# su1phurd/UAV-WRF-LES-PPO-LSTM

Hardware: AMD Instinct MI355X
Metric: env-steps/sec (rollout + GAE + 5-epoch PPO update), 4096 envs x 128 T per GPU, LSTM h=128 x1 (higher is better)
Workload: dtype f32

## Files before the change

include/uavppo.h:

```cpp
#ifndef UAVPPO_H
#define UAVPPO_H

#include <stddef.h>
#include <stdint.h>

#ifdef __cplusplus
extern "C" {
#endif

typedef struct uav_ctx uav_ctx;
typedef void* uav_stream;

#define UAV_ABI_VERSION 9

#define UAV_GAE_REFERENCE_EXACT 0
#define UAV_GAE_STANDARD        1

#define UAV_ENV_V20 0
#define UAV_ENV_V21 1
#define UAV_ENV_V11 2

#define UAV_FIELD_PROCEDURAL   0
#define UAV_FIELD_MATERIALISED 1

int         uav_abi_version(void);
const char* uav_last_error(void);

int  uav_create(uav_ctx** out, int device, size_t ws_bytes);
void uav_destroy(uav_ctx* ctx);

#define UAV_ARITH_FP16X3   0
#define UAV_ARITH_BF16X6   1
#define UAV_ARITH_F32_MFMA 2
int uav_set_lstm_arith(uav_ctx* ctx, int mode);
int uav_get_lstm_arith(const uav_ctx* ctx);
#define UAV_DEBUG_STEP_F32 1u
#define UAV_DEBUG_X_F32    2u
#define UAV_DEBUG_DG_F32   4u
#define UAV_DEBUG_GEMM_TN_OFF 0x10u
int uav_set_debug_flags(uav_ctx* ctx, unsigned flags);
int uav_absmax(uav_ctx* ctx, const float* x, int64_t n, float* out, uav_stream stream);

int uav_gae(uav_ctx* ctx, const float* rew, const float* val, const float* done,
            const float* last_val, int n_env, int horizon, float gamma, float lam, int mode,
            float* adv, uav_stream stream);

int uav_adv_stats(uav_ctx* ctx, const float* adv, int64_t n, double* stats3, uav_stream stream);
int uav_adv_normalise(uav_ctx* ctx, const float* adv, const float* val, int64_t n,
                      const double* stats3, float* adv_out, float* ret_out, uav_stream stream);

int uav_pack_success_bits(uav_ctx* ctx, const uint8_t* flags, int64_t n, int cap, uint8_t* msg, uav_stream stream);

int uav_ppo_loss(uav_ctx* ctx, const float* logits, const float* value, const int32_t* act,
                 const float* logp_old, const float* adv, const float* ret, const float* val_old,
                 int64_t n, int n_act, float inv_n, float clip, float ent_beta,
                 double* loss_sums, float* dlogits, float* dvalue, float* dhead_bias,
                 uav_stream stream);

int uav_ppo_loss_from_y(uav_ctx* ctx, const float* y, const float* w_head, const float* b_head,
                        const int32_t* act, const float* logp_old, const float* adv, const float* ret,
                        const float* val_old, int64_t n, int hidden, int n_act, float inv_n, float clip,
                        float ent_beta, double* loss_sums, float* dheads, float* dhead_bias,
                        uav_stream stream);

int uav_policy_sample(uav_ctx* ctx, const float* logits, int64_t n, int n_act, const float* u,
                      uint64_t seed, uint64_t counter, int64_t index_offset, const int32_t* forced_act,
                      int32_t* act_out, float* logp_out, float* probs_out, int32_t* nan_count,
                      uav_stream stream);

int uav_policy_sample_at(uav_ctx* ctx, const float* heads, int64_t heads_stride, int64_t n, int n_act, uint64_t seed,
                         uint64_t counter, int64_t index_offset, const int32_t* forced_act, int32_t* act_out, int T, int t,
                         int32_t* act_buf, float* val_buf, float* logp_buf, int32_t* nan_count, uav_stream stream);
int uav_store_transition(uav_ctx* ctx, int n, int T, int t, float* keep, const float* rew, const float* done,
                         const uint8_t* flags, float* keep_buf, float* rew_buf, float* done_buf, uint8_t* flags_buf,
                         uav_stream stream);

int uav_clip_adam(uav_ctx* ctx, float* param, const float* grad, float* exp_avg,
                  float* exp_avg_sq, int64_t n, int64_t step, float lr, float beta1, float beta2,
                  float eps, float max_norm, float* gnorm_out, float* pmax_out, uav_stream stream);
int uav_clip_adamw(uav_ctx* ctx, float* param, const float* grad, float* exp_avg, float* exp_avg_sq, int64_t n,
                   int64_t step, float lr, float beta1, float beta2, float eps, float weight_decay, float max_norm,
                   float* gnorm_out, uav_stream stream);
int uav_smooth_l1(uav_ctx* ctx, const float* pred, const float* target, int64_t n, float beta, double* loss_mean,
                  float* dpred, uav_stream stream);
int uav_mse_bce(uav_ctx* ctx, const float* out, const float* target, int64_t n, double* loss_mean, float* dout,
                uav_stream stream);

size_t uav_disc_param_count(int obs_dim, int n_act, int hidden);

int uav_disc_grad(uav_ctx* ctx, const float* params, const float* obs_e, const int32_t* act_e, int64_t n_e, const float* obs_p,
                  const int32_t* act_p, int64_t n_p, int obs_dim, int n_act, int hidden, float inv_ne, float inv_np,
                  double* loss_sums, float* grad, uav_stream stream);

int uav_disc_reward(uav_ctx* ctx, const float* params, const float* obs, const int32_t* act, int64_t n, int obs_dim, int n_act,
                    int hidden, float env_coef, float gail_coef, const float* rew_env, float* rew_out, uav_stream stream);

size_t uav_lstm_stepper_bytes(int N, int I, int H);
int uav_lstm_stepper_begin(uav_ctx* ctx, void* state, const float* w_ih, const float* w_hh, const float* b_ih,
                           const float* b_hh, const float* h0, const float* c0, int N, int I, int H, uav_stream stream);
int uav_lstm_stepper_step(uav_ctx* ctx, void* state, const float* x, const void* below, const float* keep_t, int N, int T,
                          int t, int I, int H, float* y, float* stash, float* hn, float* cn, uav_stream stream);
typedef struct uav_stepper_call {
    void* state; const float* x; const void* below; const float* keep_t;
    int t, I;
    float *y, *stash, *hn, *cn;
} uav_stepper_call;
int uav_lstm_stepper_step_pair(uav_ctx* ctx, const uav_stepper_call* a, const uav_stepper_call* b, int N, int T, int H,
                               uav_stream stream);

int uav_gemm_f32(uav_ctx* ctx, int64_t M, int64_t N, int64_t K, const float* A, int64_t sa_m,
                 int64_t sa_k, const float* B, int64_t sb_k, int64_t sb_n, float* C, int64_t ldc,
                 const float* bias, int accumulate, uav_stream stream);

int uav_gemm_f16x3(uav_ctx* ctx, int64_t M, int64_t N, int64_t K, const float* A, int64_t sa_m,
                   int64_t sa_k, const float* B, int64_t sb_k, int64_t sb_n, float* C, int64_t ldc,
                   const float* bias, int accumulate, const float* a_absmax, uav_stream stream);

int uav_colsum(uav_ctx* ctx, const float* x, int64_t rows, int cols, float* out, uav_stream stream);
int uav_ln_relu(uav_ctx* ctx, float* z, float* a, float* rstd, const float* gamma, const float* beta, int64_t rows,
                int cols, uav_stream stream);
int uav_ln_relu_bwd(uav_ctx* ctx, float* d, const float* xhat, const float* rstd, const float* gamma, const float* beta,
                    int64_t rows, int cols, float* dgamma, float* dbeta, uav_stream stream);

int64_t uav_mlp_param_count(int in_dim, int h1, int h2, int n_act);
int64_t uav_mlp_stash_floats(int h1, int h2);
int uav_mlp_fwd(uav_ctx* ctx, const float* params, const float* x, int64_t B, int in_dim, int h1,
                int h2, int n_act, float* heads, float* stash, uav_stream stream);
int uav_mlp_bwd(uav_ctx* ctx, const float* params, const float* x, float* stash,
                const float* dheads, int64_t B, int in_dim, int h1, int h2, int n_act,
                float* grad, uav_stream stream);

int uav_mlp_ppo_grad(uav_ctx* ctx, const float* params, const float* obs, const int32_t* act, const float* logp_old,
                     const float* adv, const float* ret, const float* val_old, int64_t n, int in_dim, int h1, int h2,
                     int n_act, float inv_n, float clip, float ent_beta, double* loss_sums, float* grad,
                     uav_stream stream);

int uav_lstm_fwd(uav_ctx* ctx, const float* x, const float* keep, const float* h0, const float* c0,
                 const float* w_ih, const float* w_hh, const float* b_ih, const float* b_hh,
                 int N, int T, int I, int H, float* y, float* hn, float* cn, float* stash,
                 const float* w_head, const float* b_head, int n_heads, float* heads,
                 uav_stream stream);
int uav_lstm_bwd(uav_ctx* ctx, const float* keep, const float* stash, const float* w_hh,
                 const float* dy, const float* dheads, const float* w_head, int n_heads,
                 const float* dhn, const float* dcn, int N, int T, int H, float* dgates, float* dh0,
                 float* dc0, const float* w_ih, int I, float* dx, uav_stream stream);
size_t uav_lstm_dgates_bytes(uav_ctx* ctx, int N, int T, int H);
int uav_lstm_dgates_f32(uav_ctx* ctx, const float* dgates, int N, int T, int H, float* out, uav_stream stream);
#define UAV_BWD_FUSES_DX 1
#define UAV_BWD_TAKES_DHEADS 2
#define UAV_BWD_STACKS 4
int uav_lstm_bwd_caps(uav_ctx* ctx, int I, int H);
typedef struct uav_lstm_bwd_layer {
    const float* keep;
    const float* stash;
    const float* w_hh;
    const float* w_ih;
    float* dgates;
    float* dx;
    const float* dhn;
    const float* dcn;
    float* dh0;
    float* dc0;
} uav_lstm_bwd_layer;
int uav_lstm_bwd_stack(uav_ctx* ctx, int n_layers, const uav_lstm_bwd_layer* layers, const float* dy, const float* dheads,
                       const float* w_head, int n_heads, int N, int T, int H, uav_stream stream);
int uav_lstm_wgrad(uav_ctx* ctx, const float* x, const float* keep, const float* h0, const float* y,
                   const float* stash, const float* dgates, const float* w_ih, const float* dheads,
                   int n_heads, int N, int T, int I, int H, float* dw_ih, float* dw_hh, float* db, float* db_hh,
                   float* dw_head, float* dx, uav_stream stream);

typedef struct uav_env_cfg {
    int32_t variant;
    int32_t field_mode;
    int32_t n_fields;
    int32_t bonus_is_f64;
    int32_t env_offset;
    int32_t n_env_total;
    int32_t trend_k;
    int32_t pad_;
    double  radius;
    double  bonus;
    uint64_t seed;
    const double* bank;
    const double* bank_src;
    const void*   curriculum;
} uav_env_cfg;

int uav_episode_rows(uav_ctx* ctx, const float* rew, const float* info, const uint8_t* flags, int n_env, int T, int env_offset,
                     double* carry, double* rows, int cap, int32_t* count, uav_stream stream);
size_t uav_curriculum_state_bytes(void);
int uav_curriculum_init(uav_ctx* ctx, void* state, double radius, double bonus, int bonus_is_f64, uav_stream stream);
int uav_curriculum_update(uav_ctx* ctx, void* state, const uint8_t* msgs, int world, int cap, uav_stream stream);

size_t uav_env_state_bytes(int n_env);
int uav_env_reset(uav_ctx* ctx, void* state, int n_env, const uav_env_cfg* cfg ,
                  float* obs_out, uav_stream stream);
int uav_env_step(uav_ctx* ctx, void* state, int n_env, const uav_env_cfg* cfg ,
                 const int32_t* act, const double* noise, float* obs_out, float* rew, float* done,
                 uint8_t* flags, float* info, float* term_obs, double* rew64, uav_stream stream);
int uav_env_peek(uav_ctx* ctx, const void* state, int n_env, float* pos, double* source,
                 int32_t* steps, int32_t* episode, uav_stream stream);

int uav_env_materialise(uav_ctx* ctx, const void* state, int n_env, const uav_env_cfg* cfg ,
                        int env_index, double* field_out, uav_stream stream);

int uav_rollout(uav_ctx* ctx, void* env_state, int n_env, const uav_env_cfg* cfg ,
                int policy_kind, const float* params, int hidden, int horizon, uint64_t iter,
                float* cur_obs, float* h, float* c, float* obs, int32_t* act, float* rew,
                float* val, float* logp, float* done, uint8_t* flags, float* keep, float* last_val,
                const int32_t* forced_act, const double* noise, int32_t* nan_count,
                float* stash, float* y_out, float* info, float* heads, uav_stream stream);

int uav_greedy_episodes(uav_ctx* ctx, void* env_state, int n_env, const uav_env_cfg* cfg , int policy_kind,
                        const float* params, int hidden, int steps, float* cur_obs, float* h, float* c, uint8_t* active,
                        const double* noise, int32_t* act, float* obs, float* pos, uint8_t* flags, int32_t* nan_count,
                        uav_stream stream);

typedef struct uav_stop_rule {
    int32_t window;
    float   pos_std_max, conc_coef, conc_peak, conc_min;
} uav_stop_rule;

int uav_greedy_episodes_stop(uav_ctx* ctx, void* env_state, int n_env, const uav_env_cfg* cfg , int policy_kind,
                             const float* params, int hidden, int steps, float* cur_obs, float* h, float* c, uint8_t* active,
                             const double* noise, int32_t* act, float* obs, float* pos, uint8_t* flags, int32_t* nan_count,
                             const uav_stop_rule* rule , float* stop_win, int32_t* stop_cnt, float* rule_val,
                             uav_stream stream);

int uav_stop_stability(uav_ctx* ctx, int n, const uav_stop_rule* rule , const float* pos, const float* obs2,
                       int64_t obs2_stride, const uint8_t* active, float* stop_win, int32_t* stop_cnt, uint8_t* stop,
                       float* value, uav_stream stream);

size_t uav_peak_stop_param_count(int hidden);

int uav_peak_stop_scan(uav_ctx* ctx, const float* params, int hidden, int window, const float* series, int64_t row_stride,
                       int64_t elem_stride, int n, int steps, const uint8_t* active, float* hist, int32_t* hist_cnt,
                       float prob_min, float* peak, float* prob, int32_t* first_hit, uav_stream stream);

int uav_rollout_tail(uav_ctx* ctx, void* env_state, int n_env, const uav_env_cfg* cfg , const float* y, int64_t y_stride,
                     int hidden, const float* w_head, const float* b_head, int n_act, float* heads, int64_t heads_stride, int T,
                     int t, uint64_t seed, uint64_t counter, int64_t index_offset, const int32_t* forced_act, const double* noise,
                     int32_t* act_out, float* cur_obs, float* obs_seq, float* keep, int32_t* act_buf, float* val_buf,
                     float* logp_buf, float* keep_buf, float* rew_buf, float* done_buf, uint8_t* flags_buf, int32_t* nan_count,
                     uav_stream stream);

#define UAV_COMM_ID_BYTES 128
int uav_rccl_version(int* out );
int uav_comm_unique_id(void* id_out );
int uav_comm_init(uav_ctx* ctx, const void* id , int rank, int world);
int uav_comm_world(const uav_ctx* ctx);
int uav_comm_rank(const uav_ctx* ctx);
int uav_comm_destroy(uav_ctx* ctx);
int uav_allreduce(uav_ctx* ctx, float* flat_grad, int64_t count, uav_stream stream);
int uav_allreduce_f64(uav_ctx* ctx, double* buf, int64_t count, uav_stream stream);
int uav_allgather_bytes(uav_ctx* ctx, const void* send, void* recv, int64_t bytes_per_rank, uav_stream stream);

#ifdef __cplusplus
}
#endif
#endif
```

uav-wrf-les-ppo-lstm_amd/csrc/adam.hip:

```cpp
#include "common.h"

constexpr int NORM_BLOCKS = 256;

__global__ __launch_bounds__(256) void sumsq_partial(const float* __restrict__ g, int64_t n,
                                                     double* __restrict__ partial, unsigned* __restrict__ pmax_bits) {
    __shared__ double sm[4];
    if (pmax_bits && blockIdx.x == 0 && threadIdx.x == 0) *pmax_bits = 0u;
    double q = 0.0;
    for (int64_t i = (int64_t)blockIdx.x * 256 + threadIdx.x; i < n; i += (int64_t)gridDim.x * 256) {
        const double v = (double)g[i];
        q += v * v;
    }
    q = block256_sum(q, sm);
    if (threadIdx.x == 0) partial[blockIdx.x] = q;
}

__global__ __launch_bounds__(256) void adam_kernel(float* __restrict__ p, const float* __restrict__ g,
                                                   float* __restrict__ m, float* __restrict__ v, int64_t n,
                                                   const double* __restrict__ partial, int nb, float max_norm,
                                                   float* __restrict__ gnorm_out, float b1, float b2,
                                                   float step_size, float sqrt_bc2, float eps, float decay,
                                                   unsigned* __restrict__ pmax_bits) {
#pragma clang fp contract(off)
    __shared__ double sm[4];
    __shared__ float coef_s;
    double q = 0.0;
    for (int i = threadIdx.x; i < nb; i += 256) q += partial[i];
    q = block256_sum(q, sm);
    if (threadIdx.x == 0) {
        const float norm = (float)sqrt(q);
        float coef = max_norm / (norm + 1e-6f);
        coef = coef > 1.0f ? 1.0f : coef;
        if (!(max_norm > 0.f)) coef = 1.0f;
        coef_s = coef;
        if (gnorm_out && blockIdx.x == 0) *gnorm_out = norm;
    }
    __syncthreads();
    const float coef = coef_s;
    float amax = 0.f;
    for (int64_t i = (int64_t)blockIdx.x * 256 + threadIdx.x; i < n; i += (int64_t)gridDim.x * 256) {
        const float gi = g[i] * coef;
        const float mi = m[i] + (gi - m[i]) * (1.0f - b1);
        const float vi = v[i] * b2 + (1.0f - b2) * gi * gi;
        m[i] = mi;
        v[i] = vi;
        const float denom = sqrtf(vi) / sqrt_bc2 + eps;
        const float pn = p[i] * decay - step_size * (mi / denom);
        p[i] = pn;
        amax = fmaxf(amax, pn == pn ? fabsf(pn) : __builtin_inff());
    }
    if (pmax_bits) {
#pragma unroll
        for (int o = 32; o > 0; o >>= 1) amax = fmaxf(amax, __shfl_xor(amax, o, 64));
        __shared__ float wmax[4];
        if ((threadIdx.x & 63) == 0) wmax[threadIdx.x >> 6] = amax;
        __syncthreads();
        if (threadIdx.x == 0)
            atomicMax(pmax_bits, __float_as_uint(fmaxf(fmaxf(wmax[0], wmax[1]), fmaxf(wmax[2], wmax[3]))));
    }
}

__global__ __launch_bounds__(256) void absmax_kernel(const float* __restrict__ x, int64_t n, unsigned* __restrict__ out) {
    float amax = 0.f;
    for (int64_t i = (int64_t)blockIdx.x * 256 + threadIdx.x; i < n; i += (int64_t)gridDim.x * 256) {
        const float v = x[i];
        amax = fmaxf(amax, v == v ? fabsf(v) : __builtin_inff());
    }
#pragma unroll
    for (int o = 32; o > 0; o >>= 1) amax = fmaxf(amax, __shfl_xor(amax, o, 64));
    if ((threadIdx.x & 63) == 0) atomicMax(out, __float_as_uint(amax));
}

extern "C" int uav_absmax(uav_ctx* ctx, const float* x, int64_t n, float* out, uav_stream stream) {
    UAV_REQUIRE(ctx && x && out && n > 0, "uav_absmax: bad argument");
    UAV_CHECK_HIP(hipMemsetAsync(out, 0, sizeof(float), as_stream(stream)));
    int nb = (int)((n + 4095) / 4096);
    if (nb > 1024) nb = 1024;
    hipLaunchKernelGGL(absmax_kernel, dim3(nb), dim3(256), 0, as_stream(stream), x, n, reinterpret_cast<unsigned*>(out));
    UAV_LAUNCH_CHECK();
    return 0;
}

static int clip_adam_impl(uav_ctx* ctx, float* param, const float* grad, float* exp_avg, float* exp_avg_sq, int64_t n,
                          int64_t step, float lr, float beta1, float beta2, float eps, float weight_decay, float max_norm,
                          float* gnorm_out, float* pmax_out, uav_stream stream) {
    UAV_REQUIRE(ctx && param && grad && exp_avg && exp_avg_sq && n > 0 && step >= 1, "uav_clip_adam: bad argument");
    unsigned* pmax_bits = reinterpret_cast<unsigned*>(pmax_out);
    double* partial = (double*)ctx->ws;
    int nb = (int)((n + 1023) / 1024);
    if (nb > NORM_BLOCKS) nb = NORM_BLOCKS;
    hipLaunchKernelGGL(sumsq_partial, dim3(nb), dim3(256), 0, as_stream(stream), grad, n, partial, pmax_bits);
    const double bc1 = 1.0 - pow((double)beta1, (double)step);
    const double bc2 = 1.0 - pow((double)beta2, (double)step);
    const float step_size = (float)((double)lr / bc1);
    const float sqrt_bc2 = (float)sqrt(bc2);
    int ab = (int)((n + 255) / 256);
    if (ab > 2048) ab = 2048;
    hipLaunchKernelGGL(adam_kernel, dim3(ab), dim3(256), 0, as_stream(stream), param, grad, exp_avg, exp_avg_sq, n,
                       partial, nb, max_norm, gnorm_out, beta1, beta2, step_size, sqrt_bc2, eps, 1.0f - lr * weight_decay, pmax_bits);
    UAV_LAUNCH_CHECK();
    return 0;
}

extern "C" int uav_clip_adam(uav_ctx* ctx, float* param, const float* grad, float* exp_avg, float* exp_avg_sq, int64_t n,
                             int64_t step, float lr, float beta1, float beta2, float eps, float max_norm, float* gnorm_out,
                             float* pmax_out, uav_stream stream) {
    return clip_adam_impl(ctx, param, grad, exp_avg, exp_avg_sq, n, step, lr, beta1, beta2, eps, 0.f, max_norm, gnorm_out,
                          pmax_out, stream);
}

extern "C" int uav_clip_adamw(uav_ctx* ctx, float* param, const float* grad, float* exp_avg, float* exp_avg_sq, int64_t n,
                              int64_t step, float lr, float beta1, float beta2, float eps, float weight_decay, float max_norm,
                              float* gnorm_out, uav_stream stream) {
    return clip_adam_impl(ctx, param, grad, exp_avg, exp_avg_sq, n, step, lr, beta1, beta2, eps, weight_decay, max_norm,
                          gnorm_out, nullptr, stream);
}

__global__ __launch_bounds__(256) void smooth_l1_kernel(const float* __restrict__ pred, const float* __restrict__ target,
                                                        int64_t n, float beta, double* __restrict__ loss_mean,
                                                        float* __restrict__ dpred) {
    __shared__ double sm[4];
    double s = 0.0;
    const float inv_n = 1.0f / (float)n;
    for (int64_t i = threadIdx.x; i < n; i += 256) {
        const float d = pred[i] - target[i], a = fabsf(d);
        if (a < beta) { s += 0.5 * (double)d * d / beta; dpred[i] = d / beta * inv_n; }
        else { s += (double)a - 0.5 * beta; dpred[i] = (d > 0.f ? 1.f : d < 0.f ? -1.f : d) * inv_n; }
    }
    const double r = block256_sum(s, sm);
    if (threadIdx.x == 0) loss_mean[0] = r / (double)n;
}

extern "C" int uav_smooth_l1(uav_ctx* ctx, const float* pred, const float* target, int64_t n, float beta, double* loss_mean,
                             float* dpred, uav_stream stream) {
    UAV_REQUIRE(ctx && pred && target && loss_mean && dpred && n > 0 && beta > 0.f, "uav_smooth_l1: bad argument");
    hipLaunchKernelGGL(smooth_l1_kernel, dim3(1), dim3(256), 0, as_stream(stream), pred, target, n, beta, loss_mean, dpred);
    UAV_LAUNCH_CHECK();
    return 0;
}

__global__ __launch_bounds__(256) void mse_bce_kernel(const float* __restrict__ out, const float* __restrict__ target, int64_t n,
                                                      double* __restrict__ loss_mean, float* __restrict__ dout) {
    __shared__ double sm[4];
    double s = 0.0;
    const float inv_n = 1.0f / (float)n;
    for (int64_t i = threadIdx.x; i < n; i += 256) {
        const float d = out[2 * i] - target[2 * i];
        const float z = out[2 * i + 1], yb = target[2 * i + 1];
        const float p = 1.0f / (1.0f + expf(-z));
        const float lgp = logf(p), lgq = logf(1.0f - p);
        const float lp = lgp < -100.f ? -100.f : lgp, lq = lgq < -100.f ? -100.f : lgq;
        s += (double)d * d - ((double)yb * lp + (1.0 - (double)yb) * lq);
// ... 15 lines not shown
```

uav-wrf-les-ppo-lstm_amd/csrc/gae.hip:

```cpp
#include "common.h"

__global__ __launch_bounds__(256) void gae_scan_kernel(const float* __restrict__ rew,
                                                       const float* __restrict__ val,
                                                       const float* __restrict__ done,
                                                       const float* __restrict__ last_val, int n_env,
                                                       int T, float gamma, float gl, int mode,
                                                       float* __restrict__ adv) {
#pragma clang fp contract(off)
    const int lane = threadIdx.x & 63;
    const int env = blockIdx.x * 4 + (threadIdx.x >> 6);
    if (env >= n_env) return;
    const size_t row = (size_t)env * T;
    const int nchunk = (T + 63) >> 6;
    float carry = 0.f;
    float v_right = 0.f, d_right = 0.f;
    for (int c = nchunk - 1; c >= 0; --c) {
        const int t = c * 64 + lane;
        const bool in = t < T;
        const float r = in ? rew[row + t] : 0.f;
        const float v = in ? val[row + t] : 0.f;
        const float d = in ? done[row + t] : 0.f;
        float v1 = __shfl_down(v, 1, 64);
        float d1 = __shfl_down(d, 1, 64);
        if (lane == 63) { v1 = v_right; d1 = d_right; }
        float a = 1.f, b = 0.f;
        if (in) {
            float nnt, nv;
            const bool last = (t == T - 1);
            if (mode == UAV_GAE_REFERENCE_EXACT) {
                nnt = 1.0f - (last ? d : d1);
                nv = (last ? v : v1) * nnt;
            } else {
                nnt = 1.0f - d;
                nv = (last ? (last_val ? last_val[env] : 0.f) : v1) * nnt;
            }
            b = (r + gamma * nv) - v;
            a = gl * nnt;
        }
#pragma unroll
        for (int o = 1; o < 64; o <<= 1) {
            const float a2 = __shfl_down(a, o, 64);
            const float b2 = __shfl_down(b, o, 64);
            if (lane + o < 64) {
                b = b + a * b2;
                a = a * a2;
            }
        }
        const float A = b + a * carry;
        if (in) adv[row + t] = A;
        carry = __shfl(A, 0, 64);
        v_right = __shfl(v, 0, 64);
        d_right = __shfl(d, 0, 64);
    }
}

constexpr int STATS_BLOCKS = 512;

__global__ __launch_bounds__(256) void adv_stats_partial(const float* __restrict__ x, int64_t n,
                                                         double* __restrict__ partial) {
    __shared__ double sm[4];
    double s = 0.0, q = 0.0;
    for (int64_t i = (int64_t)blockIdx.x * 256 + threadIdx.x; i < n; i += (int64_t)gridDim.x * 256) {
        const double v = (double)x[i];
        s += v;
        q += v * v;
    }
    s = block256_sum(s, sm);
    q = block256_sum(q, sm);
    if (threadIdx.x == 0) {
        partial[2 * blockIdx.x] = s;
        partial[2 * blockIdx.x + 1] = q;
    }
}

__global__ __launch_bounds__(256) void adv_stats_final(const double* __restrict__ partial, int nb,
                                                       int64_t n, double* __restrict__ stats3) {
    __shared__ double sm[4];
    double s = 0.0, q = 0.0;
    for (int i = threadIdx.x; i < nb; i += 256) {
        s += partial[2 * i];
        q += partial[2 * i + 1];
    }
    s = block256_sum(s, sm);
    q = block256_sum(q, sm);
    if (threadIdx.x == 0) {
        stats3[0] = s;
        stats3[1] = q;
        stats3[2] = (double)n;
    }
}

__global__ __launch_bounds__(256) void adv_normalise_kernel(const float* __restrict__ adv,
                                                            const float* __restrict__ val, int64_t n,
                                                            const double* __restrict__ stats3,
                                                            float* __restrict__ adv_out,
                                                            float* __restrict__ ret_out) {
#pragma clang fp contract(off)
    const double cnt = stats3[2];
    const double mean_d = stats3[0] / cnt;
    const double var = (stats3[1] - cnt * mean_d * mean_d) / (cnt - 1.0);
    const float mean = (float)mean_d;
    float sd = (float)sqrt(var > 0.0 ? var : (var == var ? 0.0 : var));
    if (sd < 1e-6f || sd != sd) sd = 1.0f;
    const float den = sd + 1e-6f;
    for (int64_t i = (int64_t)blockIdx.x * 256 + threadIdx.x; i < n; i += (int64_t)gridDim.x * 256) {
        const float a = (adv[i] - mean) / den;
        adv_out[i] = a;
        ret_out[i] = a + val[i];
    }
}

__global__ __launch_bounds__(1024) void pack_success_kernel(const uint8_t* __restrict__ flags, int64_t n, int cap,
                                                            uint8_t* __restrict__ msg) {
    __shared__ int part[32];
    const int tid = threadIdx.x;
    int64_t per = (n + 1023) / 1024;
    per = (per + 15) / 16 * 16;
    const int64_t lo = (int64_t)tid * per, hi = (lo + per < n) ? lo + per : n;
    const bool vec = (reinterpret_cast<uintptr_t>(flags) & 15) == 0;
    auto visit = [&](auto&& f) {
        int64_t i = lo;
        if (vec)
            for (; i + 16 <= hi; i += 16) {
                const uint4 w = *reinterpret_cast<const uint4*>(flags + i);
                if ((w.x | w.y | w.z | w.w) == 0u) continue;
                const unsigned ww[4] = {w.x, w.y, w.z, w.w};
#pragma unroll
                for (int q = 0; q < 4; ++q)
#pragma unroll
                    for (int k = 0; k < 4; ++k) {
                        const uint8_t v = (ww[q] >> (8 * k)) & 255;
                        if (v) f(v);
                    }
            }
        for (; i < hi; ++i)
            if (flags[i]) f(flags[i]);
    };
    int cnt = 0;
    visit([&](uint8_t) { ++cnt; });
    for (int i = tid; i < 4 + cap + 1; i += 1024) msg[i] = 0;
    const int lane = tid & 63, wv = tid >> 6;
    int inc = cnt;
#pragma unroll
    for (int o = 1; o < 64; o <<= 1) {
        const int v = __shfl_up(inc, o, 64);
        if (lane >= o) inc += v;
    }
    if (lane == 63) part[wv] = inc;
    __syncthreads();
    if (wv == 0) {
        int t = lane < 16 ? part[lane] : 0;
#pragma unroll
        for (int o = 1; o < 16; o <<= 1) {
// ... 91 lines not shown
            __syncthreads();
            for (int i = lane; i < nb; i += 64) chunk[i] = m[4 + base + i];
            __syncthreads();
            CurriculumState s = sh;
            for (int k = 0; k < nb;) {
                const int need = CUR_WINDOW - s.hist_len;
                const int n = (nb - k < need) ? nb - k : need;
                int succ = 0;
                for (int j = 0; j < n; j += 64) {
                    const int i = j + lane;
                    succ += __popcll(__ballot(i < n && chunk[k + i] != 0));
                }
                k += n;
                const double env_radius = s.radius;
                s.episodes += n; s.successes += succ;
                s.hist_len += n; s.win_succ += succ;
                const bool full = s.hist_len >= CUR_WINDOW;
                double rate = 0.0;
                if (full) {
                    rate = (double)s.win_succ / (double)s.hist_len;
                    s.bonus = s.bonus * pow(CUR_DECAY_FACTOR, 1.0 + rate);
                    s.bonus_is_f64 = 1.0;
                }
                s.bonus = fmax(s.bonus, 0.1);
                if (full) {
                    if (rate > CUR_SUCCESS_THRESHOLD)
                        s.radius = fmax(CUR_MIN_RADIUS, s.radius * pow(CUR_RADIUS_DECAY, 2.0 + 3.0 * (rate - CUR_SUCCESS_THRESHOLD)));
                    else if (rate < 0.25)
                        s.radius = fmin(CUR_INITIAL_RADIUS, s.radius * 1.1);
                    const double d = s.radius - env_radius;
                    if (fabs(d) > 5.0) s.radius = env_radius + 5.0 * (d > 0.0 ? 1.0 : (d < 0.0 ? -1.0 : 0.0));
                    s.hist_len = 0; s.win_succ = 0;
                }
            }
            __syncthreads();
            if (lane == 0) sh = s;
        }
    }
    __syncthreads();
    if (lane == 0) *st = sh;
}

extern "C" {

int uav_gae(uav_ctx* ctx, const float* rew, const float* val, const float* done,
            const float* last_val, int n_env, int horizon, float gamma, float lam, int mode,
            float* adv, uav_stream stream) {
    UAV_REQUIRE(ctx && rew && val && done && adv, "uav_gae: NULL argument");
    UAV_REQUIRE(n_env > 0 && horizon > 0, "uav_gae: n_env=%d horizon=%d", n_env, horizon);
    UAV_REQUIRE(mode == UAV_GAE_REFERENCE_EXACT || mode == UAV_GAE_STANDARD, "uav_gae: mode %d", mode);
    const float gl = (float)((double)gamma * (double)lam);
    const int blocks = (n_env + 3) / 4;
    hipLaunchKernelGGL(gae_scan_kernel, dim3(blocks), dim3(256), 0, as_stream(stream), rew, val, done,
                       last_val, n_env, horizon, gamma, gl, mode, adv);
    UAV_LAUNCH_CHECK();
    return 0;
}

int uav_adv_stats(uav_ctx* ctx, const float* adv, int64_t n, double* stats3, uav_stream stream) {
    UAV_REQUIRE(ctx && adv && stats3 && n > 0, "uav_adv_stats: bad argument");
    int nb = (int)((n + 1023) / 1024);
    if (nb > STATS_BLOCKS) nb = STATS_BLOCKS;
    double* partial = (double*)ctx->ws;
    hipLaunchKernelGGL(adv_stats_partial, dim3(nb), dim3(256), 0, as_stream(stream), adv, n, partial);
    hipLaunchKernelGGL(adv_stats_final, dim3(1), dim3(256), 0, as_stream(stream), partial, nb, n, stats3);
    UAV_LAUNCH_CHECK();
    return 0;
}

int uav_adv_normalise(uav_ctx* ctx, const float* adv, const float* val, int64_t n,
                      const double* stats3, float* adv_out, float* ret_out, uav_stream stream) {
    UAV_REQUIRE(ctx && adv && val && stats3 && adv_out && ret_out && n > 0, "uav_adv_normalise: bad argument");
    int nb = (int)((n + 1023) / 1024);
    if (nb > 2048) nb = 2048;
    hipLaunchKernelGGL(adv_normalise_kernel, dim3(nb), dim3(256), 0, as_stream(stream), adv, val, n, stats3,
                       adv_out, ret_out);
    UAV_LAUNCH_CHECK();
    return 0;
}


int uav_episode_rows(uav_ctx* ctx, const float* rew, const float* info, const uint8_t* flags, int n_env, int T, int env_offset,
                     double* carry, double* rows, int cap, int32_t* count, uav_stream stream) {
    UAV_REQUIRE(ctx && rew && info && flags && carry && rows && count && n_env > 0 && T > 0 && cap > 0, "uav_episode_rows: bad argument");
    hipLaunchKernelGGL(episode_rows_kernel, dim3((n_env + 63) / 64), dim3(64), 0, as_stream(stream), rew, info, flags, n_env, T, env_offset,
                       carry, rows, cap, count);
    UAV_LAUNCH_CHECK();
    return 0;
}

size_t uav_curriculum_state_bytes(void) { return sizeof(CurriculumState); }

int uav_curriculum_init(uav_ctx* ctx, void* state, double radius, double bonus, int bonus_is_f64, uav_stream stream) {
    UAV_REQUIRE(ctx && state && radius > 0.0, "uav_curriculum_init: bad argument");
    hipLaunchKernelGGL(curriculum_init_kernel, dim3(1), dim3(64), 0, as_stream(stream), (CurriculumState*)state, radius, bonus, bonus_is_f64);
    UAV_LAUNCH_CHECK();
    return 0;
}

int uav_curriculum_update(uav_ctx* ctx, void* state, const uint8_t* msgs, int world, int cap, uav_stream stream) {
    UAV_REQUIRE(ctx && state && msgs && world > 0 && cap > 0, "uav_curriculum_update: bad argument");
    hipLaunchKernelGGL(curriculum_update_kernel, dim3(1), dim3(64), 0, as_stream(stream), (CurriculumState*)state, msgs, world, cap);
    UAV_LAUNCH_CHECK();
    return 0;
}

int uav_pack_success_bits(uav_ctx* ctx, const uint8_t* flags, int64_t n, int cap, uint8_t* msg, uav_stream stream) {
    UAV_REQUIRE(ctx && flags && msg && n > 0 && cap > 0, "uav_pack_success_bits: bad argument");
    hipLaunchKernelGGL(pack_success_kernel, dim3(1), dim3(1024), 0, as_stream(stream), flags, n, cap, msg);
    UAV_LAUNCH_CHECK();
    return 0;
}

}
```

uav-wrf-les-ppo-lstm_amd/csrc/lstm.hip:

```cpp
#include <stdlib.h>
#include <type_traits>
#include "common.h"

int gemm_f32(uav_ctx* ctx, int64_t M, int64_t N, int64_t K, const float* A, int64_t sa_m, int64_t sa_k,
             const float* B, int64_t sb_k, int64_t sb_n, float* C, int64_t ldc, const float* bias,
             int accumulate, hipStream_t st);
int colsum(uav_ctx* ctx, const float* X, int64_t B, int C, float* out, float* scratch, hipStream_t st);
int colsum_absmax(uav_ctx* ctx, const float* X, int64_t B, int C, float* out, float* scratch, unsigned* absmax_bits,
                  hipStream_t st);
int colsum_xw(uav_ctx* ctx, const float* X, int64_t B, int C, const float* x, int I, float* colsum_out, float* xw_out,
              float* scratch, unsigned* absmax_bits, hipStream_t st, int xw_transposed = 0);
bool gemm_h3_ok(int64_t M, int64_t N, int64_t K, const float* A, int64_t sa_m, int64_t sa_k, const float* B, int64_t sb_k,
                int64_t sb_n);
int gemm_h3(uav_ctx* ctx, int64_t M, int64_t N, int64_t K, const float* A, int64_t sa_m, int64_t sa_k, const float* B,
            int64_t sb_k, int64_t sb_n, float* C, int64_t ldc, const float* bias, int accumulate, const unsigned* a_absmax,
            hipStream_t st);
int lstm_generic_fwd(uav_ctx* ctx, const float* keep, const float* h0, const float* c0, const float* w_hh, int N, int T,
                     int H, float* y, float* hn, float* cn, float* stash, hipStream_t st);
int lstm_h3_fwd(uav_ctx* ctx, const float* x, int I, const float* w_ih, const float* b_ih, const float* b_hh,
                const float* keep, const float* h0, const float* c0, const float* w_hh, int N, int T, float* y, float* hn,
                float* cn, float* stash, hipStream_t st);
bool lstm_h3_step_path(int H);
int lstm_generic_bwd(uav_ctx* ctx, const float* keep, const float* stash, const float* w_hh, const float* dy,
                     const float* dheads, const float* w_head, int n_heads,
                     const float* dhn, const float* dcn, int N, int T, int H, float* dgates, float* dh0, float* dc0,
                     const float* w_ih, int I, float* dx, hipStream_t st);
int lstm_generic_bwd_caps(int I, int H);
bool lstm_h3_stack_ok(int H);
bool lstm_h3_dg_packed(int H);
int lstm_pc_unpack(const void* dgates, int N, int T, float* out, hipStream_t st);
int lstm_pc_hprev_rows(const float* y, const float* keep, const float* h0, int N, int T, float* out, hipStream_t st);
int lstm_pc_wgrad(uav_ctx* ctx, const float* x, const float* y, const float* h0, const void* dgates, int N, int T, int I, float* dw_ih,
                  float* dw_hh, float* db, float* db_hh, hipStream_t st);
int lstm_h3_bwd_stack(uav_ctx* ctx, int nl, const uav_lstm_bwd_layer* layers, const float* dy, const float* dheads,
                      const float* w_head, int n_heads, int N, int T, hipStream_t st);
int lstm_wgrad_fused(uav_ctx* ctx, const float* dgates, const float* y, const float* keep, const float* h0,
                     const float* x, int I, const float* dheads, int NH, int N, int T, int H,
                     float* dw_ih, float* dw_hh, float* db, float* db_hh, float* dw_head, hipStream_t st);

constexpr int MT = 16;
constexpr int TC = 32;

#define sigmoidf_ fast_sigmoid
#define tanhf_ fast_tanh

template <int H>
struct FwdGeom {
    static constexpr int NW = H / 16;
    static constexpr int KS = H / 4;
    static constexpr int SEG = KS + 4;
    static constexpr int S = 4 * SEG + 8;
    static constexpr size_t LDS = (2 * MT * S + TC * MT * 8 + (TC + 1) * MT) * sizeof(float);
};
template <int H>
__device__ __forceinline__ int hpos(int u) { return (u / (H / 4)) * FwdGeom<H>::SEG + (u % (H / 4)); }

template <int H, bool FUSE_X>
__global__ __launch_bounds__(H * 4) void lstm_fwd_kernel(
    const float* __restrict__ x, const float* __restrict__ keep, const float* __restrict__ h0,
    const float* __restrict__ c0, const float* __restrict__ w_ih, const float* __restrict__ w_hh,
    const float* __restrict__ b_ih, const float* __restrict__ b_hh, int N, int T, int I,
    float* __restrict__ y, float* __restrict__ hn, float* __restrict__ cn, float* __restrict__ stash) {
    using G = FwdGeom<H>;
    constexpr int KS = G::KS, SEG = G::SEG, S = G::S;
    extern __shared__ __attribute__((aligned(16))) float smem[];
    float* hbuf = smem;
    float* xbuf = hbuf + 2 * MT * S;
    float* kbuf = xbuf + TC * MT * 8;

    const int lane = threadIdx.x & 63, w = threadIdx.x >> 6;
    const int j = lane & 15, kq = lane >> 4;
    const int u = 16 * w + j;
    const int n0 = blockIdx.x * MT;

    float wh[4][KS];
#pragma unroll
    for (int q = 0; q < 4; ++q) {
        const float* src = w_hh + (size_t)(q * H + u) * H + kq * KS;
#pragma unroll
        for (int s = 0; s < KS; s += 4) {
            const float4 v = *reinterpret_cast<const float4*>(src + s);
            wh[q][s] = v.x; wh[q][s + 1] = v.y; wh[q][s + 2] = v.z; wh[q][s + 3] = v.w;
        }
    }
    float wx[4][2], bias[4];
#pragma unroll
    for (int q = 0; q < 4; ++q) {
        bias[q] = FUSE_X ? (b_ih[q * H + u] + b_hh[q * H + u]) : 0.f;
#pragma unroll
        for (int s = 0; s < 2; ++s) {
            const int k = 2 * kq + s;
// ... 916 lines not shown

int uav_lstm_bwd_caps(uav_ctx* ctx, int I, int H) {
    if (!ctx) return 0;
    if (H == 64 || H == 128) return UAV_BWD_TAKES_DHEADS;
    uav_enter(ctx);
    return lstm_generic_bwd_caps(I, H);
}

size_t uav_lstm_dgates_bytes(uav_ctx* ctx, int N, int T, int H) {
    if (!ctx || N <= 0 || T <= 0 || H <= 0) return 0;
    uav_enter(ctx);
    if (H == DgPack::H && lstm_h3_dg_packed(H)) return DgPack(N, T).bytes();
    return (size_t)N * T * 4 * H * sizeof(float);
}

int uav_lstm_dgates_f32(uav_ctx* ctx, const float* dgates, int N, int T, int H, float* out, uav_stream stream) {
    UAV_REQUIRE(ctx && dgates && out && N > 0 && T > 0 && H > 0, "uav_lstm_dgates_f32: bad argument");
    uav_enter(ctx);
    const int form = H == DgPack::H ? uav_dg_form(ctx, dgates) : 0;
    if (form > 0 || (form < 0 && H == DgPack::H && lstm_h3_dg_packed(H))) return lstm_pc_unpack(dgates, N, T, out, as_stream(stream));
    UAV_CHECK_HIP(hipMemcpyAsync(out, dgates, (size_t)N * T * 4 * H * sizeof(float), hipMemcpyDeviceToDevice, as_stream(stream)));
    return 0;
}

int uav_lstm_bwd_stack(uav_ctx* ctx, int n_layers, const uav_lstm_bwd_layer* layers, const float* dy, const float* dheads,
                       const float* w_head, int n_heads, int N, int T, int H, uav_stream stream) {
    UAV_REQUIRE(ctx && layers, "uav_lstm_bwd_stack: NULL argument");
    uav_enter(ctx);
    UAV_REQUIRE((dy != nullptr) != (dheads != nullptr), "uav_lstm_bwd_stack: give exactly one of dy / dheads");
    UAV_REQUIRE(!dheads || (w_head && n_heads > 0 && n_heads <= 8), "uav_lstm_bwd_stack: dheads needs w_head and 1..8 heads");
    UAV_REQUIRE(N > 0 && T > 0, "uav_lstm_bwd_stack: N=%d T=%d", N, T);
    UAV_REQUIRE(H == 256 && lstm_h3_stack_ok(H), "uav_lstm_bwd_stack: H = 256 on the fp16-split arithmetic only (uav_lstm_bwd_caps)");
    return lstm_h3_bwd_stack(ctx, n_layers, layers, dy, dheads, w_head, n_heads, N, T, as_stream(stream));
}

int uav_lstm_bwd(uav_ctx* ctx, const float* keep, const float* stash, const float* w_hh, const float* dy,
                 const float* dheads, const float* w_head, int n_heads, const float* dhn, const float* dcn, int N,
                 int T, int H, float* dgates, float* dh0, float* dc0, const float* w_ih, int I, float* dx,
                 uav_stream stream) {
    UAV_REQUIRE(ctx && stash && w_hh && dgates, "uav_lstm_bwd: NULL argument");
    uav_enter(ctx);
    UAV_REQUIRE((dy != nullptr) != (dheads != nullptr), "uav_lstm_bwd: give exactly one of dy / dheads");
    UAV_REQUIRE(!dheads || (w_head && n_heads > 0 && n_heads <= 8), "uav_lstm_bwd: dheads needs w_head and 1..8 heads");
    UAV_REQUIRE(N > 0 && T > 0, "uav_lstm_bwd: N=%d T=%d", N, T);
    if (H != 64 && H != 128) {
        return lstm_generic_bwd(ctx, keep, stash, w_hh, dy, dheads, w_head, n_heads, dhn, dcn, N, T, H, dgates, dh0, dc0, w_ih, I, dx,
                                as_stream(stream));
    }
    UAV_REQUIRE(!dx, "uav_lstm_bwd: dx is not formed by the H = 64 / 128 sequence kernels (uav_lstm_wgrad does it)");
    return lstm_bwd_seq(keep, stash, w_hh, dy, dheads, w_head, n_heads, dhn, dcn, N, T, H, dgates, dh0, dc0,
                        as_stream(stream));
}

int uav_lstm_wgrad(uav_ctx* ctx, const float* x, const float* keep, const float* h0, const float* y,
                   const float* stash, const float* dgates, const float* w_ih, const float* dheads, int n_heads, int N,
                   int T, int I, int H, float* dw_ih, float* dw_hh, float* db, float* db_hh, float* dw_head, float* dx,
                   uav_stream stream) {
    UAV_REQUIRE(ctx && x && h0 && y && dgates && w_ih && dw_ih && dw_hh && db, "uav_lstm_wgrad: NULL argument");
    uav_enter(ctx);
    UAV_REQUIRE(N > 0 && T > 0 && I > 0 && H > 0, "uav_lstm_wgrad: N=%d T=%d I=%d H=%d", N, T, I, H);
    UAV_REQUIRE(!dheads || (dw_head && n_heads > 0 && n_heads <= 8), "uav_lstm_wgrad: dheads needs dw_head, 1..8 heads");
    hipStream_t st = as_stream(stream);
    const int64_t NT = (int64_t)N * T;
    int rc;
    if (I <= 6 && (H == 64 || H == 128)) {
        if ((rc = lstm_wgrad_fused(ctx, dgates, y, keep, h0, x, I, dheads, n_heads, N, T, H, dw_ih, dw_hh, db, db_hh,
                                   dw_head, st))) return rc;
    } else {
        UAV_REQUIRE(stash, "uav_lstm_wgrad: stash is required when I > 6");
        const size_t red_floats = (size_t)1024 * 9 * 4 * H + 64;
        UAV_REQUIRE(ctx->ws_bytes >= red_floats * sizeof(float) * 2, "uav_lstm_wgrad: workspace too small");
        float* red = (float*)((char*)ctx->ws + ctx->ws_bytes) - red_floats;
        uav_ctx sub = *ctx;
        sub.ws_bytes = ctx->ws_bytes - red_floats * sizeof(float);
        bool done = false;
        const float* hprev = stash + 5 * H;
        int64_t ld_hprev = 6 * H;
        {
            const int form = uav_dg_form(ctx, dgates), want = lstm_h3_dg_packed(H) ? 1 : 0;
            UAV_REQUIRE(form < 0 || H != DgPack::H || form == want, "uav_lstm_wgrad: this dgates buffer was written as %s but the handle's "
                        "arithmetic mode / debug flags now read %s (they must not change between uav_lstm_bwd and uav_lstm_wgrad)",
                        form ? "fp16 piece chunks" : "f32 rows", want ? "fp16 piece chunks" : "f32 rows");
            UAV_REQUIRE(H != DgPack::H || want || ctx->hslot_form.find(stash) != 0, "uav_lstm_wgrad: this stash was written by "
                        "uav_lstm_fwd / the stepper on the fp16-split arithmetic, which leaves out its h_prev slot, but the handle's "
                        "arithmetic mode / debug flags now read that slot (they must not change between the forward pass and "
                        "uav_lstm_wgrad)");
        }
        if (lstm_h3_dg_packed(H)) {
            if ((I <= 8 || I == H) && !dx) {
                if ((rc = lstm_pc_wgrad(ctx, x, y, h0, dgates, N, T, I, dw_ih, dw_hh, db, db_hh, st))) return rc;
                done = true;
            } else {
                const size_t f32_bytes = (size_t)NT * 5 * H * sizeof(float);
                UAV_REQUIRE(sub.ws_bytes >= f32_bytes + (64u << 20), "uav_lstm_wgrad (h=256, I=%d%s): needs %zu bytes of workspace for "
                            "the gate gradients and h_prev as f32 rows", I, dx ? ", dx" : "", f32_bytes + (64u << 20));
                float* rows = (float*)((char*)sub.ws + sub.ws_bytes - f32_bytes);
                sub.ws_bytes -= f32_bytes;
                if ((rc = lstm_pc_unpack(dgates, N, T, rows, st))) return rc;
                float* hp = rows + (size_t)NT * 4 * H;
                if ((rc = lstm_pc_hprev_rows(y, keep, h0, N, T, hp, st))) return rc;
                dgates = rows;
                hprev = hp;
                ld_hprev = H;
            }
        }
        const bool h3 = !uav_want_f32_mfma() && !uav_want_bf16x6() && (reinterpret_cast<uintptr_t>(dgates) & 15) == 0;
        unsigned* amax = h3 ? reinterpret_cast<unsigned*>(red + (size_t)1024 * 9 * 4 * H) : nullptr;
        auto product = [&](int64_t M, int64_t Nn, int64_t K, const float* A, int64_t sa_m, int64_t sa_k, const float* B,
                           int64_t sb_k, int64_t sb_n, float* C, int64_t ldc) {
            if (h3 && gemm_h3_ok(M, Nn, K, A, sa_m, sa_k, B, sb_k, sb_n))
                return gemm_h3(&sub, M, Nn, K, A, sa_m, sa_k, B, sb_k, sb_n, C, ldc, nullptr, 0, amax, st);
            return gemm_f32(&sub, M, Nn, K, A, sa_m, sa_k, B, sb_k, sb_n, C, ldc, nullptr, 0, st);
        };
        if (!done) {
            const bool narrow = I <= 8 && (reinterpret_cast<uintptr_t>(dgates) & 15) == 0;
            if (narrow) rc = colsum_xw(&sub, dgates, NT, 4 * H, x, I, db, dw_ih, red, amax, st);
            else rc = colsum_absmax(&sub, dgates, NT, 4 * H, db, red, amax, st);
            if (rc) return rc;
            if (db_hh) UAV_CHECK_HIP(hipMemcpyAsync(db_hh, db, (size_t)4 * H * sizeof(float), hipMemcpyDeviceToDevice, st));
            if ((rc = product(4 * H, H, NT, dgates, 1, 4 * H, hprev, ld_hprev, 1, dw_hh, H))) return rc;
            if (!narrow && (rc = product(4 * H, I, NT, dgates, 1, 4 * H, x, I, 1, dw_ih, I))) return rc;
        }
        if (dheads) {
            if (H % 4 == 0 && (reinterpret_cast<uintptr_t>(y) & 15) == 0)
                rc = colsum_xw(&sub, y, NT, H, dheads, n_heads, nullptr, dw_head, red, nullptr, st, 1);
            else
                rc = gemm_f32(&sub, n_heads, H, NT, dheads, 1, n_heads, y, H, 1, dw_head, H, nullptr, 0, st);
            if (rc) return rc;
        }
        if (dx) return product(NT, I, 4 * H, dgates, 4 * H, 1, w_ih, I, 1, dx, I);
        return 0;
    }
    if (dx) return gemm_f32(ctx, NT, I, 4 * H, dgates, 4 * H, 1, w_ih, I, 1, dx, I, nullptr, 0, st);
    return 0;
}

}
```

uav-wrf-les-ppo-lstm_amd/csrc/rollout.hip:

```cpp
#include "env_core.h"
#include "loss_core.h"
#include "rows_dot_core.h"
#include "stop_rule_core.h"

typedef float f32x4 __attribute__((ext_vector_type(4)));

int env_params_from_cfg(const uav_ctx* ctx, const uav_env_cfg* cfg, int n_env, EnvParams& P);
int launch_rollout_mlp(uav_ctx* ctx, void* env_state, int n_env, const uav_env_cfg* cfg, const float* params, int horizon,
                       uint64_t iter, float* cur_obs, float* obs, int32_t* act, float* rew, float* val, float* logp,
                       float* done, uint8_t* flags, float* last_val, const int32_t* forced_act, const double* noise,
                       int32_t* nan_count, float* info, float* heads, hipStream_t st);
int launch_greedy_mlp(const EnvParams& P, void* env_state, int n_env, const float* params, int steps, float* cur_obs,
                      uint8_t* active, const double* noise, int32_t* act, float* obs, float* pos, uint8_t* flags,
                      int32_t* nan_count, hipStream_t st);
int launch_greedy_mlp_stop(const EnvParams& P, void* env_state, int n_env, const float* params, int steps, float* cur_obs,
                           uint8_t* active, const double* noise, int32_t* act, float* obs, float* pos, uint8_t* flags,
                           int32_t* nan_count, const StopRule& rule, float* stop_win, int32_t* stop_cnt, float* rule_val,
                           hipStream_t st);

constexpr int RMT = 16;

#ifdef UAV_X6_PROFILE
__device__ unsigned long long g_roll_prof[8];
#define R_PROF_DECL unsigned long long pm_[8] = {0, 0, 0, 0, 0, 0, 0, 0}, pl_ = __builtin_readcyclecounter()
#define R_PROF_MARK(i) do { const unsigned long long n_ = __builtin_readcyclecounter(); pm_[i] += n_ - pl_; pl_ = n_; } while (0)
#define R_PROF_FLUSH() do { if (blockIdx.x == 0 && threadIdx.x == 0) for (int i_ = 0; i_ < 8; ++i_) g_roll_prof[i_] = pm_[i_]; } while (0)
extern "C" int uav_roll_prof_read(unsigned long long* out) {
    return hipMemcpyFromSymbol(out, HIP_SYMBOL(g_roll_prof), sizeof(g_roll_prof)) == hipSuccess ? 0 : 1;
}
#else
#define R_PROF_DECL
#define R_PROF_MARK(i)
#define R_PROF_FLUSH()
#endif
constexpr float R_F32_EPS = 1.1920928955078125e-07f;

#define r_sigmoid fast_sigmoid
#define r_tanh fast_tanh


template <int H>
struct RGeom {
    static constexpr int NW = H / 16;
    static constexpr int NS = H / 32;
    static constexpr int RS = H + 8;
    static constexpr int PLANE = RMT * RS;
    static constexpr int W0 = 4 * NS * 2 * 64 * 8;
    static constexpr size_t LDS = (2 * PLANE  + 2 * PLANE  + W0) * sizeof(unsigned short) +
                                  (NW * 8 * 64  + 4 * H ) * sizeof(float);
};

struct RolloutBufs {
    float* cur_obs; float* h; float* c;
    float* obs; int32_t* act; float* rew; float* val; float* logp; float* done; uint8_t* flags; float* keep;
    float* last_val; const int32_t* forced_act; const double* noise; int32_t* nan_count;
    float* info;
    float* heads;
    float* stash; float* y;
    uint8_t* active; float* pos;
    float* stop_win; int32_t* stop_cnt; float* rule_val; StopRule rule;
};

template <int H, int NA, bool GREEDY = false, bool STOP = false, bool TREND = false>
__global__ __launch_bounds__(H * 4) void rollout_lstm_kernel(EnvParams P_arg, EnvBlob blob, int N, int T,
                                                                        uint64_t iter, const float* __restrict__ params,
                                                                        RolloutBufs B) {
    using G = RGeom<H>;
    constexpr int NS = G::NS, RS = G::RS, PLANE = G::PLANE, W0 = G::W0, NW = G::NW;
    constexpr int NH = NA + 1;
    extern __shared__ __attribute__((aligned(16))) float smem[];
    unsigned short* hpl = reinterpret_cast<unsigned short*>(smem);
    unsigned short* whp = hpl + 2 * PLANE;
    unsigned short* w0p = whp + 2 * PLANE;
    float* wxl = reinterpret_cast<float*>(w0p + W0);
    float* bl = wxl + NW * 512;
    __shared__ __attribute__((aligned(16))) float xbuf[RMT * 8];
    __shared__ float kbuf[RMT];
    __shared__ float hd[RMT * 16];
    __shared__ unsigned short vis[RMT * NVIS];
    __shared__ EnvState es_s[RMT];
    __shared__ float trs[4 * RMT * 8];
    __shared__ __attribute__((aligned(16))) f32x4 acc0[4 * 64];
    __shared__ double env_tab[ENV_LDS_TABLE_DOUBLES];
    static_assert(!STOP || GREEDY, "rollout_lstm_kernel: the stop rule belongs to the greedy episodes");
    constexpr size_t STOP_LDS = STOP ? RMT * 2 * STOP_WIN_MAX * sizeof(float) : 0;
    static_assert(G::LDS + sizeof(xbuf) + sizeof(kbuf) + sizeof(hd) + sizeof(vis) + sizeof(es_s) + sizeof(trs) + sizeof(acc0) +
                      sizeof(env_tab) + STOP_LDS <= 160 * 1024, "rollout_lstm_kernel: LDS over 160 KB per workgroup");
    float* ring = nullptr;
    StopRing sr{0, 0};
    if constexpr (STOP) {
        __shared__ float rings[RMT * 2 * STOP_WIN_MAX];
        static_assert(sizeof(rings) == STOP_LDS, "stop rings");
        ring = rings + (threadIdx.x & 15) * 2 * STOP_WIN_MAX;
    }
    EnvParams P = P_arg;
    env_params_refresh(P);
    env_tables_to_lds(P, env_tab, threadIdx.x, H * 4);
    const int I = TREND ? 6 + P.trend_k : 6;

    const float* w_ih = params;
    const float* w_hh = w_ih + 4 * H * I;
    const float* b_ih = w_hh + 4 * H * H;
    const float* b_hh = b_ih + 4 * H;
    const float* w_hd = b_hh + 4 * H;
    const float* b_hd = w_hd + NH * H;

    const int lane = threadIdx.x & 63;
    const int w = __builtin_amdgcn_readfirstlane(threadIdx.x >> 6);
    const int j = lane & 15, kq = lane >> 4;
    const int n0 = blockIdx.x * RMT;
    const bool is_env_wave = (w == 0);
    const int uw = 16 * w + j;
    const int uo = 16 * w + 4 * kq;
    const int nj = min(n0 + j, N - 1);
    const bool live = n0 + j < N;
    const int my_env = n0 + lane;
    const bool env_lane = is_env_wave && lane < RMT && my_env < N;
    unsigned short* myvis = vis + (lane & 15) * NVIS;

    f16x8 wb[4][NS][2];
    f16x8* const w0f = reinterpret_cast<f16x8*>(w0p) + lane;
#pragma unroll
    for (int q = 0; q < 4; ++q)
#pragma unroll
        for (int s = 0; s < NS; ++s) {
            const float* src = w_hh + (size_t)(q * H + uw) * H + 32 * s + 8 * kq;
            const float4 v0 = *reinterpret_cast<const float4*>(src), v1 = *reinterpret_cast<const float4*>(src + 4);
            const float v[8] = {v0.x, v0.y, v0.z, v0.w, v1.x, v1.y, v1.z, v1.w};
            f16x8 p0v, p1v;
#pragma unroll
            for (int i = 0; i < 8; ++i) {
                _Float16 p0, p1;
                split2h(v[i], p0, p1);
                p0v[i] = p0; p1v[i] = p1;
            }
            if (is_env_wave) {
                w0f[((q * NS + s) * 2 + 0) * 64] = p0v;
                w0f[((q * NS + s) * 2 + 1) * 64] = p1v;
            } else {
                wb[q][s][0] = p0v; wb[q][s][1] = p1v;
            }
        }
    float* const wxw = wxl + w * 512 + lane;
#pragma unroll
    for (int q = 0; q < 4; ++q)
#pragma unroll
        for (int s = 0; s < 2; ++s) {
            const int k = 2 * kq + s;
            wxw[(2 * q + s) * 64] = (k < I) ? w_ih[(size_t)(q * H + uw) * I + k] : 0.f;
        }
    for (int idx = threadIdx.x; idx < 4 * H; idx += H * 4) bl[idx] = b_ih[idx] + b_hh[idx];
    for (int idx = threadIdx.x; idx < 16 * H; idx += H * 4) {
        const int hdx = idx / H, uu = idx % H;
        _Float16 p0, p1;
        split2h((hdx < NH) ? w_hd[(size_t)hdx * H + uu] : 0.f, p0, p1);
        unsigned short* d = whp + hdx * RS + uu;
        d[0] = h_bits(p0); d[PLANE] = h_bits(p1);
    }
    auto put_h = [&](const float (&hv)[4]) {
        unsigned short b[2][4];
#pragma unroll
        for (int r = 0; r < 4; ++r) {
            _Float16 p0, p1;
            split2h(hv[r], p0, p1);
            b[0][r] = h_bits(p0); b[1][r] = h_bits(p1);
        }
#pragma unroll
        for (int pc = 0; pc < 2; ++pc) {
            uint2 v;
            v.x = (unsigned)b[pc][0] | ((unsigned)b[pc][1] << 16);
            v.y = (unsigned)b[pc][2] | ((unsigned)b[pc][3] << 16);
            *reinterpret_cast<uint2*>(hpl + pc * PLANE + j * RS + uo) = v;
        }
    };
    float c_reg[4];
    {
        const float4 cv = *reinterpret_cast<const float4*>(B.c + (size_t)nj * H + uo);
        const float4 hv = *reinterpret_cast<const float4*>(B.h + (size_t)nj * H + uo);
        c_reg[0] = cv.x; c_reg[1] = cv.y; c_reg[2] = cv.z; c_reg[3] = cv.w;
        const float h_in[4] = {hv.x, hv.y, hv.z, hv.w};
        put_h(h_in);
        if constexpr (TREND && !GREEDY)
            if (B.stash && live) *reinterpret_cast<float4*>(B.stash + (size_t)(n0 + j) * T * (6 * H) + 5 * H + uo) = hv;
    }
    bool ran = true;
    if (is_env_wave && lane < RMT) {
        const int n = min(my_env, N - 1);
        es_s[lane] = env_load(blob, n);
        for (int k = 0; k < NVIS; ++k) myvis[k] = blob.visited[(size_t)n * NVIS + k];
#pragma unroll
        for (int f = 0; f < 8; ++f) xbuf[lane * 8 + f] = f < I ? B.cur_obs[(size_t)n * I + f] : 0.f;
        if constexpr (GREEDY) {
            ran = my_env < N && B.active[n] != 0;
            kbuf[lane] = ran ? 1.f : 0.f;
            if constexpr (STOP)
                sr = stop_ring_load(ring, B.stop_win + (size_t)n * B.rule.window * 2, B.stop_cnt[n], B.rule.window);
        } else {
            kbuf[lane] = 1.f;
        }
    }
    lds_barrier();

    f32x4 acc[4];
    int bo = uo;
    asm volatile("" : "+v"(bo));
    const float* blu = bl + bo;
    auto bias_acc = [&]() {
#pragma unroll
        for (int q = 0; q < 4; ++q) {
            const float4 v = *reinterpret_cast<const float4*>(blu + q * H);
            acc[q] = f32x4{v.x, v.y, v.z, v.w};
        }
    };
    auto recurrent = [&](auto&& wp0, auto&& wp1) {
        bias_acc();
        f32x4 acl[4];
#pragma unroll
        for (int q = 0; q < 4; ++q) acl[q] = f32x4{0.f, 0.f, 0.f, 0.f};
        const unsigned short* hrow = hpl + j * RS + 8 * kq;
#pragma unroll
        for (int s = 0; s < NS; ++s) {
            const f16x8 a0 = *reinterpret_cast<const f16x8*>(hrow + 32 * s);
            const f16x8 a1 = *reinterpret_cast<const f16x8*>(hrow + PLANE + 32 * s);
#pragma unroll
            for (int q = 0; q < 4; ++q) acl[q] = __builtin_amdgcn_mfma_f32_16x16x32_f16(wp1(q, s), a0, acl[q], 0, 0, 0);
#pragma unroll
            for (int q = 0; q < 4; ++q) acc[q] = __builtin_amdgcn_mfma_f32_16x16x32_f16(wp0(q, s), a0, acc[q], 0, 0, 0);
#pragma unroll
            for (int q = 0; q < 4; ++q) acl[q] = __builtin_amdgcn_mfma_f32_16x16x32_f16(wp0(q, s), a1, acl[q], 0, 0, 0);
            asm volatile("" ::: "memory");
        }
#pragma unroll
        for (int q = 0; q < 4; ++q) acc[q] = acc[q] + acl[q] * H3_LO;
    };
    auto recurrent_regs = [&]() {
        recurrent([&](int q, int s) { return wb[q][s][0]; }, [&](int q, int s) { return wb[q][s][1]; });
// ... 301 lines not shown
                    if (B.heads) {
#pragma unroll
                        for (int a = 0; a < NA; ++a) trs[3 * RMT * 8 + lane * 8 + a] = z[a];
                    }
                    if (B.info) {
#pragma unroll
                        for (int f = 0; f < 5; ++f) trs[2 * RMT * 8 + lane * 8 + f] = (float)so.info[f];
                        trs[2 * RMT * 8 + lane * 8 + 5] = so.obs[2];
                        trs[2 * RMT * 8 + lane * 8 + 6] = es.px;
                        trs[2 * RMT * 8 + lane * 8 + 7] = es.py;
                    }
                    constexpr int OW = TREND ? 8 : 6;
                    constexpr int SRC = TREND ? 3 * RMT * 8 + 5 : RMT * 8 + 6;
                    float ob_old[OW];
#pragma unroll
                    for (int f = 0; f < OW; ++f) ob_old[f] = xbuf[lane * 8 + f];
#pragma unroll
                    for (int f = 0; f < OW; ++f) trs[RMT * 8 + lane * 8 + f] = ob_old[f];
                    trs[SRC + lane * 8] = (float)es.sx;
                    trs[SRC + lane * 8 + 1] = (float)es.sy;
                    if (so.done) {
                        es.episode += 1;
                        env_begin_episode(P, eg, es, myvis);
                        env_obs(P, es, myvis, so.obs);
                    }
#pragma unroll
                    for (int f = 0; f < OW; ++f) xbuf[lane * 8 + f] = f < I ? so.obs[f] : 0.f;
                    es_s[lane] = es;
                    kbuf[lane] = so.done ? 0.f : 1.f;
                }
            }
            R_PROF_MARK(5);
            lds_barrier();
            if (!value_only && t + 1 < steps) {
#pragma unroll
                for (int q = 0; q < 4; ++q) acc[q] = acc0[q * 64 + lane];
            }
            if (!value_only) keep_fixup(t);
        }
        R_PROF_FLUSH();
    }
    if (live) *reinterpret_cast<float4*>(B.c + (size_t)(n0 + j) * H + uo) = float4{c_reg[0], c_reg[1], c_reg[2], c_reg[3]};
    if (GREEDY && env_lane) B.active[my_env] = kbuf[lane] != 0.f ? 1 : 0;
    if (env_lane && ran) {
        env_store(blob, my_env, es_s[lane]);
        for (int k = 0; k < NVIS; ++k) blob.visited[(size_t)my_env * NVIS + k] = myvis[k];
#pragma unroll
        for (int f = 0; f < (TREND ? 8 : 6); ++f) if (f < I) B.cur_obs[(size_t)my_env * I + f] = xbuf[lane * 8 + f];
        if constexpr (STOP)
            B.stop_cnt[my_env] = stop_ring_store(ring, sr, B.stop_win + (size_t)my_env * B.rule.window * 2, B.rule.window);
    }
}

template <int H, bool GREEDY = false, bool STOP = false, bool TREND = false>
static int launch_rollout(const EnvParams& P, EnvBlob blob, int N, int T, uint64_t iter, const float* params,
                          const RolloutBufs& B, hipStream_t st) {
    const dim3 grid((N + RMT - 1) / RMT), block(H * 4);
    UAV_CHECK_HIP(uav_dyn_lds(reinterpret_cast<const void*>(&rollout_lstm_kernel<H, 5, GREEDY, STOP, TREND>), (int)RGeom<H>::LDS));
    hipLaunchKernelGGL((rollout_lstm_kernel<H, 5, GREEDY, STOP, TREND>), grid, block, RGeom<H>::LDS, st, P, blob, N, T, iter, params, B);
    UAV_LAUNCH_CHECK();
    return 0;
}

template <int A>
__global__ __launch_bounds__(256) void rollout_tail_kernel(
    EnvParams P, EnvBlob b, int n, const float* __restrict__ y, int64_t ldy, int K, const float* __restrict__ w_head,
    const float* __restrict__ b_head, float* __restrict__ heads, int64_t ldh, int T, int t, uint64_t seed, uint64_t counter,
    int64_t index_offset, const int32_t* __restrict__ forced, const double* __restrict__ noise, int32_t* __restrict__ act_out,
    float* __restrict__ cur_obs, float* __restrict__ obs_seq, float* __restrict__ keep, int32_t* __restrict__ act_buf,
    float* __restrict__ val_buf, float* __restrict__ logp_buf, float* __restrict__ keep_buf, float* __restrict__ rew_buf,
    float* __restrict__ done_buf, uint8_t* __restrict__ flags_buf, int32_t* __restrict__ nan_count) {
    const int lane = threadIdx.x & 63;
    const int64_t m0 = ((int64_t)blockIdx.x * 4 + (threadIdx.x >> 6)) * 4;
    if (m0 >= n) return;
    env_params_refresh(P);
    RowsDot<8, 1> rd;
    rd.load_w(w_head, K, A + 1, K, lane);
    float red[4];
    rd.rows4(y, ldy, m0, n, K, lane, red);
    float z[A + 1];
#pragma unroll
    for (int o = 0; o <= A; ++o) {
        float v = 0.f;
#pragma unroll
        for (int r = 0; r < 4; ++r) {
            const float tot = RowsDot<8, 1>::total(red[r], o);
            if (lane == r) v = tot;
        }
        z[o] = v + b_head[o];
    }
    const int64_t i64 = m0 + lane;
    if (lane >= 4 || i64 >= n) return;
    const int i = (int)i64;
#pragma unroll
    for (int o = 0; o <= A; ++o) heads[i64 * ldh + o] = z[o];
    float p[A], qa;
    bool bad;
    int a = sample_categorical<A>(z, p, nullptr, seed, counter, index_offset + i, forced ? &forced[i] : nullptr, qa, bad);
    if (bad) atomicAdd(nan_count, 1);
    const int64_t col = i64 * T + t;
    act_out[i] = a;
    act_buf[col] = a;
    logp_buf[col] = logf(fminf(fmaxf(qa, F32_EPS), 1.0f - F32_EPS));
    val_buf[col] = z[A];
    EnvState s = env_load(b, i);
    unsigned short* vis = b.visited + (size_t)i * NVIS;
    const int eg = P.env_offset + i;
    double z0, z1;
    if (noise) { z0 = noise[2 * (size_t)i]; z1 = noise[2 * (size_t)i + 1]; }
    else env_step_noise(P, eg, s, z0, z1);
    a = a < 0 ? 0 : (a > 4 ? 4 : a);
    StepOut o;
// ... 6 lines not shown
    if (o.done) {
        s.episode += 1;
        env_begin_episode(P, eg, s, vis);
        env_obs(P, s, vis, o.obs);
    }
    env_store(b, i, s);
    keep_buf[col] = keep[i];
    rew_buf[col] = rw;
    done_buf[col] = d;
    flags_buf[col] = fl;
    keep[i] = 1.0f - d;
    const int od = 6 + P.trend_k;
    for (int k = 0; k < od; ++k) {
        cur_obs[(size_t)i * od + k] = o.obs[k];
        if (t + 1 < T) obs_seq[((size_t)i * T + t + 1) * od + k] = o.obs[k];
    }
}

extern "C" int uav_rollout_tail(uav_ctx* ctx, void* env_state, int n_env, const uav_env_cfg* cfg, const float* y, int64_t y_stride,
                                int hidden, const float* w_head, const float* b_head, int n_act, float* heads, int64_t heads_stride,
                                int T, int t, uint64_t seed, uint64_t counter, int64_t index_offset, const int32_t* forced_act,
                                const double* noise, int32_t* act_out, float* cur_obs, float* obs_seq, float* keep,
                                int32_t* act_buf, float* val_buf, float* logp_buf, float* keep_buf, float* rew_buf, float* done_buf,
                                uint8_t* flags_buf, int32_t* nan_count, uav_stream stream) {
    UAV_REQUIRE(ctx && env_state && y && w_head && b_head && heads && act_out && cur_obs && obs_seq && keep && act_buf && val_buf &&
                logp_buf && keep_buf && rew_buf && done_buf && flags_buf && nan_count, "uav_rollout_tail: NULL argument");
    UAV_REQUIRE(n_env > 0 && T > 0 && t >= 0 && t < T, "uav_rollout_tail: n_env=%d T=%d t=%d", n_env, T, t);
    UAV_REQUIRE(hidden >= 4 && hidden <= 256 && hidden % 4 == 0 && y_stride % 4 == 0 && y_stride >= hidden &&
                (reinterpret_cast<uintptr_t>(y) & 15) == 0 && (reinterpret_cast<uintptr_t>(w_head) & 15) == 0,
                "uav_rollout_tail: hidden %d (a multiple of 4 up to 256), y rows 16-byte aligned", hidden);
    UAV_REQUIRE(heads_stride > n_act, "uav_rollout_tail: heads_stride=%lld n_act=%d", (long long)heads_stride, n_act);
    EnvParams P;
    int rc = env_params_from_cfg(ctx, cfg, n_env, P);
    if (rc) return rc;
    const dim3 grid((unsigned)((n_env + 15) / 16));
#define LAUNCH_T(A_)                                                                                                              \
    hipLaunchKernelGGL(rollout_tail_kernel<A_>, grid, dim3(256), 0, as_stream(stream), P, env_blob_view(env_state, n_env), n_env, \
                       y, y_stride, hidden, w_head, b_head, heads, heads_stride, T, t, seed, counter, index_offset, forced_act,   \
                       noise, act_out, cur_obs, obs_seq, keep, act_buf, val_buf, logp_buf, keep_buf, rew_buf, done_buf,           \
                       flags_buf, nan_count)
    switch (n_act) {
        case 2: LAUNCH_T(2); break;
        case 3: LAUNCH_T(3); break;
        case 4: LAUNCH_T(4); break;
        case 5: LAUNCH_T(5); break;
        case 6: LAUNCH_T(6); break;
        default: UAV_REQUIRE(false, "uav_rollout_tail: n_act=%d unsupported (2..6)", n_act);
    }
#undef LAUNCH_T
    UAV_LAUNCH_CHECK();
    return 0;
}

extern "C" int uav_rollout(uav_ctx* ctx, void* env_state, int n_env, const uav_env_cfg* cfg, int policy_kind,
                           const float* params, int hidden, int horizon, uint64_t iter, float* cur_obs, float* h,
                           float* c, float* obs, int32_t* act, float* rew, float* val, float* logp, float* done,
                           uint8_t* flags, float* keep, float* last_val, const int32_t* forced_act,
                           const double* noise, int32_t* nan_count, float* stash, float* y_out, float* info,
                           float* heads, uav_stream stream) {
    UAV_REQUIRE(ctx && env_state && params && cur_obs && obs && act && rew && val && logp && done && flags && nan_count,
                "uav_rollout: NULL argument");
    UAV_REQUIRE(n_env > 0 && horizon > 0, "uav_rollout: n_env=%d horizon=%d", n_env, horizon);
    UAV_REQUIRE(policy_kind == 0 || policy_kind == 1, "uav_rollout: policy_kind %d (0 = MLP, 1 = LSTM)", policy_kind);
    if (policy_kind == 0) {
        UAV_REQUIRE(!stash && !y_out, "uav_rollout: stash / y_out belong to the LSTM policy");
        return launch_rollout_mlp(ctx, env_state, n_env, cfg, params, horizon, iter, cur_obs, obs, act, rew, val, logp, done,
                                  flags, last_val, forced_act, noise, nan_count, info, heads, as_stream(stream));
    }
    UAV_REQUIRE(h && c && keep, "uav_rollout: LSTM policy needs h, c, keep");
    EnvParams P;
    int rc = env_params_from_cfg(ctx, cfg, n_env, P);
    if (rc) return rc;
    UAV_REQUIRE((stash == nullptr) == (y_out == nullptr), "uav_rollout: stash and y_out go together");
    UAV_REQUIRE(!stash || (int64_t)n_env * horizon * 6 * hidden < (1ll << 32), "uav_rollout: stash rows exceed 32-bit offsets");
    RolloutBufs B{cur_obs, h, c, obs, act, rew, val, logp, done, flags, keep, last_val, forced_act, noise, nan_count, info, heads, stash, y_out};
    EnvBlob blob = env_blob_view(env_state, n_env);
    const bool trend = P.trend_k != 0;
    switch (hidden) {
        case 64: return trend ? launch_rollout<64, false, false, true>(P, blob, n_env, horizon, iter, params, B, as_stream(stream))
                              : launch_rollout<64>(P, blob, n_env, horizon, iter, params, B, as_stream(stream));
        case 128: return trend ? launch_rollout<128, false, false, true>(P, blob, n_env, horizon, iter, params, B, as_stream(stream))
                               : launch_rollout<128>(P, blob, n_env, horizon, iter, params, B, as_stream(stream));
    }
    UAV_REQUIRE(false, "uav_rollout: hidden=%d unsupported (64, 128)", hidden);
}

static int greedy_episodes_impl(const char* who, uav_ctx* ctx, void* env_state, int n_env, const uav_env_cfg* cfg, int policy_kind,
                                const float* params, int hidden, int steps, float* cur_obs, float* h, float* c, uint8_t* active,
                                const double* noise, int32_t* act, float* obs, float* pos, uint8_t* flags, int32_t* nan_count,
                                const uav_stop_rule* rule, float* stop_win, int32_t* stop_cnt, float* rule_val, hipStream_t st) {
    UAV_REQUIRE(ctx && env_state && params && cur_obs && active && act && obs && pos && flags && nan_count,
                "%s: NULL argument", who);
    UAV_REQUIRE(n_env > 0 && steps > 0, "%s: n_env=%d steps=%d", who, n_env, steps);
    UAV_REQUIRE(policy_kind == 0 || policy_kind == 1, "%s: policy_kind %d (0 = MLP, 1 = LSTM)", who, policy_kind);
    UAV_REQUIRE(ctx->lstm_arith == UAV_ARITH_FP16X3,
                "%s: the fused greedy kernels exist in the fp16x3 arithmetic only (handle mode %d)", who, ctx->lstm_arith);
    StopRule R{};
    if (rule) {
        UAV_REQUIRE(rule->window >= 1 && rule->window <= STOP_WIN_MAX, "%s: rule window=%d (1 .. %d)", who, rule->window,
                    STOP_WIN_MAX);
        UAV_REQUIRE(stop_win && stop_cnt, "%s: NULL stop_win / stop_cnt (the rule's window buffers)", who);
        R = StopRule{rule->window, rule->pos_std_max, rule->conc_coef, rule->conc_peak, rule->conc_min};
    }
    EnvParams P;
    int rc = env_params_from_cfg(ctx, cfg, n_env, P);
    if (rc) return rc;
    UAV_REQUIRE(policy_kind == 1 || P.trend_k == 0, "%s: trend_k=%d unsupported (the fused MLP kernels take 6 observation features)",
                who, P.trend_k);
    UAV_REQUIRE((int64_t)n_env * steps * (6 + P.trend_k) < (1ll << 31), "%s: n_env * steps too large", who);
    if (policy_kind == 0)
        return rule ? launch_greedy_mlp_stop(P, env_state, n_env, params, steps, cur_obs, active, noise, act, obs, pos, flags,
                                             nan_count, R, stop_win, stop_cnt, rule_val, st)
                    : launch_greedy_mlp(P, env_state, n_env, params, steps, cur_obs, active, noise, act, obs, pos, flags, nan_count, st);
    UAV_REQUIRE(h && c, "%s: LSTM policy needs h, c", who);
    RolloutBufs B{cur_obs, h, c, obs, act, nullptr, nullptr, nullptr, nullptr, flags, nullptr, nullptr, nullptr, noise, nan_count,
                  nullptr, nullptr, nullptr, nullptr, active, pos, stop_win, stop_cnt, rule_val, R};
    EnvBlob blob = env_blob_view(env_state, n_env);
#define LAUNCH_G(H_)                                                                                      \
    (P.trend_k ? (rule ? launch_rollout<H_, true, true, true>(P, blob, n_env, steps, 0, params, B, st)        \
                       : launch_rollout<H_, true, false, true>(P, blob, n_env, steps, 0, params, B, st))      \
               : (rule ? launch_rollout<H_, true, true>(P, blob, n_env, steps, 0, params, B, st)              \
                       : launch_rollout<H_, true>(P, blob, n_env, steps, 0, params, B, st)))
    switch (hidden) {
        case 64: return LAUNCH_G(64);
        case 128: return LAUNCH_G(128);
    }
#undef LAUNCH_G
    UAV_REQUIRE(false, "%s: hidden=%d unsupported by the fused kernel (64, 128)", who, hidden);
}

extern "C" int uav_greedy_episodes(uav_ctx* ctx, void* env_state, int n_env, const uav_env_cfg* cfg, int policy_kind,
                                   const float* params, int hidden, int steps, float* cur_obs, float* h, float* c,
                                   uint8_t* active, const double* noise, int32_t* act, float* obs, float* pos, uint8_t* flags,
                                   int32_t* nan_count, uav_stream stream) {
    return greedy_episodes_impl("uav_greedy_episodes", ctx, env_state, n_env, cfg, policy_kind, params, hidden, steps, cur_obs, h, c,
                                active, noise, act, obs, pos, flags, nan_count, nullptr, nullptr, nullptr, nullptr, as_stream(stream));
}

extern "C" int uav_greedy_episodes_stop(uav_ctx* ctx, void* env_state, int n_env, const uav_env_cfg* cfg, int policy_kind,
                                        const float* params, int hidden, int steps, float* cur_obs, float* h, float* c,
                                        uint8_t* active, const double* noise, int32_t* act, float* obs, float* pos, uint8_t* flags,
                                        int32_t* nan_count, const uav_stop_rule* rule, float* stop_win, int32_t* stop_cnt,
                                        float* rule_val, uav_stream stream) {
    UAV_REQUIRE(rule, "uav_greedy_episodes_stop: NULL rule");
    return greedy_episodes_impl("uav_greedy_episodes_stop", ctx, env_state, n_env, cfg, policy_kind, params, hidden, steps, cur_obs,
                                h, c, active, noise, act, obs, pos, flags, nan_count, rule, stop_win, stop_cnt, rule_val,
                                as_stream(stream));
}

__global__ __launch_bounds__(256) void stop_stability_kernel(StopRule R, int n, const float* __restrict__ pos,
                                                             const float* __restrict__ obs2, int64_t obs2_stride,
                                                             const uint8_t* __restrict__ active, float* __restrict__ stop_win,
                                                             int32_t* __restrict__ stop_cnt, uint8_t* __restrict__ stop,
                                                             float* __restrict__ value) {
    const int i = blockIdx.x * 256 + threadIdx.x;
    if (i >= n) return;
    if (active && active[i] == 0) {
        stop[i] = 0;
        value[i] = __builtin_nanf("");
        return;
    }
    float ring[2 * STOP_WIN_MAX];
    float* win = stop_win + (size_t)i * R.window * 2;
    StopRing sr = stop_ring_load(ring, win, stop_cnt[i], R.window);
    float v;
    const bool hit = stop_rule_step(R, ring, sr, pos[2 * (size_t)i], pos[2 * (size_t)i + 1], obs2[(size_t)i * obs2_stride], true, v);
    stop_cnt[i] = stop_ring_store(ring, sr, win, R.window);
    stop[i] = hit ? 1 : 0;
    value[i] = v;
// ... 17 lines not shown
```

uav-wrf-les-ppo-lstm_amd/csrc/wgrad.hip:

```cpp
#include <stdlib.h>
#include <type_traits>
#include "common.h"

typedef float f32x4 __attribute__((ext_vector_type(4)));

constexpr int KC = 16;

template <int H>
struct WG {
    static constexpr int NW = H / 16;
    static constexpr int NT_ = H / 16 + 1;
    static constexpr int NC = H + 16;
    static constexpr int SG = 4 * H + 16;
    static constexpr int SB = H + 16;
    static constexpr int SY = H + 16;
    static constexpr int SD = 48;
    static constexpr int BUF = KC * (SG + SB + SY + SD);
    static constexpr size_t LDS = 2 * BUF * sizeof(float);
    static constexpr size_t SLAB = (size_t)4 * H * NC + 16 * H;
};

template <int H>
__global__ __launch_bounds__(H * 4) void lstm_wgrad_kernel(
    const float* __restrict__ dgates, const float* __restrict__ y, const float* __restrict__ keep,
// ... 423 lines not shown
    WX_PROF_DECL;
    for (int sl = 0; sl < nslab; ++sl) {
        const int buf = sl & 1;
        WX_PROF_MARK(0);
        mfma_pair(buf, 0, sl);
        WX_PROF_DEP(acc[0][NT_ - 1]); WX_PROF_DEP(acc[1][NT_ - 1]); WX_PROF_MARK(2);
        commit_b(buf ^ 1);
        if constexpr (!P::LOADS_BETWEEN_TILES) load_b(sl + 2);
        WX_PROF_MARK(5);
        split_pair(sl, 1);
        WX_PROF_DEP(ap[0][0]); WX_PROF_DEP(ap[1][NP - 1]); WX_PROF_MARK(3);
        mfma_pair(buf, 1, sl);
        WX_PROF_DEP(acc[2][NT_ - 1]); WX_PROF_DEP(acc[3][NT_ - 1]); WX_PROF_MARK(4);
        if (!late) { lds_barrier(); WX_PROF_MARK(7); }
        split_pair(sl + 1, 0);
        WX_PROF_DEP(ap[0][0]); WX_PROF_DEP(ap[1][NP - 1]); WX_PROF_MARK(1);
        if (late) { lds_barrier(); WX_PROF_MARK(7); }
    }
    WX_PROF_FLUSH();
    float* slab = slabs + (size_t)blockIdx.x * WG<H>::SLAB;
#pragma unroll
    for (int mi = 0; mi < 4; ++mi)
#pragma unroll
        for (int r = 0; r < 4; ++r) {
            const float usc = pol.row_unscale(mi, r, kq);
#pragma unroll
            for (int ni = 0; ni < NT_; ++ni)
                slab[(size_t)(64 * w + 32 * (mi >> 1) + 2 * (4 * kq + r) + (mi & 1)) * G::NC + 16 * ni + j] =
                    acc[mi][ni][r] * (ni == NT_ - 1 ? usc * (P::BSCALE / P::XSCALE) : usc);
        }
#pragma unroll
    for (int r = 0; r < 4; ++r) slab[(size_t)4 * H * G::NC + (size_t)(4 * kq + r) * H + 16 * w + j] = acch[r];
}

template <int H, bool HEADS>
__global__ __launch_bounds__(H * 4) void lstm_wgrad_x6_kernel(
    const float* __restrict__ dgates, const float* __restrict__ y, const float* __restrict__ keep,
    const float* __restrict__ h0, const float* __restrict__ x, int I, const float* __restrict__ dheads, int NH,
    int N, int T, int rows_per_block, float* __restrict__ slabs) {
    lstm_wgrad_split<H, HEADS, WgBf16x6>(dgates, y, keep, h0, x, I, dheads, NH, N, T, rows_per_block, slabs);
}
template <int H, bool HEADS>
__global__ __launch_bounds__(H * 4) void lstm_wgrad_h3_kernel(
    const float* __restrict__ dgates, const float* __restrict__ y, const float* __restrict__ keep,
    const float* __restrict__ h0, const float* __restrict__ x, int I, const float* __restrict__ dheads, int NH,
    int N, int T, int rows_per_block, float* __restrict__ slabs) {
    lstm_wgrad_split<H, HEADS, WgF16x3>(dgates, y, keep, h0, x, I, dheads, NH, N, T, rows_per_block, slabs);
}

template <int H>
__global__ __launch_bounds__(256) void wgrad_reduce_kernel(const float* __restrict__ slabs, int nb, int I, int NH,
                                                           float* __restrict__ dw_ih, float* __restrict__ dw_hh,
                                                           float* __restrict__ db, float* __restrict__ db_hh,
                                                           float* __restrict__ dw_head) {
    using G = WG<H>;
    const size_t o = (size_t)blockIdx.x * 256 + threadIdx.x;
    if (o >= G::SLAB) return;
    float p8[8] = {0.f, 0.f, 0.f, 0.f, 0.f, 0.f, 0.f, 0.f};
    int b = 0;
    for (; b + 8 <= nb; b += 8)
#pragma unroll
        for (int k = 0; k < 8; ++k) p8[k] += slabs[(size_t)(b + k) * G::SLAB + o];
    for (; b < nb; ++b) p8[0] += slabs[(size_t)b * G::SLAB + o];
    const float s = ((p8[0] + p8[1]) + (p8[2] + p8[3])) + ((p8[4] + p8[5]) + (p8[6] + p8[7]));
    const size_t gsz = (size_t)4 * H * G::NC;
    if (o < gsz) {
        const int m = (int)(o / G::NC), c = (int)(o % G::NC);
        if (c < H) dw_hh[(size_t)m * H + c] = s;
        else if (c - H < I) dw_ih[(size_t)m * I + (c - H)] = s;
        else if (c - H == 6) {
            db[m] = s;
            if (db_hh) db_hh[m] = s;
        }
    } else if (dw_head) {
        const int a = (int)((o - gsz) / H), uu = (int)((o - gsz) % H);
        if (a < NH) dw_head[(size_t)a * H + uu] = s;
    }
}

template <class P, int H, bool HEADS>
static constexpr auto wgrad_split_kernel() {
    if constexpr (std::is_same<P, WgF16x3>::value) return &lstm_wgrad_h3_kernel<H, HEADS>;
    else return &lstm_wgrad_x6_kernel<H, HEADS>;
}

template <class P, int H>
static int launch_wgrad_split(const float* dgates, const float* y, const float* keep, const float* h0, const float* x, int I,
                              const float* dheads, int NH, int N, int T, int nb, int rpb, float* slabs, hipStream_t st) {
    const auto kern = dheads ? wgrad_split_kernel<P, H, true>() : wgrad_split_kernel<P, H, false>();
    const size_t lds = WGS<H, P>::LDS;
    UAV_CHECK_HIP(uav_dyn_lds(reinterpret_cast<const void*>(kern), (int)lds));
    hipLaunchKernelGGL(kern, dim3(nb), dim3(H * 4), lds, st, dgates, y, keep, h0, x, I, dheads, NH, N, T, rpb, slabs);
    return 0;
}

template <int H>
static int launch_wgrad(uav_ctx* ctx, const float* dgates, const float* y, const float* keep, const float* h0,
                        const float* x, int I, const float* dheads, int NH, int N, int T,
                        float* dw_ih, float* dw_hh, float* db, float* db_hh, float* dw_head, hipStream_t st) {
    using G = WG<H>;
    const int64_t NTr = (int64_t)N * T;
    int nb = ctx->num_cu;
    const int64_t max_nb = (int64_t)(ctx->ws_bytes / (G::SLAB * sizeof(float)));
    if (nb > max_nb) nb = (int)max_nb;
    UAV_REQUIRE(nb >= 1, "uav_lstm_wgrad: workspace too small for one slab");
    int64_t rpb = (NTr + nb - 1) / nb;
    rpb = (rpb + KC - 1) / KC * KC;
    nb = (int)((NTr + rpb - 1) / rpb);
    float* slabs = (float*)ctx->ws;
    {
        int64_t rpx = (NTr + nb - 1) / nb;
        rpx = (rpx + KS6 - 1) / KS6 * KS6;
        const int nbx = (int)((NTr + rpx - 1) / rpx);
        const bool split_ok = (NTr % rpx == 0) && T >= 8 && I <= 6 && (!dheads || NH <= 8) && NTr * 4 * H < (1ll << 30) &&
                              !uav_want_f32_mfma();
        if (split_ok) {
            const int rc = uav_want_bf16x6()
                               ? launch_wgrad_split<WgBf16x6, H>(dgates, y, keep, h0, x, I, dheads, NH, N, T, nbx, (int)rpx, slabs, st)
                               : launch_wgrad_split<WgF16x3, H>(dgates, y, keep, h0, x, I, dheads, NH, N, T, nbx, (int)rpx, slabs, st);
            if (rc) return rc;
            hipLaunchKernelGGL((wgrad_reduce_kernel<H>), dim3((unsigned)((G::SLAB + 255) / 256)), dim3(256), 0, st, slabs,
                               nbx, I, NH, dw_ih, dw_hh, db, db_hh, dw_head);
            UAV_LAUNCH_CHECK();
            return 0;
        }
    }
    UAV_CHECK_HIP(uav_dyn_lds(reinterpret_cast<const void*>(&lstm_wgrad_kernel<H>), (int)G::LDS));
    hipLaunchKernelGGL((lstm_wgrad_kernel<H>), dim3(nb), dim3(H * 4), G::LDS, st, dgates, y, keep, h0, x, I, dheads, NH, N,
                       T, rpb, slabs);
    hipLaunchKernelGGL((wgrad_reduce_kernel<H>), dim3((unsigned)((G::SLAB + 255) / 256)), dim3(256), 0, st, slabs, nb, I,
                       NH, dw_ih, dw_hh, db, db_hh, dw_head);
    UAV_LAUNCH_CHECK();
    return 0;
}

int lstm_wgrad_fused(uav_ctx* ctx, const float* dgates, const float* y, const float* keep, const float* h0,
                     const float* x, int I, const float* dheads, int NH, int N, int T, int H,
                     float* dw_ih, float* dw_hh, float* db, float* db_hh, float* dw_head, hipStream_t st) {
    switch (H) {
        case 64: return launch_wgrad<64>(ctx, dgates, y, keep, h0, x, I, dheads, NH, N, T, dw_ih, dw_hh, db, db_hh, dw_head, st);
        case 128: return launch_wgrad<128>(ctx, dgates, y, keep, h0, x, I, dheads, NH, N, T, dw_ih, dw_hh, db, db_hh, dw_head, st);
    }
    uav_set_error("lstm_wgrad_fused: H=%d unsupported", H);
    return 2;
}
```

uav-wrf-les-ppo-lstm_amd/uavppo/_lib.py:

```python
from __future__ import annotations

import ctypes as C
import os

import torch

_HERE = os.path.dirname(os.path.abspath(__file__))
LIB_PATH = os.environ.get("UAVPPO_LIB") or os.path.join(_HERE, "libuavppo.so")

c_f32p = C.c_void_p
P, I32, I64, U64, F32, F64, SZ = C.c_void_p, C.c_int, C.c_int64, C.c_uint64, C.c_float, C.c_double, C.c_size_t


class EnvCfg(C.Structure):
    _fields_ = [("variant", C.c_int32), ("field_mode", C.c_int32), ("n_fields", C.c_int32),
                ("bonus_is_f64", C.c_int32), ("env_offset", C.c_int32), ("n_env_total", C.c_int32),
                ("trend_k", C.c_int32), ("pad_", C.c_int32),
                ("radius", C.c_double), ("bonus", C.c_double),
                ("seed", C.c_uint64), ("bank", C.c_void_p), ("bank_src", C.c_void_p), ("curriculum", C.c_void_p)]


class StopRule(C.Structure):
    _fields_ = [("window", C.c_int32), ("pos_std_max", C.c_float), ("conc_coef", C.c_float), ("conc_peak", C.c_float),
                ("conc_min", C.c_float)]


class StepperCall(C.Structure):
    _fields_ = [("state", C.c_void_p), ("x", C.c_void_p), ("below", C.c_void_p), ("keep_t", C.c_void_p), ("t", C.c_int), ("I", C.c_int),
                ("y", C.c_void_p), ("stash", C.c_void_p), ("hn", C.c_void_p), ("cn", C.c_void_p)]


class LstmBwdLayer(C.Structure):
    _fields_ = [(n, C.c_void_p) for n in ("keep", "stash", "w_hh", "w_ih", "dgates", "dx", "dhn", "dcn", "dh0", "dc0")]


SIGNATURES = {
    "uav_abi_version": (I32, []),
    "uav_last_error": (C.c_char_p, []),
    "uav_create": (I32, [C.POINTER(C.c_void_p), I32, SZ]),
    "uav_destroy": (None, [P]),
    "uav_set_lstm_arith": (I32, [P, I32]),
    "uav_get_lstm_arith": (I32, [P]),
    "uav_set_debug_flags": (I32, [P, C.c_uint]),
    "uav_absmax": (I32, [P, P, I64, P, P]),
    "uav_gae": (I32, [P, P, P, P, P, I32, I32, F32, F32, I32, P, P]),
    "uav_adv_stats": (I32, [P, P, I64, P, P]),
    "uav_adv_normalise": (I32, [P, P, P, I64, P, P, P, P]),
    "uav_pack_success_bits": (I32, [P, P, I64, I32, P, P]),
    "uav_episode_rows": (I32, [P, P, P, P, I32, I32, I32, P, P, I32, P, P]),
    "uav_curriculum_state_bytes": (SZ, []),
    "uav_curriculum_init": (I32, [P, P, C.c_double, C.c_double, I32, P]),
    "uav_curriculum_update": (I32, [P, P, P, I32, I32, P]),
    "uav_ppo_loss": (I32, [P, P, P, P, P, P, P, P, I64, I32, F32, F32, F32, P, P, P, P, P]),
    "uav_ppo_loss_from_y": (I32, [P, P, P, P, P, P, P, P, P, I64, I32, I32, F32, F32, F32, P, P, P, P]),
    "uav_policy_sample": (I32, [P, P, I64, I32, P, U64, U64, I64, P, P, P, P, P, P]),
    "uav_policy_sample_at": (I32, [P, P, I64, I64, I32, U64, U64, I64, P, P, I32, I32, P, P, P, P, P]),
    "uav_store_transition": (I32, [P, I32, I32, I32, P, P, P, P, P, P, P, P, P]),
    "uav_rollout_tail": (I32, [P, P, I32, P, P, I64, I32, P, P, I32, P, I64, I32, I32, U64, U64, I64, P, P, P, P, P, P, P, P, P, P, P, P, P, P, P]),
    "uav_clip_adam": (I32, [P, P, P, P, P, I64, I64, F32, F32, F32, F32, F32, P, P, P]),
    "uav_clip_adamw": (I32, [P, P, P, P, P, I64, I64, F32, F32, F32, F32, F32, F32, P, P]),
    "uav_smooth_l1": (I32, [P, P, P, I64, F32, P, P, P]),
    "uav_mse_bce": (I32, [P, P, P, I64, P, P, P]),
    "uav_disc_param_count": (SZ, [I32, I32, I32]),
    "uav_disc_grad": (I32, [P, P, P, P, I64, P, P, I64, I32, I32, I32, F32, F32, P, P, P]),
    "uav_disc_reward": (I32, [P, P, P, P, I64, I32, I32, I32, F32, F32, P, P, P]),
    "uav_lstm_stepper_bytes": (SZ, [I32, I32, I32]),
    "uav_lstm_stepper_begin": (I32, [P, P, P, P, P, P, P, P, I32, I32, I32, P]),
    "uav_lstm_stepper_step": (I32, [P, P, P, P, P, I32, I32, I32, I32, I32, P, P, P, P, P]),
    "uav_lstm_stepper_step_pair": (I32, [P, P, P, I32, I32, I32, P]),
    "uav_gemm_f32": (I32, [P, I64, I64, I64, P, I64, I64, P, I64, I64, P, I64, P, I32, P]),
    "uav_gemm_f16x3": (I32, [P, I64, I64, I64, P, I64, I64, P, I64, I64, P, I64, P, I32, P, P]),
    "uav_colsum": (I32, [P, P, I64, I32, P, P]),
    "uav_ln_relu": (I32, [P, P, P, P, P, P, I64, I32, P]),
    "uav_ln_relu_bwd": (I32, [P, P, P, P, P, P, I64, I32, P, P, P]),
    "uav_mlp_param_count": (I64, [I32, I32, I32, I32]),
    "uav_mlp_stash_floats": (I64, [I32, I32]),
    "uav_mlp_fwd": (I32, [P, P, P, I64, I32, I32, I32, I32, P, P, P]),
    "uav_mlp_bwd": (I32, [P, P, P, P, P, I64, I32, I32, I32, I32, P, P]),
    "uav_mlp_ppo_grad": (I32, [P, P, P, P, P, P, P, P, I64, I32, I32, I32, I32, F32, F32, F32, P, P, P]),
    "uav_lstm_fwd": (I32, [P, P, P, P, P, P, P, P, P, I32, I32, I32, I32, P, P, P, P, P, P, I32, P, P]),
    "uav_lstm_bwd": (I32, [P, P, P, P, P, P, P, I32, P, P, I32, I32, I32, P, P, P, P, I32, P, P]),
    "uav_lstm_bwd_caps": (I32, [P, I32, I32]),
    "uav_lstm_dgates_bytes": (SZ, [P, I32, I32, I32]),
    "uav_lstm_dgates_f32": (I32, [P, P, I32, I32, I32, P, P]),
    "uav_lstm_bwd_stack": (I32, [P, I32, P, P, P, P, I32, I32, I32, I32, P]),
    "uav_lstm_wgrad": (I32, [P, P, P, P, P, P, P, P, P, I32, I32, I32, I32, I32, P, P, P, P, P, P, P]),
    "uav_env_state_bytes": (SZ, [I32]),
    "uav_env_reset": (I32, [P, P, I32, C.POINTER(EnvCfg), P, P]),
    "uav_env_step": (I32, [P, P, I32, C.POINTER(EnvCfg), P, P, P, P, P, P, P, P, P, P]),
    "uav_env_peek": (I32, [P, P, I32, P, P, P, P, P]),
    "uav_env_materialise": (I32, [P, P, I32, C.POINTER(EnvCfg), I32, P, P]),
    "uav_rollout": (I32, [P, P, I32, C.POINTER(EnvCfg), I32, P, I32, I32, U64, P, P, P, P, P, P, P, P, P, P,
                          P, P, P, P, P, P, P, P, P, P]),
    "uav_greedy_episodes": (I32, [P, P, I32, C.POINTER(EnvCfg), I32, P, I32, I32, P, P, P, P, P, P, P, P, P, P, P]),
    "uav_greedy_episodes_stop": (I32, [P, P, I32, C.POINTER(EnvCfg), I32, P, I32, I32, P, P, P, P, P, P, P, P, P, P,
                                       C.POINTER(StopRule), P, P, P, P]),
    "uav_stop_stability": (I32, [P, I32, C.POINTER(StopRule), P, P, I64, P, P, P, P, P, P]),
    "uav_peak_stop_param_count": (SZ, [I32]),
    "uav_peak_stop_scan": (I32, [P, P, I32, I32, P, I64, I64, I32, I32, P, P, P, F32, P, P, P, P]),
    "uav_rccl_version": (I32, [C.POINTER(C.c_int)]),
    "uav_comm_unique_id": (I32, [P]),
    "uav_comm_init": (I32, [P, P, I32, I32]),
    "uav_comm_world": (I32, [P]),
    "uav_comm_rank": (I32, [P]),
    "uav_comm_destroy": (I32, [P]),
    "uav_allreduce": (I32, [P, P, I64, P]),
    "uav_allreduce_f64": (I32, [P, P, I64, P]),
    "uav_allgather_bytes": (I32, [P, P, P, I64, P]),
}

_lib = None


def lib():
    global _lib
    if _lib is None:
        if not os.path.exists(LIB_PATH):
            raise RuntimeError(
                f"{LIB_PATH} not found: build it with `make -C uav-wrf-les-ppo-lstm_amd/csrc` "
                "(or python -c 'import __graft_entry__ as g; g.build()'). There is no CPU fallback.")
        _lib = C.CDLL(LIB_PATH)
        for name, (res, args) in SIGNATURES.items():
            fn = getattr(_lib, name)
            fn.restype = res
            fn.argtypes = args
    return _lib


def check(rc, what):
    if rc != 0:
        raise RuntimeError(f"{what} failed ({rc}): {lib().uav_last_error().decode()}")
```

uav-wrf-les-ppo-lstm_amd/uavppo/ops.py:

```python
from __future__ import annotations

import ctypes as C

import torch

from . import _lib
from ._lib import EnvCfg, check, lib

GAE_MODES = {"reference_exact": 0, "standard": 1}
WS_BYTES = 256 << 20


class Context:
    _per_device: dict = {}

    def __init__(self, device_index):
        if not torch.cuda.is_available():
            raise RuntimeError("uavppo needs an MI355X (gfx950) GPU: torch.cuda.is_available() is False "
                               "and there is no CPU fallback")
        h = C.c_void_p()
        check(lib().uav_create(C.byref(h), int(device_index), WS_BYTES), "uav_create")
        self.handle = h
        self.device = device_index
        self.initial_arith = {0: "fp16x3", 1: "bf16x6", 2: "f32_mfma"}[int(lib().uav_get_lstm_arith(h))]
# ... 25 lines not shown
        raise RuntimeError(f"{name}: expected a contiguous tensor")
    if dtype is not None and t.dtype != dtype:
        raise RuntimeError(f"{name}: expected {dtype}, got {t.dtype}")
    if shape is not None and tuple(t.shape) != tuple(shape):
        raise RuntimeError(f"{name}: expected shape {tuple(shape)}, got {tuple(t.shape)}")
    return C.c_void_p(t.data_ptr())


F32, F64, I32, U8 = torch.float32, torch.float64, torch.int32, torch.uint8


class _KernelTimer:

    CAP = 48

    def __init__(self):
        self.names, self.events = (), {}

    def enable(self, names):
        self.names, self.events = tuple(names), {n: [] for n in names}

    def disable(self):
        self.names, self.events = (), {}

    def bracket(self, name):
        if name not in self.names or len(self.events[name]) >= self.CAP:
            return None
        a, b = torch.cuda.Event(enable_timing=True), torch.cuda.Event(enable_timing=True)
        self.events[name].append((a, b))
        a.record()
        return b

    def summary(self):
        torch.cuda.synchronize()
        out = {}
        for n, ev in self.events.items():
            if ev:
                ms = [a.elapsed_time(b) for a, b in ev]
                out[n] = {"avg_ms": sum(ms) / len(ms), "n": len(ms)}
        return out


KERNEL_TIMER = _KernelTimer()


def gae(rew, val, done, gamma, lam, mode="reference_exact", last_val=None, out=None):
    n, T = rew.shape
    adv = torch.empty_like(rew) if out is None else out
    check(lib().uav_gae(_h(rew), _p(rew, F32, (n, T), "rew"), _p(val, F32, (n, T), "val"),
                        _p(done, F32, (n, T), "done"), _p(last_val, F32, (n,), "last_val"), n, T,
                        float(gamma), float(lam), GAE_MODES[mode], _p(adv, F32, (n, T), "adv"), _stream()),
          "uav_gae")
    return adv


def adv_stats(adv, out=None):
    stats = torch.empty(3, dtype=F64, device=adv.device) if out is None else out
    check(lib().uav_adv_stats(_h(adv), _p(adv, F32, name="adv"), adv.numel(), _p(stats, F64, (3,), "stats3"),
                              _stream()), "uav_adv_stats")
    return stats


def adv_normalise(adv, val, stats3, adv_out=None, ret_out=None):
    adv_out = torch.empty_like(adv) if adv_out is None else adv_out
    ret_out = torch.empty_like(adv) if ret_out is None else ret_out
    if val.shape != adv.shape:
        raise RuntimeError("adv_normalise: val/adv shape mismatch")
    check(lib().uav_adv_normalise(_h(adv), _p(adv, F32, name="adv"), _p(val, F32, name="val"), adv.numel(),
                                  _p(stats3, F64, (3,), "stats3"), _p(adv_out, F32, adv.shape, "adv_out"),
                                  _p(ret_out, F32, adv.shape, "ret_out"), _stream()), "uav_adv_normalise")
    return adv_out, ret_out


def pack_success_bits(flags, cap, out=None):
    f = flags.reshape(-1)
    out = torch.empty(4 + cap + 1, dtype=U8, device=f.device) if out is None else out
    check(lib().uav_pack_success_bits(_h(f), _p(f, U8, name="flags"), f.numel(), int(cap), _p(out, U8, (4 + cap + 1,), "msg"),
                                      _stream()), "uav_pack_success_bits")
    return out


def episode_rows(rew, info, flags, carry, rows, count, env_offset=0):
    N, T = rew.shape
    check(lib().uav_episode_rows(_h(rew), _p(rew, F32, (N, T), "rew"), _p(info, F32, (N, T, 10), "info"), _p(flags, U8, (N, T), "flags"),
                                 N, T, int(env_offset), _p(carry, torch.float64, (N, 8), "carry"),
                                 _p(rows, torch.float64, (rows.shape[0], 12), "rows"), int(rows.shape[0]), _p(count, I32, (1,), "count"),
                                 _stream()), "uav_episode_rows")


def curriculum_state(device, radius=50.0, bonus=0.6, bonus_is_f64=False):
    st = torch.zeros(int(lib().uav_curriculum_state_bytes()), dtype=U8, device=device)
    curriculum_init(st, radius, bonus, bonus_is_f64)
    return st


def curriculum_init(state, radius, bonus, bonus_is_f64=False):
    check(lib().uav_curriculum_init(_h(state), _p(state, U8, name="curriculum state"), float(radius), float(bonus), int(bool(bonus_is_f64)),
                                    _stream()), "uav_curriculum_init")


def curriculum_update(state, msgs, cap):
    world = int(msgs.shape[0])
    check(lib().uav_curriculum_update(_h(state), _p(state, U8, name="curriculum state"), _p(msgs, U8, (world, 4 + cap + 1), "msgs"), world,
                                      int(cap), _stream()), "uav_curriculum_update")


# ... 152 lines not shown
    check(lib().uav_comm_init(Context.get(device).handle, C.c_char_p(uid), int(rank), int(world)), "uav_comm_init")


def comm_world(device=None):
    return int(lib().uav_comm_world(Context.get(device).handle))


def comm_destroy(device=None):
    check(lib().uav_comm_destroy(Context.get(device).handle), "uav_comm_destroy")


def comm_allreduce(t):
    if t.dtype == torch.float32:
        check(lib().uav_allreduce(_h(t), _p(t, F32, name="t"), t.numel(), _stream()), "uav_allreduce")
    elif t.dtype == torch.float64:
        check(lib().uav_allreduce_f64(_h(t), _p(t, torch.float64, name="t"), t.numel(), _stream()), "uav_allreduce_f64")
    else:
        raise RuntimeError(f"comm_allreduce: f32 or f64, got {t.dtype}")
    return t


def comm_allgather_bytes(msg):
    w = comm_world(msg.device)
    if w < 1:
        raise RuntimeError("comm_allgather_bytes: no communicator on this device's handle")
    out = torch.empty(w, msg.numel(), dtype=torch.uint8, device=msg.device)
    check(lib().uav_allgather_bytes(_h(msg), _p(msg, torch.uint8, name="msg"), _p(out, torch.uint8, name="out"), msg.numel(), _stream()),
          "uav_allgather_bytes")
    return out


def get_lstm_arith(device=None):
    m = int(lib().uav_get_lstm_arith(Context.get(device).handle))
    return {v: k for k, v in ARITH.items()}[m]


def absmax(x, out=None):
    out = torch.empty(1, dtype=F32, device=x.device) if out is None else out
    check(lib().uav_absmax(_h(x), _p(x, F32, name="x"), x.numel(), _p(out, F32, (1,), "out"), _stream()), "uav_absmax")
    return out


def clip_adam(param, grad, exp_avg, exp_avg_sq, step, lr, beta1=0.9, beta2=0.999, eps=1e-8, max_norm=0.5,
              gnorm_out=None, pmax_out=None):
    n = param.numel()
    for t, nm in ((grad, "grad"), (exp_avg, "exp_avg"), (exp_avg_sq, "exp_avg_sq")):
        if t.numel() != n:
            raise RuntimeError(f"clip_adam: {nm} has {t.numel()} elements, param has {n}")
    check(lib().uav_clip_adam(_h(param), _p(param, F32, name="param"), _p(grad, F32, name="grad"),
                              _p(exp_avg, F32, name="exp_avg"), _p(exp_avg_sq, F32, name="exp_avg_sq"), n, int(step),
                              float(lr), float(beta1), float(beta2), float(eps), float(max_norm),
                              _p(gnorm_out, F32, (1,), "gnorm_out"), _p(pmax_out, F32, (1,), "pmax_out"), _stream()),
          "uav_clip_adam")


def gemm_rows(a, b_t, bias, out):
    N, K = a.shape
    M = b_t.shape[0]
    if a.stride(1) != 1 or out.stride(1) != 1 or tuple(out.shape) != (N, M) or b_t.shape[1] != K:
        raise RuntimeError("gemm_rows: a [N, K] and out [N, M] need unit stride along the last index; b_t is [M, K]")
    for t, nm in ((a, "a"), (out, "out")):
        if not t.is_cuda or t.dtype != F32:
            raise RuntimeError(f"gemm_rows: {nm}: expected a float32 GPU tensor")
    check(lib().uav_gemm_f32(_h(a), N, M, K, C.c_void_p(a.data_ptr()), a.stride(0), 1, _p(b_t, F32, name="b_t"), 1, K,
                             C.c_void_p(out.data_ptr()), out.stride(0), _p(bias, F32, (M,), "bias"), 0, _stream()),
          "uav_gemm_f32")
    return out


def gemm(a, b, trans_a=False, trans_b=False, bias=None, out=None, accumulate=False, split_fp16=False, a_absmax=None):
    if a.dim() != 2 or b.dim() != 2:
        raise RuntimeError("gemm: 2-D tensors expected")
    M, K = (a.shape[1], a.shape[0]) if trans_a else a.shape
    K2, N = (b.shape[1], b.shape[0]) if trans_b else b.shape
    if K != K2:
        raise RuntimeError(f"gemm: inner dimensions differ ({K} vs {K2})")
    sa_m, sa_k = (1, a.shape[1]) if trans_a else (a.shape[1], 1)
    sb_k, sb_n = (1, b.shape[1]) if trans_b else (b.shape[1], 1)
    if out is None:
        if accumulate:
            raise RuntimeError("gemm: accumulate needs out")
        out = torch.empty(M, N, dtype=F32, device=a.device)
    if split_fp16:
        check(lib().uav_gemm_f16x3(_h(a), M, N, K, _p(a, F32, name="a"), sa_m, sa_k, _p(b, F32, name="b"), sb_k, sb_n,
                                   _p(out, F32, (M, N), "out"), N, _p(bias, F32, (N,), "bias"), int(accumulate),
                                   _p(a_absmax, F32, (1,), "a_absmax"), _stream()), "uav_gemm_f16x3")
        return out
    check(lib().uav_gemm_f32(_h(a), M, N, K, _p(a, F32, name="a"), sa_m, sa_k, _p(b, F32, name="b"), sb_k, sb_n,
                             _p(out, F32, (M, N), "out"), N, _p(bias, F32, (N,), "bias"), int(accumulate), _stream()),
          "uav_gemm_f32")
    return out


def mlp_param_count(in_dim=6, h1=256, h2=128, n_act=5):
    return int(lib().uav_mlp_param_count(in_dim, h1, h2, n_act))


def mlp_fwd(params, x, in_dim=6, h1=256, h2=128, n_act=5, stash=None):
    B = x.shape[0]
    if params.numel() != mlp_param_count(in_dim, h1, h2, n_act):
        raise RuntimeError("mlp_fwd: flat parameter buffer has the wrong size")
    heads = torch.empty(B, n_act + 1, dtype=F32, device=x.device)
    per = int(lib().uav_mlp_stash_floats(h1, h2))
    if stash is None:
        stash = torch.empty(B * per, dtype=F32, device=x.device)
    elif stash.numel() < B * per:
# ... 128 lines not shown
                                          I, H, _p(y, F32, (N, T, H), "y"), _p(stash, F32, (N, T, 6 * H), "stash"), _p(self.hn),
                                          _p(self.cn), _stream()), "uav_lstm_stepper_step")


def _stepper_call(sp, x, t, y, stash, below, keep):
    N, I, H = sp.N, sp.I, sp.H
    T = x.shape[1]
    c = _lib.StepperCall()
    c.state = _p(sp.state).value
    c.x = _p(x, F32, (N, T, I), "x").value
    c.below = None if below is None else _p(below.state).value
    c.keep_t = None if keep is None else _p(keep, F32, (N,), "keep").value
    c.t, c.I = int(t), I
    c.y = _p(y, F32, (N, T, H), "y").value
    c.stash = _p(stash, F32, (N, T, 6 * H), "stash").value
    c.hn, c.cn = _p(sp.hn).value, _p(sp.cn).value
    return c


def lstm_stepper_step_pair(a, b):
    ca, cb = _stepper_call(*a), _stepper_call(*b)
    sp, x = a[0], a[1]
    check(lib().uav_lstm_stepper_step_pair(_h(sp.state), C.byref(ca), C.byref(cb), sp.N, x.shape[1], sp.H, _stream()),
          "uav_lstm_stepper_step_pair")


def lstm_dgates_bytes(N, T, H, device):
    n = int(lib().uav_lstm_dgates_bytes(Context.get(torch.device(device)).handle, int(N), int(T), int(H)))
    if n <= 0:
        raise RuntimeError(f"uav_lstm_dgates_bytes({N}, {T}, {H}) = {n}")
    return n


def lstm_dgates(N, T, H, device):
    nbytes = lstm_dgates_bytes(N, T, H, device)
    if nbytes == N * T * 4 * H * 4:
        return torch.empty(N, T, 4 * H, dtype=F32, device=device)
    return torch.empty((nbytes + 3) // 4, dtype=F32, device=device)


def _pdg(dgates, N, T, H):
    need = lstm_dgates_bytes(N, T, H, dgates.device)
    if dgates.numel() * 4 < need:
        raise RuntimeError(f"dgates: {dgates.numel() * 4} bytes, uav_lstm_dgates_bytes({N}, {T}, {H}) = {need} (allocate with ops.lstm_dgates)")
    return _p(dgates, F32, None, "dgates")


def lstm_dgates_f32(dgates, N, T, H):
    out = torch.empty(N, T, 4 * H, dtype=F32, device=dgates.device)
    check(lib().uav_lstm_dgates_f32(_h(dgates), _pdg(dgates, N, T, H), N, T, H, _p(out), _stream()), "uav_lstm_dgates_f32")
    return out


def lstm_wgrad(x, keep, h0, y, stash, dgates, w_ih, dheads=None):
    N, T, I = x.shape
    H = y.shape[-1]
    dev = x.device
    nh = 0 if dheads is None else dheads.shape[-1]
    dw_ih = torch.empty(4 * H, I, dtype=F32, device=dev)
    dw_hh = torch.empty(4 * H, H, dtype=F32, device=dev)
    db = torch.empty(4 * H, dtype=F32, device=dev)
    dw_head = torch.empty(nh, H, dtype=F32, device=dev) if nh else None
    check(lib().uav_lstm_wgrad(_h(x), _p(x, F32, (N, T, I), "x"), _p(keep, F32, (N, T), "keep"), _p(h0, F32, (N, H), "h0"),
                               _p(y, F32, (N, T, H), "y"), _p(stash, F32, (N, T, 6 * H), "stash"),
                               _pdg(dgates, N, T, H), _p(w_ih, F32, (4 * H, I), "w_ih"),
                               _p(dheads, F32, (N, T, nh), "dheads"), nh, N, T, I, H,
                               _p(dw_ih, F32, (4 * H, I), "dw_ih"), _p(dw_hh, F32, (4 * H, H), "dw_hh"),
                               _p(db, F32, (4 * H,), "db"), None, _p(dw_head, F32, (nh, H), "dw_head"), _p(None), _stream()),
          "uav_lstm_wgrad")
    return {"dw_ih": dw_ih, "dw_hh": dw_hh, "db": db, "dw_head": dw_head}


def lstm_bwd_caps(device, I, H):
    return int(lib().uav_lstm_bwd_caps(Context.get(torch.device(device)).handle, int(I), int(H)))


def lstm_bwd_stack(layers, keep, dy=None, dheads=None, w_head=None):
    N, T, H6 = layers[0]["stash"].shape
    H = H6 // 6
    arr = (_lib.LstmBwdLayer * len(layers))()
    for a, d in zip(arr, layers):
        a.keep = None if keep is None else _p(keep, F32, (N, T), "keep").value
        a.stash = _p(d["stash"], F32, (N, T, 6 * H), "stash").value
        a.w_hh = _p(d["w_hh"], F32, (4 * H, H), "w_hh").value
        a.w_ih = None if d.get("w_ih") is None else _p(d["w_ih"], F32, (4 * H, H), "w_ih").value
        a.dgates = _pdg(d["dgates"], N, T, H).value
        a.dx = None if d.get("dx") is None else _p(d["dx"], F32, (N, T, H), "dx").value
        a.dhn = a.dcn = a.dh0 = a.dc0 = None
    nh = 0 if dheads is None else dheads.shape[-1]
    _t = KERNEL_TIMER.bracket("lstm_bwd")
    check(lib().uav_lstm_bwd_stack(_h(layers[0]["stash"]), len(layers), C.byref(arr), _p(dy, F32, (N, T, H), "dy"),
                                   _p(dheads, F32, (N, T, nh), "dheads"), _p(w_head, F32, (nh, H), "w_head"), nh, N, T, H, _stream()),
          "uav_lstm_bwd_stack")
    if _t is not None:
        _t.record()


def lstm_bwd(x, keep, stash, w_ih, w_hh, y, h0, dy=None, dheads=None, w_head=None, dhn=None, dcn=None, need_dx=False,
             dgates=None, dw_ih=None, dw_hh=None, db=None, dw_head=None, want_dstate=True, wgrad_dheads=None, bwd_done=False,
             db_hh=None):
    N, T, I = x.shape
    H = w_hh.shape[1]
    dev = x.device
    dgates = lstm_dgates(N, T, H, dev) if dgates is None else dgates
    dx = torch.empty(N, T, I, dtype=F32, device=dev) if (need_dx and not bwd_done) else None
    dw_ih = torch.empty(4 * H, I, dtype=F32, device=dev) if dw_ih is None else dw_ih
    dw_hh = torch.empty(4 * H, H, dtype=F32, device=dev) if dw_hh is None else dw_hh
    db = torch.empty(4 * H, dtype=F32, device=dev) if db is None else db
    dh0 = torch.empty(N, H, dtype=F32, device=dev) if want_dstate else None
    dc0 = torch.empty(N, H, dtype=F32, device=dev) if want_dstate else None
    nh = 0 if dheads is None else dheads.shape[-1]
    if wgrad_dheads is None:
        wgrad_dheads = dheads
    nhw = 0 if wgrad_dheads is None else wgrad_dheads.shape[-1]
    if wgrad_dheads is not None and dw_head is None:
        dw_head = torch.empty(nhw, H, dtype=F32, device=dev)
    dx_in_bwd = bool(need_dx and lstm_bwd_caps(x.device, I, H) & 1) or bwd_done
    _t = None if bwd_done else KERNEL_TIMER.bracket("lstm_bwd")
    if not bwd_done:
        check(lib().uav_lstm_bwd(_h(x), _p(keep, F32, (N, T), "keep"), _p(stash, F32, (N, T, 6 * H), "stash"),
                                 _p(w_hh, F32, (4 * H, H), "w_hh"), _p(dy, F32, (N, T, H), "dy"),
                                 _p(dheads, F32, (N, T, nh), "dheads"), _p(w_head, F32, (nh, H), "w_head"), nh,
                                 _p(dhn, F32, (N, H), "dhn"), _p(dcn, F32, (N, H), "dcn"), N, T, H,
                                 _pdg(dgates, N, T, H), _p(dh0), _p(dc0),
                                 _p(w_ih, F32, (4 * H, I), "w_ih") if dx_in_bwd else None, I, _p(dx) if dx_in_bwd else None,
                                 _stream()), "uav_lstm_bwd")
    if _t is not None:
        _t.record()
    _t = KERNEL_TIMER.bracket("lstm_wgrad")
    check(lib().uav_lstm_wgrad(_h(x), _p(x, F32, (N, T, I), "x"), _p(keep, F32, (N, T), "keep"), _p(h0, F32, (N, H), "h0"),
                               _p(y, F32, (N, T, H), "y"), _p(stash, F32, (N, T, 6 * H), "stash"),
                               _pdg(dgates, N, T, H), _p(w_ih, F32, (4 * H, I), "w_ih"),
                               _p(wgrad_dheads, F32, (N, T, nhw), "dheads"), nhw, N, T, I, H,
                               _p(dw_ih, F32, (4 * H, I), "dw_ih"), _p(dw_hh, F32, (4 * H, H), "dw_hh"),
                               _p(db, F32, (4 * H,), "db"), _p(db_hh, F32, (4 * H,), "db_hh"), _p(dw_head, F32, (nhw, H), "dw_head"),
                               None if dx_in_bwd else _p(dx), _stream()),
          "uav_lstm_wgrad")
    if _t is not None:
        _t.record()
    return {"dx": dx, "dw_ih": dw_ih, "dw_hh": dw_hh, "db": db, "dh0": dh0, "dc0": dc0, "dgates": dgates,
            "dw_head": dw_head}


def env_materialise(state, n_env, cfg, env_index, out=None):
    out = torch.empty(500, 500, 2, dtype=F64, device=state.device) if out is None else out
    check(lib().uav_env_materialise(_h(state), _p(state, U8, name="env state"), n_env, C.byref(cfg), int(env_index),
                                    _p(out, F64, (500, 500, 2), "field_out"), _stream()), "uav_env_materialise")
    return out


def ln_relu(z, gamma, beta, want_stats=False):
    rows, cols = z.shape
    a = torch.empty_like(z)
    rstd = torch.empty(rows, dtype=F32, device=z.device)
    check(lib().uav_ln_relu(_h(z), _p(z, F32, (rows, cols), "z"), _p(a, F32), _p(rstd, F32), _p(gamma, F32, (cols,), "gamma"),
                            _p(beta, F32, (cols,), "beta"), rows, cols, _stream()), "uav_ln_relu")
    return (a, rstd) if want_stats else a


def ln_relu_bwd(d, xhat, rstd, gamma, beta, dgamma=None, dbeta=None):
    rows, cols = d.shape
    dg = torch.empty(cols, dtype=F32, device=d.device) if dgamma is None else dgamma
    db = torch.empty(cols, dtype=F32, device=d.device) if dbeta is None else dbeta
    check(lib().uav_ln_relu_bwd(_h(d), _p(d, F32, (rows, cols), "d"), _p(xhat, F32, (rows, cols), "xhat"),
                                _p(rstd, F32, (rows,), "rstd"), _p(gamma, F32, (cols,), "gamma"), _p(beta, F32, (cols,), "beta"),
                                rows, cols, _p(dg, F32, (cols,), "dgamma"), _p(db, F32, (cols,), "dbeta"), _stream()),
          "uav_ln_relu_bwd")
    return d, dg, db


def smooth_l1(pred, target, beta):
    n = pred.numel()
    loss = torch.zeros(1, dtype=F64, device=pred.device)
    dpred = torch.empty(n, dtype=F32, device=pred.device)
    check(lib().uav_smooth_l1(_h(pred), _p(pred, F32, (n,), "pred"), _p(target, F32, (n,), "target"), n, float(beta),
                              _p(loss, F64), _p(dpred, F32), _stream()), "uav_smooth_l1")
    return loss, dpred


def mse_bce(out, target):
    n = out.shape[0]
    loss = torch.zeros(1, dtype=F64, device=out.device)
    dout = torch.empty(n, 2, dtype=F32, device=out.device)
    check(lib().uav_mse_bce(_h(out), _p(out, F32, (n, 2), "out"), _p(target, F32, (n, 2), "target"), n, _p(loss, F64),
                            _p(dout, F32), _stream()), "uav_mse_bce")
    return loss, dout


def clip_adamw(param, grad, exp_avg, exp_avg_sq, step, lr, beta1=0.9, beta2=0.999, eps=1e-8, weight_decay=0.01, max_norm=1.0,
               gnorm_out=None):
    n = param.numel()
    check(lib().uav_clip_adamw(_h(param), _p(param, F32, (n,), "param"), _p(grad, F32, (n,), "grad"),
                               _p(exp_avg, F32, (n,), "exp_avg"), _p(exp_avg_sq, F32, (n,), "exp_avg_sq"), n, int(step),
                               float(lr), float(beta1), float(beta2), float(eps), float(weight_decay), float(max_norm),
                               _p(gnorm_out, F32, (1,), "gnorm_out"), _stream()), "uav_clip_adamw")


def colsum(x, out=None):
    rows, cols = x.shape
    out = torch.empty(cols, dtype=F32, device=x.device) if out is None else out
    check(lib().uav_colsum(_h(x), _p(x, F32, (rows, cols), "x"), rows, cols, _p(out, F32, (cols,), "out"), _stream()),
          "uav_colsum")
    return out


def rollout_lstm(env_state, n_env, cfg, params, hidden, horizon, it, cur_obs, h, c, bufs, last_val=None,
                 forced_act=None, noise=None, nan_count=None, stash=None, y=None, info=None, heads=None):
    N, T, D = n_env, horizon, 6 + cfg.trend_k
    _t = KERNEL_TIMER.bracket("rollout")
    check(lib().uav_rollout(_h(cur_obs), _p(env_state, U8, name="env state"), N, C.byref(cfg), 1,
                            _p(params, F32, name="params"), int(hidden), T, int(it),
                            _p(cur_obs, F32, (N, D), "cur_obs"), _p(h, F32, (N, hidden), "h"), _p(c, F32, (N, hidden), "c"),
                            _p(bufs["obs"], F32, (N, T, D), "obs"), _p(bufs["act"], I32, (N, T), "act"),
                            _p(bufs["rew"], F32, (N, T), "rew"), _p(bufs["val"], F32, (N, T), "val"),
                            _p(bufs["logp"], F32, (N, T), "logp"), _p(bufs["done"], F32, (N, T), "done"),
                            _p(bufs["flags"], U8, (N, T), "flags"), _p(bufs["keep"], F32, (N, T), "keep"),
                            _p(last_val, F32, (N,), "last_val"), _p(forced_act, I32, (N, T), "forced_act"),
                            _p(noise, F64, (N, T, 2), "noise"), _p(nan_count, I32, (1,), "nan_count"),
                            _p(stash, F32, (N, T, 6 * hidden), "stash"), _p(y, F32, (N, T, hidden), "y"),
                            _p(info, F32, (N, T, 10), "info"), _p(heads, F32, (N, T, 6), "heads"), _stream()),
          "uav_rollout")
    if _t is not None:
        _t.record()


def rollout_mlp(env_state, n_env, cfg, params, horizon, it, cur_obs, bufs, last_val=None, forced_act=None, noise=None,
                nan_count=None, info=None, heads=None):
    N, T = n_env, horizon
    _t = KERNEL_TIMER.bracket("rollout")
    check(lib().uav_rollout(_h(cur_obs), _p(env_state, U8, name="env state"), N, C.byref(cfg), 0,
                            _p(params, F32, name="params"), 0, T, int(it), _p(cur_obs, F32, (N, 6), "cur_obs"), None, None,
                            _p(bufs["obs"], F32, (N, T, 6), "obs"), _p(bufs["act"], I32, (N, T), "act"),
                            _p(bufs["rew"], F32, (N, T), "rew"), _p(bufs["val"], F32, (N, T), "val"),
                            _p(bufs["logp"], F32, (N, T), "logp"), _p(bufs["done"], F32, (N, T), "done"),
                            _p(bufs["flags"], U8, (N, T), "flags"), None, _p(last_val, F32, (N,), "last_val"),
                            _p(forced_act, I32, (N, T), "forced_act"), _p(noise, F64, (N, T, 2), "noise"),
                            _p(nan_count, I32, (1,), "nan_count"), None, None, _p(info, F32, (N, T, 10), "info"),
                            _p(heads, F32, (N, T, 6), "heads"), _stream()), "uav_rollout")
    if _t is not None:
        _t.record()


def greedy_episodes(env_state, n_env, cfg, params, hidden, steps, cur_obs, h, c, active, recs, noise=None, nan_count=None):
    N, T, D = n_env, steps, 6 + cfg.trend_k
    kind = 0 if hidden == 0 else 1
    if nan_count is None:
        nan_count = torch.zeros(1, dtype=I32, device=cur_obs.device)
    _t = KERNEL_TIMER.bracket("greedy")
    check(lib().uav_greedy_episodes(_h(cur_obs), _p(env_state, U8, name="env state"), N, C.byref(cfg), kind,
                                    _p(params, F32, name="params"), int(hidden), T, _p(cur_obs, F32, (N, D), "cur_obs"),
                                    _p(h, F32, (N, hidden), "h") if kind else None,
                                    _p(c, F32, (N, hidden), "c") if kind else None,
                                    _p(active, U8, (N,), "active"), _p(noise, F64, (N, T, 2), "noise"),
                                    _p(recs["act"], I32, (N, T), "act"), _p(recs["obs"], F32, (N, T, D), "obs"),
                                    _p(recs["pos"], F32, (N, T, 2), "pos"), _p(recs["flags"], U8, (N, T), "flags"),
                                    _p(nan_count, I32, (1,), "nan_count"), _stream()), "uav_greedy_episodes")
    if _t is not None:
        _t.record()


STOP_WIN_MAX = 16


def make_stop_rule(window=10, pos_std_max=2.0, conc_coef=2.0, conc_peak=100.0, conc_min=80.0):
    if not 1 <= int(window) <= STOP_WIN_MAX:
        raise RuntimeError(f"stop rule: window {window} outside 1 .. {STOP_WIN_MAX}")
    return _lib.StopRule(int(window), float(pos_std_max), float(conc_coef), float(conc_peak), float(conc_min))


def greedy_episodes_stop(env_state, n_env, cfg, params, hidden, steps, cur_obs, h, c, active, recs, rule, stop_win, stop_cnt,
                         noise=None, nan_count=None, rule_val=None):
    N, T, W, D = n_env, steps, int(rule.window), 6 + cfg.trend_k
    kind = 0 if hidden == 0 else 1
    if nan_count is None:
# ... 103 lines not shown
```

uav-wrf-les-ppo-lstm_amd/uavppo/policy.py:

```python
from __future__ import annotations

import math

import numpy as np
import torch

from . import ops


class _FlatPolicy:

    def _alloc(self, layout, device):
        self.layout = layout
        total = sum(int(np.prod(s)) for _, s in layout)
        self.flat = torch.zeros(total, dtype=torch.float32, device=device)
        self.grad = torch.zeros_like(self.flat)
        self.views, self.grad_views = {}, {}
        o = 0
        for name, shape in layout:
            n = int(np.prod(shape))
            self.views[name] = self.flat[o:o + n].view(shape)
            self.grad_views[name] = self.grad[o:o + n].view(shape)
            o += n

# ... 178 lines not shown
    def _interleaved_forward_ok(self, N, work, T=None):
        if not getattr(self, "use_stepper_forward", True) or self.num_layers < 2 or self.hidden != 256:
            return False
        sp = getattr(self, "_steppers", None)
        if sp is None or sp[0].N != N or ops.lstm_bwd_caps(self.device, self.obs_dim, 256) == 0:
            return False
        return all(work.get(f"y{l}") is not None and work[f"y{l}"].shape[0] == N and work.get(f"stash{l}") is not None
                   and work[f"stash{l}"].shape[0] == N
                   and (T is None or (work[f"y{l}"].shape[1] == T and work[f"stash{l}"].shape[1] == T))
                   for l in range(self.num_layers))

    def steppers(self, N, device):
        if getattr(self, "_steppers", None) is None or self._steppers[0].N != N:
            self._steppers = [ops.LstmStepper(N, self.obs_dim if l == 0 else self.hidden, self.hidden, device)
                              for l in range(self.num_layers)]
        return self._steppers

    def begin_steps(self, h, c):
        v = self.views
        for l, sp in enumerate(self.steppers(h.shape[1], h.device)):
            sp.begin(v[f"lstm.weight_ih_l{l}"], v[f"lstm.weight_hh_l{l}"], v[f"lstm.bias_ih_l{l}"], v[f"lstm.bias_hh_l{l}"],
                     h[l], c[l])

    def step_at(self, obs_seq, t, work, heads_seq, keep=None):
        x = self.step_layers_at(obs_seq, t, work, keep=keep)
        v = self.views
        return ops.gemm_rows(x[:, t], v["head.weight"], v["head.bias"], heads_seq[:, t])

    def step_layers_at(self, obs_seq, t, work, keep=None):
        x = obs_seq
        for l, sp in enumerate(self._steppers):
            sp.step(x, t, work[f"y{l}"], work[f"stash{l}"], below=self._steppers[l - 1] if l > 0 and self.hidden == 256 else None,
                    keep=keep)
            x = work[f"y{l}"]
        return x

    def step(self, obs, h, c, keep=None, work=None):
        N = obs.shape[0]
        x = obs.view(N, 1, -1)
        k = None if keep is None else keep.view(N, 1)
        work = work if work is not None else {}
        v = self.views
        for l in range(self.num_layers):
            st = work.get(f"step_stash{l}")
            if st is None:
                st = work[f"step_stash{l}"] = torch.empty(N, 1, 6 * self.hidden, dtype=torch.float32, device=obs.device)
            y, hn, cn, _ = ops.lstm_fwd(x, k, h[l], c[l], v[f"lstm.weight_ih_l{l}"], v[f"lstm.weight_hh_l{l}"],
                                        v[f"lstm.bias_ih_l{l}"], v[f"lstm.bias_hh_l{l}"], stash=st)
            h[l].copy_(hn)
            c[l].copy_(cn)
            x = y
        return ops.gemm(x.view(N, self.hidden), v["head.weight"], trans_b=True, bias=v["head.bias"])

    def backward(self, dheads, work=None, dhead_bias=None):
        saved, keep, y_last = self._saved
        N, T, H = y_last.shape
        v, g = self.views, self.grad_views
        work = work or {}
        if dhead_bias is not None:
            if dhead_bias.data_ptr() != g["head.bias"].data_ptr():
                g["head.bias"].copy_(dhead_bias)
        else:
            ops.colsum(dheads, out=g["head.bias"])
        dy = None
        top_in = self.obs_dim if self.num_layers == 1 else self.hidden
        caps = ops.lstm_bwd_caps(dheads.device, top_in, self.hidden)
        fused_heads = bool(caps & 2)
        L = self.num_layers
        if L >= 2 and (caps & 4) and getattr(self, "use_stack_bwd", True):
            specs = []
            for l in reversed(range(L)):
                x, stash, y, h0 = saved[l]
                key = f"dgates{l}"
                dg_bytes = ops.lstm_dgates_bytes(N, T, H, dheads.device)
                if work.get(key) is None or work[key].numel() * 4 < dg_bytes:
                    work[key] = work["dgates"] if (l == L - 1 and work.get("dgates") is not None and work["dgates"].numel() * 4 >= dg_bytes) \
                        else ops.lstm_dgates(N, T, H, dheads.device)
                if l > 0 and (work.get(f"dx{l}") is None or work[f"dx{l}"].shape[0] != N):
                    work[f"dx{l}"] = torch.empty(N, T, H, dtype=torch.float32, device=dheads.device)
                specs.append({"stash": stash, "w_hh": v[f"lstm.weight_hh_l{l}"], "w_ih": v[f"lstm.weight_ih_l{l}"] if l > 0 else None,
                              "dgates": work[key], "dx": work[f"dx{l}"] if l > 0 else None})
            ops.lstm_bwd_stack(specs, keep, dheads=dheads.view(N, T, -1), w_head=v["head.weight"])
            for l in reversed(range(L)):
                x, stash, y, h0 = saved[l]
                top = (l == L - 1)
                ops.lstm_bwd(x, keep, stash, v[f"lstm.weight_ih_l{l}"], v[f"lstm.weight_hh_l{l}"], y, h0,
                             wgrad_dheads=dheads.view(N, T, -1) if top else None, dgates=work[f"dgates{l}"],
                             dw_ih=g[f"lstm.weight_ih_l{l}"], dw_hh=g[f"lstm.weight_hh_l{l}"], db=g[f"lstm.bias_ih_l{l}"],
                             dw_head=g["head.weight"] if top else None, want_dstate=False, bwd_done=True,
                             db_hh=g[f"lstm.bias_hh_l{l}"])
            self._saved = None
            return self.grad
        if not fused_heads:
            if work.get("dy") is None or work["dy"].shape[0] != N * T:
                work["dy"] = torch.empty(N * T, H, dtype=torch.float32, device=dheads.device)
            dy = ops.gemm(dheads, v["head.weight"], out=work["dy"]).view(N, T, H)
        for l in reversed(range(self.num_layers)):
            x, stash, y, h0 = saved[l]
            top = (l == self.num_layers - 1)
            use_dheads = top and fused_heads
            r = ops.lstm_bwd(x, keep, stash, v[f"lstm.weight_ih_l{l}"], v[f"lstm.weight_hh_l{l}"], y, h0,
                             dy=None if use_dheads else dy,
                             dheads=dheads.view(N, T, -1) if use_dheads else None,
                             w_head=v["head.weight"] if use_dheads else None,
                             wgrad_dheads=dheads.view(N, T, -1) if top else None,
                             need_dx=(l > 0), dgates=work.get("dgates"), dw_ih=g[f"lstm.weight_ih_l{l}"],
                             dw_hh=g[f"lstm.weight_hh_l{l}"], db=g[f"lstm.bias_ih_l{l}"],
                             dw_head=g["head.weight"] if top else None, want_dstate=False, db_hh=g[f"lstm.bias_hh_l{l}"])
            dy = r["dx"]
        self._saved = None
        return self.grad
```

uav-wrf-les-ppo-lstm_amd/uavppo/trainer.py:

```python
from __future__ import annotations


import numpy as np
import torch

from . import ops
from .dist_utils import (SUCC_CAP, abi_collectives, allreduce_adv_stats, allreduce_grad, allreduce_sum, collectives_on, env_shard, exchange_successes, pack_local_successes,
                         unpack_episode_successes)
from .curriculum import Curriculum
from .policy import LSTMActorCritic, MLPActorCritic

DEFAULTS = dict(gamma=0.99, lam=0.95, clip=0.2, ent_beta=0.01, lr=3e-5, epochs=5, max_grad_norm=0.5)
RANGE_LIMITS = (0.5 * 65504.0, 0.5 * 4096.0, 0.5 * 64.0)
MLP_RANGE_LIMITS = (0.5 * 2048.0, float("inf"), float("inf"))


_SIDE_STREAMS = {}


def _side_stream(device):
    device = torch.device(device)
    key = device.index if device.index is not None else torch.cuda.current_device()
    if key not in _SIDE_STREAMS:
        _SIDE_STREAMS[key] = torch.cuda.Stream(device=device)
    return _SIDE_STREAMS[key]


class _DeviceCurriculumView:

    def __init__(self, tr):
        self._tr = tr

    @property
    def current_radius(self):
        return self._tr.radius

    @property
    def explore_bonus(self):
        return self._tr.bonus

    @property
    def success_history(self):
        self._tr._sync_curriculum()
        return [None] * self._tr._hist_len


class VecPPOTrainer:
    def __init__(self, num_envs, horizon, policy="lstm", hidden=128, layers=1, variant="v2.0", device="cuda",
                 seed=1234, gae_mode="reference_exact", num_minibatches=1, bank=None, bank_sources=None,
                 rank=0, world_size=1, use_curriculum=True, trend_k=0, log_info=False, device_curriculum=None, **hp):
        self.hp = dict(DEFAULTS)
        self.hp.update(hp)
        self.N, self.T = int(num_envs), int(horizon)
        self.rank, self.world = int(rank), int(world_size)
        self._coll = self.world > 1 or collectives_on()
        self.device = torch.device(device)
        self.variant, self.seed = variant, int(seed)
        self.gae_mode = gae_mode
        self.num_minibatches = int(num_minibatches)
        if self.N % self.num_minibatches:
            raise ValueError("num_envs must be divisible by num_minibatches (minibatches are whole env sequences)")
        self.kind = policy
        self.trend_k = int(trend_k)
        self.obs_dim = D = 6 + self.trend_k
        if policy == "lstm":
            self.policy = LSTMActorCritic(D, hidden, layers, 5, self.device, seed=self.seed)
        elif policy == "mlp":
            self.policy = MLPActorCritic(D, 5, device=self.device, seed=self.seed)
        else:
            raise ValueError(policy)
        N, T, d = self.N, self.T, self.device
        f32 = dict(dtype=torch.float32, device=d)
        self.buf = {"obs": torch.zeros(N, T, D, **f32), "act": torch.zeros(N, T, dtype=torch.int32, device=d),
                    "rew": torch.zeros(N, T, **f32), "val": torch.zeros(N, T, **f32), "logp": torch.zeros(N, T, **f32),
                    "done": torch.zeros(N, T, **f32), "flags": torch.zeros(N, T, dtype=torch.uint8, device=d),
                    "keep": torch.ones(N, T, **f32)}
        self.info = torch.zeros(N, T, 10, **f32) if log_info else None
        self.adv = torch.zeros(N, T, **f32)
        self.adv_n = torch.zeros(N, T, **f32)
        self.ret = torch.zeros(N, T, **f32)
        self.last_val = torch.zeros(N, **f32) if gae_mode == "standard" else None
        self.stats3 = torch.zeros(3, dtype=torch.float64, device=d)
        self.loss_sums = torch.zeros(4, dtype=torch.float64, device=d)
        self.gnorm = torch.zeros(1, **f32)
        self.dhead_bias = torch.zeros(6, **f32)
        self.nan_count = torch.zeros(1, dtype=torch.int32, device=d)
        P = self.policy.num_params()
        self.exp_avg = torch.zeros(P, **f32)
        self.exp_avg_sq = torch.zeros(P, **f32)
        self.opt_step = 0
        self.iteration = 0
        self.fused_mlp = policy == "mlp" and D == 6
        self.reuse_rollout_forward = True
        self.use_stepper = True
        self.use_fused_tail = True
        self._rollout_forward_valid = False
        self.record = False
        self.record_grads = False
        self.log = []
        self.grad_log = []
        self.ranges = torch.zeros(3, **f32)
        self._ranges_host = torch.zeros(4, 3, dtype=torch.float32).pin_memory()
        self._ranges_evs = [torch.cuda.Event() for _ in range(4)]
        self._pmax_queue = []
        self._pmax_next = 0
        self._buffers_own = False
        self.arith = "fp16x3"
        self.range_events = 0
        init_mode = ops.Context.get(self.device).initial_arith
        self.force_arith = None if init_mode == "fp16x3" else init_mode
        self._flat_version = -1
        self.env_state = torch.zeros(ops.env_state_bytes(N), dtype=torch.uint8, device=d)
        self.cur_obs = torch.zeros(N, D, **f32)
        self.bank = None if bank is None else torch.as_tensor(bank, dtype=torch.float64).to(d).contiguous()
        self.bank_sources = None if bank_sources is None else torch.as_tensor(bank_sources, dtype=torch.float64).to(d).contiguous()
        self.device_curriculum = bool(use_curriculum) if device_curriculum is None else bool(device_curriculum and use_curriculum)
        self._radius, self._bonus = 50.0, 0.6
        self._episodes_done = self._successes_done = 0
        self._hist_len = 0
        self.last_success_bits = None
        if self.device_curriculum:
            self._curr = ops.curriculum_state(self.device, self._radius, self._bonus)
            self._curr_host = torch.zeros(4, self._curr.numel(), dtype=torch.uint8).pin_memory()
            self._curr_evs = [torch.cuda.Event() for _ in range(4)]
            self._curr_queue, self._curr_next = [], 0
            self.last_mirror_slot = 0
            self._curr_done_ev = torch.cuda.Event()
            self._curr_pending = False
            self.curriculum = _DeviceCurriculumView(self)
        else:
            self._curr = None
            self.curriculum = Curriculum() if use_curriculum else None
        self._side = _side_stream(self.device) if use_curriculum else None
        self._succ_host = (torch.zeros(self.world, 4 + SUCC_CAP + 1, dtype=torch.uint8).pin_memory() if use_curriculum else None)
        self._succ_ev = torch.cuda.Event()
        self._pack_ev = torch.cuda.Event()
        self._roll_ev = torch.cuda.Event()
        self._gather_ev = torch.cuda.Event()
        self._succ_pending = False
        self._succ_exchanged = False
        self._succ_msg = None
        self.side_stream_curriculum = True
        if policy == "lstm":
            L, H = layers, hidden
            self._state = torch.zeros(2, L, N, H, **f32)
            self._state0 = torch.zeros(2, L, N, H, **f32)
            self.h, self.c = self._state[0], self._state[1]
            self.h0, self.c0 = self._state0[0], self._state0[1]
            nb = N // self.num_minibatches
            self.work = {"dgates": ops.lstm_dgates(nb, T, H, self.device), "heads": torch.empty(nb, T, 6, **f32)}
            for l in range(L):
                self.work[f"stash{l}"] = torch.empty(nb, T, 6 * H, **f32)
                self.work[f"y{l}"] = torch.empty(nb, T, H, **f32)
        else:
            nb = N // self.num_minibatches
            self.work = {"stash": None}
            self._mlp_tmp = {"rew": torch.zeros(N, **f32), "done": torch.zeros(N, **f32),
                             "flags": torch.zeros(N, dtype=torch.uint8, device=d), "stash": None}
        if policy == "lstm":
            self.dhead_bias = self.policy.grad_views["head.bias"]
        self.dheads = torch.empty((N // self.num_minibatches) * T, 6, **f32)
        self.reset()

    def env_cfg(self):
        return ops.make_env_cfg(self.variant, self._radius, self._bonus, self.seed, self.bank, self.bank_sources,
                                env_offset=env_shard(self.rank, self.N)[0], n_env_total=self.world * self.N,
                                trend_k=self.trend_k, curriculum=self._curr)

    def _sync_curriculum(self):
        if not self.device_curriculum:
            return
        if self._succ_pending and not self._succ_exchanged and not self._coll:
            self._exchange_successes()
        if self._curr_pending:
            self._curr_done_ev.synchronize()
        d = ops.curriculum_read(self._curr.cpu().numpy())
        if d["overflow"]:
            raise RuntimeError(f"device curriculum: a rank ended more than {SUCC_CAP} episodes in one rollout (message capacity)")
        self._radius = d["radius"]
        self._bonus = np.float64(d["bonus"]) if d["bonus_is_f64"] else d["bonus"]
        self._episodes_done, self._successes_done, self._hist_len = d["episodes"], d["successes"], d["hist_len"]

    def sync_curriculum(self):
        self._sync_curriculum()

    def _poll_curriculum_mirror(self):
        latest = None
        while self._curr_queue and self._curr_evs[self._curr_queue[0]].query():
            latest = self._curr_queue.pop(0)
        if latest is not None:
            d = ops.curriculum_read(self._curr_host[latest].numpy())
            if d["overflow"]:
                raise RuntimeError(f"device curriculum: a rank ended more than {SUCC_CAP} episodes in one rollout (message capacity)")
            self._radius = d["radius"]
            self._bonus = np.float64(d["bonus"]) if d["bonus_is_f64"] else d["bonus"]
            self._episodes_done, self._successes_done, self._hist_len = d["episodes"], d["successes"], d["hist_len"]

    def rollout_radius(self, k=None):
        if not self.device_curriculum:
            return self._rollout_radius
        k = self.last_mirror_slot if k is None else k
        self._curr_evs[k].synchronize()
        return ops.curriculum_read(self._curr_host[k].numpy())["radius"]

    def episodes_before_rollout(self, k):
        if not self.device_curriculum:
            return self._episodes_done
        self._curr_evs[k].synchronize()
        d = ops.curriculum_read(self._curr_host[k].numpy())
        if d["overflow"]:
            raise RuntimeError(f"device curriculum: a rank ended more than {SUCC_CAP} episodes in one rollout (message capacity)")
        return d["episodes"]

# ... 69 lines not shown
    def poll_param_range(self):
        latest = None
        while self._pmax_queue and self._ranges_evs[self._pmax_queue[0]].query():
            latest = self._pmax_queue.pop(0)
        if latest is not None and self._guarded():
            self._decide([float(self._ranges_host[latest, 0]), 0.0, 0.0])

    def check_ranges(self):
        if not self._guarded():
            return self.arith
        if self.force_arith is not None:
            self.arith = self.force_arith
        if not self._buffers_own:
            self._pmax_queue.clear()
            ops.absmax(self.policy.flat, out=self.ranges[0:1])
            if self.kind == "lstm":
                ops.absmax(self.buf["obs"], out=self.ranges[1:2])
                ops.absmax(self.h0, out=self.ranges[2:3])
            self._flat_version = self.policy.flat._version
            self._decide(self.ranges.tolist())
        else:
            self._measure_params()
        ops.set_lstm_arith(self.arith, self.device)
        return self.arith

    def reset(self):
        ops.env_reset(self.env_state, self.N, self.env_cfg(), self.cur_obs)
        if self.kind == "lstm":
            self.h.zero_()
            self.c.zero_()

    def collect(self, forced_act=None, noise=None):
        self._rollout_forward_valid = False
        self._rollout_radius = self._radius
        if self._succ_pending:
            torch.cuda.current_stream().wait_event(self._pack_ev)
        if self.device_curriculum:
            if self._succ_pending and not self._succ_exchanged:
                self._exchange_successes()
            if self._curr_pending:
                torch.cuda.current_stream().wait_event(self._curr_done_ev)
        if self._guarded():
            self.poll_param_range()
            self._measure_params()
            if self.force_arith is not None:
                self.arith = self.force_arith
            ops.set_lstm_arith(self.arith, self.device)
            self._buffers_own = True
        wide = self._guarded() and self.arith != "fp16x3"
        if self.kind == "lstm" and (self.policy.num_layers != 1 or self.policy.hidden not in (64, 128) or wide):
            self._state0.copy_(self._state)
            self._collect_stepwise_lstm(forced_act, noise)
        elif self.kind == "lstm":
            self._state0.copy_(self._state)
            reuse = self.reuse_rollout_forward and self.num_minibatches == 1
            ops.rollout_lstm(self.env_state, self.N, self.env_cfg(), self.policy.flat, self.policy.hidden, self.T,
                             self.iteration, self.cur_obs, self.h[0], self.c[0], self.buf, last_val=self.last_val,
                             forced_act=forced_act, noise=noise, nan_count=self.nan_count,
                             stash=self.work["stash0"] if reuse else None, y=self.work["y0"] if reuse else None,
                             info=self.info, heads=self.work["heads"] if reuse else None)
            self._rollout_forward_valid = reuse
        elif self.fused_mlp:
            ops.rollout_mlp(self.env_state, self.N, self.env_cfg(), self.policy.flat, self.T, self.iteration, self.cur_obs,
                            self.buf, last_val=self.last_val, forced_act=forced_act, noise=noise, nan_count=self.nan_count,
                            info=self.info)
        else:
            self._collect_stepwise(forced_act, noise)
        if self.curriculum is not None and self.side_stream_curriculum:
            self._roll_ev.record()
            with torch.cuda.stream(self._side):
                self._side.wait_event(self._roll_ev)
                self._succ_msg = pack_local_successes(self.buf["flags"])
                self._pack_ev.record(self._side)
            self._succ_pending = True
            self._succ_exchanged = False
            if not self._coll:
                self._exchange_successes()

    def _exchange_successes(self):
        msgs_main = None
        if abi_collectives() and self._coll:
            main = torch.cuda.current_stream()
            main.wait_event(self._pack_ev)
            msgs_main = exchange_successes(self._succ_msg)
            self._gather_ev.record(main)
        with torch.cuda.stream(self._side):
            if msgs_main is not None:
                self._side.wait_event(self._gather_ev)
                msgs = msgs_main
            else:
                msgs = exchange_successes(self._succ_msg)
            if tuple(msgs.shape) != tuple(self._succ_host.shape):
                raise RuntimeError(f"success exchange returned {tuple(msgs.shape)}, expected {tuple(self._succ_host.shape)}: "
                                   "is torch.distributed initialised for world_size > 1?")
            if self.device_curriculum:
                k = self._curr_next
                self._curr_next = (k + 1) % len(self._curr_evs)
                if k in self._curr_queue:
                    self._curr_queue.remove(k)
                self._curr_host[k].copy_(self._curr, non_blocking=True)
                self._curr_evs[k].record(self._side)
                self._curr_queue.append(k)
                self.last_mirror_slot = k
                ops.curriculum_update(self._curr, msgs, SUCC_CAP)
                self._curr_done_ev.record(self._side)
                self._curr_pending = True
            else:
                self._succ_host.copy_(msgs, non_blocking=True)
                self._succ_ev.record(self._side)
        self._succ_exchanged = True

    def _collect_stepwise_lstm(self, forced_act=None, noise=None):
        b = self.buf
# ... 62 lines not shown
            else:
                b["rew"][:, t] = st["rew"]
                b["done"][:, t] = st["done"]
                b["flags"][:, t] = st["flags"]
                torch.sub(1.0, st["done"], out=st["keep"])
        if stepper:
            for l, sp in enumerate(self.policy.steppers(self.N, self.device)):
                self.h[l].copy_(sp.hn)
                self.c[l].copy_(sp.cn)
            self._rollout_forward_valid = self.reuse_rollout_forward
        self.h.mul_(st["keep"][None, :, None])
        self.c.mul_(st["keep"][None, :, None])
        if self.last_val is not None:
            hh, cc = self.h.clone(), self.c.clone()
            self.last_val.copy_(self.policy.step(self.cur_obs, hh, cc, None, st["work"])[:, 5])

    def _collect_stepwise(self, forced_act=None, noise=None):
        b, tmp = self.buf, self._mlp_tmp
        cfg = self.env_cfg()
        for t in range(self.T):
            heads = self.policy.heads(self.cur_obs, stash=tmp["stash"])
            tmp["stash"] = self.policy._stash
            logits = heads[:, :5].contiguous()
            fa = None if forced_act is None else forced_act[:, t].contiguous()
            act, logp, _, _ = ops.policy_sample(logits, seed=self.seed, counter=t, iteration=self.iteration,
                                                index_offset=env_shard(self.rank, self.N)[0], forced_act=fa,
                                                nan_count=self.nan_count)
            b["obs"][:, t] = self.cur_obs
            b["act"][:, t] = act
            b["val"][:, t] = heads[:, 5]
            b["logp"][:, t] = logp
            nz = None if noise is None else noise[:, t].contiguous()
            if self.info is not None and "info" not in tmp:
                tmp["info"] = torch.zeros(self.N, 5, dtype=torch.float32, device=self.device)
                tmp["term"] = torch.zeros(self.N, self.obs_dim, dtype=torch.float32, device=self.device)
                tmp["src"] = torch.zeros(self.N, 2, dtype=torch.float64, device=self.device)
            if self.info is not None:
                ops.env_peek(self.env_state, self.N, source=tmp["src"])
            ops.env_step(self.env_state, self.N, cfg, act, self.cur_obs, tmp["rew"], tmp["done"], tmp["flags"], noise=nz,
                         info=tmp.get("info"), term_obs=tmp.get("term"))
            if self.info is not None:
                self.info[:, t, :5] = tmp["info"]
                self.info[:, t, 5] = tmp["term"][:, 2]
                self.info[:, t, 6:8] = tmp["term"][:, :2] * 500.0
                self.info[:, t, 8:10] = tmp["src"]
            b["rew"][:, t] = tmp["rew"]
            b["done"][:, t] = tmp["done"]
            b["flags"][:, t] = tmp["flags"]
        if self.last_val is not None:
            self.last_val.copy_(self.policy.heads(self.cur_obs, stash=tmp["stash"])[:, 5])

    def compute_advantages(self):
        b, hp = self.buf, self.hp
        ops.gae(b["rew"], b["val"], b["done"], hp["gamma"], hp["lam"], self.gae_mode, last_val=self.last_val, out=self.adv)
        ops.adv_stats(self.adv, out=self.stats3)
        allreduce_adv_stats(self.stats3)
        ops.adv_normalise(self.adv, b["val"], self.stats3, self.adv_n, self.ret)

    def update(self):
        if self.check_ranges() != "fp16x3":
            self._rollout_forward_valid = False
        self.compute_advantages()
        if self._succ_pending and not self._succ_exchanged:
            self._exchange_successes()
        b, hp = self.buf, self.hp
        N, T, M = self.N, self.T, self.num_minibatches
        nb = N // M
        inv_n = 1.0 / float(nb * T * self.world)
        for _ in range(hp["epochs"]):
            for m in range(M):
                sl = slice(m * nb, (m + 1) * nb)
                args = (b["act"][sl].reshape(-1), b["logp"][sl].reshape(-1), self.adv_n[sl].reshape(-1),
                        self.ret[sl].reshape(-1), b["val"][sl].reshape(-1), inv_n, hp["clip"], hp["ent_beta"],
                        self.loss_sums, self.dheads, self.dhead_bias)
                if self.kind == "lstm":
                    if self._rollout_forward_valid:
                        L = self.policy.num_layers
                        self.policy.adopt_forward(b["obs"], b["keep"], self.h0, [self.work[f"stash{l}"] for l in range(L)],
                                                  [self.work[f"y{l}"] for l in range(L)])
                        heads = self.work["heads"]
                        self._rollout_forward_valid = False
                    else:
                        heads = self.policy.heads(b["obs"][sl], b["keep"][sl],
                                                  self.h0[:, sl].contiguous() if M > 1 else self.h0,
                                                  self.c0[:, sl].contiguous() if M > 1 else self.c0, self.work)
                    ops.ppo_loss_heads(heads.view(nb * T, -1), *args)
                elif self.fused_mlp:
                    grad = ops.mlp_ppo_grad(self.policy.flat, b["obs"][sl].reshape(nb * T, self.obs_dim), *args[:8],
                                            self.loss_sums, self.policy.grad)
                else:
                    if self.work["stash"] is None:
                        self.work["stash"] = torch.empty(nb * T * (2 * 256 + 2 * 128 + 2), dtype=torch.float32, device=self.device)
                    heads = self.policy.heads(b["obs"][sl].reshape(nb * T, self.obs_dim), stash=self.work["stash"])
                    ops.ppo_loss_heads(heads, *args)
                if self.kind == "lstm":
                    grad = self.policy.backward(self.dheads, self.work, self.dhead_bias)
                elif not self.fused_mlp:
                    grad = self.policy.backward(self.dheads)
                allreduce_grad(grad)
                if self.record_grads:
                    self.grad_log.append((grad.clone(), self.policy.flat.clone()))
                self.opt_step += 1
                ops.clip_adam(self.policy.flat, grad, self.exp_avg, self.exp_avg_sq, self.opt_step, hp["lr"],
                              max_norm=hp["max_grad_norm"], gnorm_out=self.gnorm, pmax_out=self.ranges[0:1])
                if self.record:
                    self.log.append((self.loss_sums.clone(), self.gnorm.clone()))
        if self._guarded():
            if len(self._pmax_queue) == 4:
                self._ranges_evs[self._pmax_queue[0]].synchronize()
                self.poll_param_range()
            k = self._pmax_next
            self._pmax_next = (k + 1) % 4
            self._ranges_host[k].copy_(self.ranges, non_blocking=True)
            self._ranges_evs[k].record()
            self._pmax_queue.append(k)
            self._buffers_own = False
        return self.loss_sums

    def update_curriculum(self):
        if self.curriculum is None:
            return
        if self.device_curriculum:
            if not self._succ_pending:
                self._roll_ev.record()
                with torch.cuda.stream(self._side):
                    self._side.wait_event(self._roll_ev)
                    self._succ_msg = pack_local_successes(self.buf["flags"])
                    self._pack_ev.record(self._side)
                self._succ_pending, self._succ_exchanged = True, False
            if not self._succ_exchanged:
                self._exchange_successes()
            self._succ_pending = False
            self._poll_curriculum_mirror()
            return
        if not self._succ_pending:
            msgs = exchange_successes(pack_local_successes(self.buf["flags"]))
            if tuple(msgs.shape) != tuple(self._succ_host.shape):
                raise RuntimeError(f"success exchange returned {tuple(msgs.shape)}, expected {tuple(self._succ_host.shape)}: "
                                   "is torch.distributed initialised for world_size > 1?")
            self._succ_host.copy_(msgs, non_blocking=True)
            self._succ_ev.record()
        elif not self._succ_exchanged:
            self._exchange_successes()
        self._succ_ev.synchronize()
        self._succ_pending = False
        bits = unpack_episode_successes(self._succ_host.numpy(), self.buf["flags"])
        self._episodes_done += int(bits.size)
        self._successes_done += int(bits.sum())
        self.last_success_bits = bits
        self.curriculum.update_many(bits)
        self._radius, self._bonus = self.curriculum.current_radius, self.curriculum.explore_bonus

    def time_rollouts(self, event_pairs):
        self._iter_events = list(event_pairs)[::-1]

    def train_iteration(self):
        ev = self._iter_events.pop() if getattr(self, "_iter_events", None) else None
# ... 21 lines not shown
```

Before: 74.09 million.

## Fuse GAE with advantage stats, presum grad norm in wgrad, snapshot LSTM state in rollout

The GAE scan kernel now emits per-block sum and sum-of-squares partials, and the normalise kernel reduces them itself. This removes the separate adv_stats pass. The LSTM weight-gradient kernel writes gradient squared-norm partials and zeroes pmax, so Adam skips its own norm-reduction pass and only adds the head-bias remainder. The rollout also writes h0/c0 snapshots directly instead of needing a separate state copy. The aim is fewer kernel launches and fewer gradient/advantage reads, at the cost of extra per-block reductions and duplicated final stat reductions in every normalise block.

```diff
diff --git a/include/uavppo.h b/include/uavppo.h
--- a/include/uavppo.h
+++ b/include/uavppo.h
@@ -48,6 +48,9 @@
 int uav_adv_stats(uav_ctx* ctx, const float* adv, int64_t n, double* stats3, uav_stream stream);
 int uav_adv_normalise(uav_ctx* ctx, const float* adv, const float* val, int64_t n,
                       const double* stats3, float* adv_out, float* ret_out, uav_stream stream);
+int uav_gae_normalise(uav_ctx* ctx, const float* rew, const float* val, const float* done, const float* last_val, int n_env,
+                      int horizon, float gamma, float lam, int mode, float* adv, double* stats3, float* adv_out,
+                      float* ret_out, uav_stream stream);
 
 int uav_pack_success_bits(uav_ctx* ctx, const uint8_t* flags, int64_t n, int cap, uint8_t* msg, uav_stream stream);
 
@@ -81,6 +84,10 @@
 int uav_clip_adamw(uav_ctx* ctx, float* param, const float* grad, float* exp_avg, float* exp_avg_sq, int64_t n,
                    int64_t step, float lr, float beta1, float beta2, float eps, float weight_decay, float max_norm,
                    float* gnorm_out, uav_stream stream);
+int uav_clip_adam_presummed(uav_ctx* ctx, float* param, const float* grad, float* exp_avg, float* exp_avg_sq, int64_t n,
+                            int64_t step, float lr, float beta1, float beta2, float eps, float max_norm, float* gnorm_out,
+                            float* pmax_out, const double* sumsq_partial, int n_partial, int64_t rest_offset, int64_t rest_n,
+                            uav_stream stream);
 int uav_smooth_l1(uav_ctx* ctx, const float* pred, const float* target, int64_t n, float beta, double* loss_mean,
                   float* dpred, uav_stream stream);
 int uav_mse_bce(uav_ctx* ctx, const float* out, const float* target, int64_t n, double* loss_mean, float* dout,
@@ -168,6 +175,11 @@
                    const float* stash, const float* dgates, const float* w_ih, const float* dheads,
                    int n_heads, int N, int T, int I, int H, float* dw_ih, float* dw_hh, float* db, float* db_hh,
                    float* dw_head, float* dx, uav_stream stream);
+int uav_lstm_wgrad_sumsq(uav_ctx* ctx, const float* x, const float* keep, const float* h0, const float* y,
+                         const float* stash, const float* dgates, const float* w_ih, const float* dheads,
+                         int n_heads, int N, int T, int I, int H, float* dw_ih, float* dw_hh, float* db, float* db_hh,
+                         float* dw_head, float* dx, double* sumsq_partial, float* pmax_zero, uav_stream stream);
+int uav_lstm_wgrad_sumsq_count(int H);
 
 typedef struct uav_env_cfg {
     int32_t variant;
@@ -210,6 +222,13 @@
                 float* val, float* logp, float* done, uint8_t* flags, float* keep, float* last_val,
                 const int32_t* forced_act, const double* noise, int32_t* nan_count,
                 float* stash, float* y_out, float* info, float* heads, uav_stream stream);
+int uav_rollout_snapshot(uav_ctx* ctx, void* env_state, int n_env, const uav_env_cfg* cfg ,
+                         int policy_kind, const float* params, int hidden, int horizon, uint64_t iter,
+                         float* cur_obs, float* h, float* c, float* obs, int32_t* act, float* rew,
+                         float* val, float* logp, float* done, uint8_t* flags, float* keep, float* last_val,
+                         const int32_t* forced_act, const double* noise, int32_t* nan_count,
+                         float* stash, float* y_out, float* info, float* heads, float* h0_out, float* c0_out,
+                         uav_stream stream);
 
 int uav_greedy_episodes(uav_ctx* ctx, void* env_state, int n_env, const uav_env_cfg* cfg , int policy_kind,
                         const float* params, int hidden, int steps, float* cur_obs, float* h, float* c, uint8_t* active,
diff --git a/uav-wrf-les-ppo-lstm_amd/csrc/adam.hip b/uav-wrf-les-ppo-lstm_amd/csrc/adam.hip
--- a/uav-wrf-les-ppo-lstm_amd/csrc/adam.hip
+++ b/uav-wrf-les-ppo-lstm_amd/csrc/adam.hip
@@ -20,12 +20,17 @@
                                                    const double* __restrict__ partial, int nb, float max_norm,
                                                    float* __restrict__ gnorm_out, float b1, float b2,
                                                    float step_size, float sqrt_bc2, float eps, float decay,
-                                                   unsigned* __restrict__ pmax_bits) {
+                                                   unsigned* __restrict__ pmax_bits, const float* __restrict__ rest,
+                                                   int rest_n) {
 #pragma clang fp contract(off)
     __shared__ double sm[4];
     __shared__ float coef_s;
     double q = 0.0;
     for (int i = threadIdx.x; i < nb; i += 256) q += partial[i];
+    for (int i = threadIdx.x; i < rest_n; i += 256) {
+        const double r = (double)rest[i];
+        q += r * r;
+    }
     q = block256_sum(q, sm);
     if (threadIdx.x == 0) {
         const float norm = (float)sqrt(q);
@@ -97,7 +102,29 @@
     int ab = (int)((n + 255) / 256);
     if (ab > 2048) ab = 2048;
     hipLaunchKernelGGL(adam_kernel, dim3(ab), dim3(256), 0, as_stream(stream), param, grad, exp_avg, exp_avg_sq, n,
-                       partial, nb, max_norm, gnorm_out, beta1, beta2, step_size, sqrt_bc2, eps, 1.0f - lr * weight_decay, pmax_bits);
+                       partial, nb, max_norm, gnorm_out, beta1, beta2, step_size, sqrt_bc2, eps, 1.0f - lr * weight_decay, pmax_bits,
+                       (const float*)nullptr, 0);
+    UAV_LAUNCH_CHECK();
+    return 0;
+}
+
+extern "C" int uav_clip_adam_presummed(uav_ctx* ctx, float* param, const float* grad, float* exp_avg, float* exp_avg_sq, int64_t n,
+                                       int64_t step, float lr, float beta1, float beta2, float eps, float max_norm,
+                                       float* gnorm_out, float* pmax_out, const double* sumsq_partial, int n_partial,
+                                       int64_t rest_offset, int64_t rest_n, uav_stream stream) {
+    UAV_REQUIRE(ctx && param && grad && exp_avg && exp_avg_sq && n > 0 && step >= 1, "uav_clip_adam_presummed: bad argument");
+    UAV_REQUIRE(sumsq_partial && n_partial > 0, "uav_clip_adam_presummed: no partial sums");
+    UAV_REQUIRE(rest_n >= 0 && rest_n <= 65536 && rest_offset >= 0 && rest_offset + rest_n <= n,
+                "uav_clip_adam_presummed: rest range [%lld, +%lld) of %lld", (long long)rest_offset, (long long)rest_n, (long long)n);
+    const double bc1 = 1.0 - pow((double)beta1, (double)step);
+    const double bc2 = 1.0 - pow((double)beta2, (double)step);
+    const float step_size = (float)((double)lr / bc1);
+    const float sqrt_bc2 = (float)sqrt(bc2);
+    int ab = (int)((n + 255) / 256);
+    if (ab > 2048) ab = 2048;
+    hipLaunchKernelGGL(adam_kernel, dim3(ab), dim3(256), 0, as_stream(stream), param, grad, exp_avg, exp_avg_sq, n,
+                       sumsq_partial, n_partial, max_norm, gnorm_out, beta1, beta2, step_size, sqrt_bc2, eps, 1.0f,
+                       reinterpret_cast<unsigned*>(pmax_out), grad + rest_offset, (int)rest_n);
     UAV_LAUNCH_CHECK();
     return 0;
 }
diff --git a/uav-wrf-les-ppo-lstm_amd/csrc/gae.hip b/uav-wrf-les-ppo-lstm_amd/csrc/gae.hip
--- a/uav-wrf-les-ppo-lstm_amd/csrc/gae.hip
+++ b/uav-wrf-les-ppo-lstm_amd/csrc/gae.hip
@@ -5,11 +5,14 @@
                                                        const float* __restrict__ done,
                                                        const float* __restrict__ last_val, int n_env,
                                                        int T, float gamma, float gl, int mode,
-                                                       float* __restrict__ adv) {
+                                                       float* __restrict__ adv,
+                                                       double* __restrict__ stat_partial) {
 #pragma clang fp contract(off)
+    __shared__ double sm[4];
     const int lane = threadIdx.x & 63;
     const int env = blockIdx.x * 4 + (threadIdx.x >> 6);
-    if (env >= n_env) return;
+    double ssum = 0.0, ssq = 0.0;
+    if (env < n_env) {
     const size_t row = (size_t)env * T;
     const int nchunk = (T + 63) >> 6;
     float carry = 0.f;
@@ -47,10 +50,25 @@
             }
         }
         const float A = b + a * carry;
-        if (in) adv[row + t] = A;
+        if (in) {
+            adv[row + t] = A;
+            ssum += (double)A;
+            ssq += (double)A * (double)A;
+        }
         carry = __shfl(A, 0, 64);
         v_right = __shfl(v, 0, 64);
         d_right = __shfl(d, 0, 64);
+    }
+    }
+    if (stat_partial) {
+        ssum = block256_sum(ssum, sm);
+        ssq = block256_sum(ssq, sm);
+        if (threadIdx.x == 0) {
+            const int rows = min(4, n_env - (int)blockIdx.x * 4);
+            stat_partial[3 * blockIdx.x] = ssum;
+            stat_partial[3 * blockIdx.x + 1] = ssq;
+            stat_partial[3 * blockIdx.x + 2] = (double)rows * (double)T;
+        }
     }
 }
 
@@ -94,11 +112,35 @@
                                                             const float* __restrict__ val, int64_t n,
                                                             const double* __restrict__ stats3,
                                                             float* __restrict__ adv_out,
-                                                            float* __restrict__ ret_out) {
+                                                            float* __restrict__ ret_out,
+                                                            const double* __restrict__ stat_partial, int npart,
+                                                            double* __restrict__ stats3_out) {
 #pragma clang fp contract(off)
-    const double cnt = stats3[2];
-    const double mean_d = stats3[0] / cnt;
-    const double var = (stats3[1] - cnt * mean_d * mean_d) / (cnt - 1.0);
+    double st0, st1, st2;
+    if (stat_partial) {
+        __shared__ double sm[4];
+        __shared__ double fin[3];
+        double s = 0.0, q = 0.0, c = 0.0;
+        for (int i = threadIdx.x; i < npart; i += 256) {
+            s += stat_partial[3 * i];
+            q += stat_partial[3 * i + 1];
+            c += stat_partial[3 * i + 2];
+        }
+        s = block256_sum(s, sm);
+        q = block256_sum(q, sm);
+        c = block256_sum(c, sm);
+        if (threadIdx.x == 0) {
+            fin[0] = s; fin[1] = q; fin[2] = c;
+            if (blockIdx.x == 0) { stats3_out[0] = s; stats3_out[1] = q; stats3_out[2] = c; }
+        }
+        __syncthreads();
+        st0 = fin[0]; st1 = fin[1]; st2 = fin[2];
+    } else {
+        st0 = stats3[0]; st1 = stats3[1]; st2 = stats3[2];
+    }
+    const double cnt = st2;
+    const double mean_d = st0 / cnt;
+    const double var = (st1 - cnt * mean_d * mean_d) / (cnt - 1.0);
     const float mean = (float)mean_d;
     float sd = (float)sqrt(var > 0.0 ? var : (var == var ? 0.0 : var));
     if (sd < 1e-6f || sd != sd) sd = 1.0f;
@@ -296,7 +338,28 @@
     const float gl = (float)((double)gamma * (double)lam);
     const int blocks = (n_env + 3) / 4;
     hipLaunchKernelGGL(gae_scan_kernel, dim3(blocks), dim3(256), 0, as_stream(stream), rew, val, done,
-                       last_val, n_env, horizon, gamma, gl, mode, adv);
+                       last_val, n_env, horizon, gamma, gl, mode, adv, (double*)nullptr);
+    UAV_LAUNCH_CHECK();
+    return 0;
+}
+
+int uav_gae_normalise(uav_ctx* ctx, const float* rew, const float* val, const float* done, const float* last_val, int n_env,
+                      int horizon, float gamma, float lam, int mode, float* adv, double* stats3, float* adv_out, float* ret_out,
+                      uav_stream stream) {
+    UAV_REQUIRE(ctx && rew && val && done && adv && stats3 && adv_out && ret_out, "uav_gae_normalise: NULL argument");
+    UAV_REQUIRE(n_env > 0 && horizon > 0, "uav_gae_normalise: n_env=%d horizon=%d", n_env, horizon);
+    UAV_REQUIRE(mode == UAV_GAE_REFERENCE_EXACT || mode == UAV_GAE_STANDARD, "uav_gae_normalise: mode %d", mode);
+    const float gl = (float)((double)gamma * (double)lam);
+    const int blocks = (n_env + 3) / 4;
+    UAV_REQUIRE((size_t)blocks * 3 * sizeof(double) <= ctx->ws_bytes, "uav_gae_normalise: workspace too small for %d block partials", blocks);
+    double* partial = (double*)ctx->ws;
+    hipLaunchKernelGGL(gae_scan_kernel, dim3(blocks), dim3(256), 0, as_stream(stream), rew, val, done,
+                       last_val, n_env, horizon, gamma, gl, mode, adv, partial);
+    const int64_t n = (int64_t)n_env * horizon;
+    int nb = (int)((n + 1023) / 1024);
+    if (nb > 2048) nb = 2048;
+    hipLaunchKernelGGL(adv_normalise_kernel, dim3(nb), dim3(256), 0, as_stream(stream), adv, val, n, (const double*)nullptr,
+                       adv_out, ret_out, (const double*)partial, blocks, stats3);
     UAV_LAUNCH_CHECK();
     return 0;
 }
@@ -318,7 +381,7 @@
     int nb = (int)((n + 1023) / 1024);
     if (nb > 2048) nb = 2048;
     hipLaunchKernelGGL(adv_normalise_kernel, dim3(nb), dim3(256), 0, as_stream(stream), adv, val, n, stats3,
-                       adv_out, ret_out);
+                       adv_out, ret_out, (const double*)nullptr, 0, (double*)nullptr);
     UAV_LAUNCH_CHECK();
     return 0;
 }
diff --git a/uav-wrf-les-ppo-lstm_amd/csrc/lstm.hip b/uav-wrf-les-ppo-lstm_amd/csrc/lstm.hip
--- a/uav-wrf-les-ppo-lstm_amd/csrc/lstm.hip
+++ b/uav-wrf-les-ppo-lstm_amd/csrc/lstm.hip
@@ -36,7 +36,9 @@
                       const float* w_head, int n_heads, int N, int T, hipStream_t st);
 int lstm_wgrad_fused(uav_ctx* ctx, const float* dgates, const float* y, const float* keep, const float* h0,
                      const float* x, int I, const float* dheads, int NH, int N, int T, int H,
-                     float* dw_ih, float* dw_hh, float* db, float* db_hh, float* dw_head, hipStream_t st);
+                     float* dw_ih, float* dw_hh, float* db, float* db_hh, float* dw_head, double* sumsq_partial,
+                     unsigned* pmax_zero, hipStream_t st);
+int lstm_wgrad_sumsq_count(int H);
 
 constexpr int MT = 16;
 constexpr int TC = 32;
@@ -1059,11 +1061,13 @@
                         as_stream(stream));
 }
 
-int uav_lstm_wgrad(uav_ctx* ctx, const float* x, const float* keep, const float* h0, const float* y,
-                   const float* stash, const float* dgates, const float* w_ih, const float* dheads, int n_heads, int N,
-                   int T, int I, int H, float* dw_ih, float* dw_hh, float* db, float* db_hh, float* dw_head, float* dx,
-                   uav_stream stream) {
+static int lstm_wgrad_impl(uav_ctx* ctx, const float* x, const float* keep, const float* h0, const float* y,
+                           const float* stash, const float* dgates, const float* w_ih, const float* dheads, int n_heads, int N,
+                           int T, int I, int H, float* dw_ih, float* dw_hh, float* db, float* db_hh, float* dw_head, float* dx,
+                           double* sumsq_partial, float* pmax_zero, uav_stream stream) {
     UAV_REQUIRE(ctx && x && h0 && y && dgates && w_ih && dw_ih && dw_hh && db, "uav_lstm_wgrad: NULL argument");
+    UAV_REQUIRE(!sumsq_partial || (I <= 6 && (H == 64 || H == 128)),
+                "uav_lstm_wgrad_sumsq: I=%d H=%d is not on the fused weight-gradient kernels (I <= 6, H = 64 / 128)", I, H);
     uav_enter(ctx);
     UAV_REQUIRE(N > 0 && T > 0 && I > 0 && H > 0, "uav_lstm_wgrad: N=%d T=%d I=%d H=%d", N, T, I, H);
     UAV_REQUIRE(!dheads || (dw_head && n_heads > 0 && n_heads <= 8), "uav_lstm_wgrad: dheads needs dw_head, 1..8 heads");
@@ -1072,7 +1076,7 @@
     int rc;
     if (I <= 6 && (H == 64 || H == 128)) {
         if ((rc = lstm_wgrad_fused(ctx, dgates, y, keep, h0, x, I, dheads, n_heads, N, T, H, dw_ih, dw_hh, db, db_hh,
-                                   dw_head, st))) return rc;
+                                   dw_head, sumsq_partial, reinterpret_cast<unsigned*>(pmax_zero), st))) return rc;
     } else {
         UAV_REQUIRE(stash, "uav_lstm_wgrad: stash is required when I > 6");
         const size_t red_floats = (size_t)1024 * 9 * 4 * H + 64;
@@ -1142,4 +1146,23 @@
     return 0;
 }
 
-}
+int uav_lstm_wgrad(uav_ctx* ctx, const float* x, const float* keep, const float* h0, const float* y,
+                   const float* stash, const float* dgates, const float* w_ih, const float* dheads, int n_heads, int N,
+                   int T, int I, int H, float* dw_ih, float* dw_hh, float* db, float* db_hh, float* dw_head, float* dx,
+                   uav_stream stream) {
+    return lstm_wgrad_impl(ctx, x, keep, h0, y, stash, dgates, w_ih, dheads, n_heads, N, T, I, H, dw_ih, dw_hh, db, db_hh, dw_head,
+                           dx, nullptr, nullptr, stream);
+}
+
+int uav_lstm_wgrad_sumsq_count(int H) { return lstm_wgrad_sumsq_count(H); }
+
+int uav_lstm_wgrad_sumsq(uav_ctx* ctx, const float* x, const float* keep, const float* h0, const float* y,
+                         const float* stash, const float* dgates, const float* w_ih, const float* dheads, int n_heads, int N,
+                         int T, int I, int H, float* dw_ih, float* dw_hh, float* db, float* db_hh, float* dw_head, float* dx,
+                         double* sumsq_partial, float* pmax_zero, uav_stream stream) {
+    UAV_REQUIRE(sumsq_partial, "uav_lstm_wgrad_sumsq: NULL sumsq_partial");
+    return lstm_wgrad_impl(ctx, x, keep, h0, y, stash, dgates, w_ih, dheads, n_heads, N, T, I, H, dw_ih, dw_hh, db, db_hh, dw_head,
+                           dx, sumsq_partial, pmax_zero, stream);
+}
+
+}
diff --git a/uav-wrf-les-ppo-lstm_amd/csrc/rollout.hip b/uav-wrf-les-ppo-lstm_amd/csrc/rollout.hip
--- a/uav-wrf-les-ppo-lstm_amd/csrc/rollout.hip
+++ b/uav-wrf-les-ppo-lstm_amd/csrc/rollout.hip
@@ -57,11 +57,12 @@
     float* info;
     float* heads;
     float* stash; float* y;
-    uint8_t* active; float* pos;
+    union { uint8_t* active; float* h0_out; };
+    union { float* pos; float* c0_out; };
     float* stop_win; int32_t* stop_cnt; float* rule_val; StopRule rule;
 };
 
-template <int H, int NA, bool GREEDY = false, bool STOP = false, bool TREND = false>
+template <int H, int NA, bool GREEDY = false, bool STOP = false, bool TREND = false, bool SNAP = false>
 __global__ __launch_bounds__(H * 4) void rollout_lstm_kernel(EnvParams P_arg, EnvBlob blob, int N, int T,
                                                                         uint64_t iter, const float* __restrict__ params,
                                                                         RolloutBufs B) {
@@ -83,6 +84,7 @@
     __shared__ __attribute__((aligned(16))) f32x4 acc0[4 * 64];
     __shared__ double env_tab[ENV_LDS_TABLE_DOUBLES];
     static_assert(!STOP || GREEDY, "rollout_lstm_kernel: the stop rule belongs to the greedy episodes");
+    static_assert(!SNAP || (!GREEDY && !TREND), "rollout_lstm_kernel: the snapshot belongs to the plain training rollout");
     constexpr size_t STOP_LDS = STOP ? RMT * 2 * STOP_WIN_MAX * sizeof(float) : 0;
     static_assert(G::LDS + sizeof(xbuf) + sizeof(kbuf) + sizeof(hd) + sizeof(vis) + sizeof(es_s) + sizeof(trs) + sizeof(acc0) +
                       sizeof(env_tab) + STOP_LDS <= 160 * 1024, "rollout_lstm_kernel: LDS over 160 KB per workgroup");
@@ -118,6 +120,13 @@
     const bool env_lane = is_env_wave && lane < RMT && my_env < N;
     unsigned short* myvis = vis + (lane & 15) * NVIS;
 
+    if constexpr (SNAP)
+        if (live) {
+            const size_t so = (size_t)(n0 + j) * H + uo;
+            *reinterpret_cast<float4*>(B.h0_out + so) = *reinterpret_cast<const float4*>(B.h + so);
+            *reinterpret_cast<float4*>(B.c0_out + so) = *reinterpret_cast<const float4*>(B.c + so);
+        }
+
     f16x8 wb[4][NS][2];
     f16x8* const w0f = reinterpret_cast<f16x8*>(w0p) + lane;
 #pragma unroll
@@ -182,6 +191,7 @@
         put_h(h_in);
         if constexpr (TREND && !GREEDY)
             if (B.stash && live) *reinterpret_cast<float4*>(B.stash + (size_t)(n0 + j) * T * (6 * H) + 5 * H + uo) = hv;
+
     }
     bool ran = true;
     if (is_env_wave && lane < RMT) {
@@ -589,12 +599,12 @@
     }
 }
 
-template <int H, bool GREEDY = false, bool STOP = false, bool TREND = false>
+template <int H, bool GREEDY = false, bool STOP = false, bool TREND = false, bool SNAP = false>
 static int launch_rollout(const EnvParams& P, EnvBlob blob, int N, int T, uint64_t iter, const float* params,
                           const RolloutBufs& B, hipStream_t st) {
     const dim3 grid((N + RMT - 1) / RMT), block(H * 4);
-    UAV_CHECK_HIP(uav_dyn_lds(reinterpret_cast<const void*>(&rollout_lstm_kernel<H, 5, GREEDY, STOP, TREND>), (int)RGeom<H>::LDS));
-    hipLaunchKernelGGL((rollout_lstm_kernel<H, 5, GREEDY, STOP, TREND>), grid, block, RGeom<H>::LDS, st, P, blob, N, T, iter, params, B);
+    UAV_CHECK_HIP(uav_dyn_lds(reinterpret_cast<const void*>(&rollout_lstm_kernel<H, 5, GREEDY, STOP, TREND, SNAP>), (int)RGeom<H>::LDS));
+    hipLaunchKernelGGL((rollout_lstm_kernel<H, 5, GREEDY, STOP, TREND, SNAP>), grid, block, RGeom<H>::LDS, st, P, blob, N, T, iter, params, B);
     UAV_LAUNCH_CHECK();
     return 0;
 }
@@ -707,37 +717,67 @@
     return 0;
 }
 
+static int rollout_impl(uav_ctx* ctx, void* env_state, int n_env, const uav_env_cfg* cfg, int policy_kind,
+                           const float* params, int hidden, int horizon, uint64_t iter, float* cur_obs, float* h,
+                           float* c, float* obs, int32_t* act, float* rew, float* val, float* logp, float* done,
+                           uint8_t* flags, float* keep, float* last_val, const int32_t* forced_act,
+                           const double* noise, int32_t* nan_count, float* stash, float* y_out, float* info,
+                           float* heads, float* h0_out, float* c0_out, uav_stream stream) {
+    UAV_REQUIRE(ctx && env_state && params && cur_obs && obs && act && rew && val && logp && done && flags && nan_count,
+                "uav_rollout: NULL argument");
+    UAV_REQUIRE(n_env > 0 && horizon > 0, "uav_rollout: n_env=%d horizon=%d", n_env, horizon);
+    UAV_REQUIRE(policy_kind == 0 || policy_kind == 1, "uav_rollout: policy_kind %d (0 = MLP, 1 = LSTM)", policy_kind);
+    UAV_REQUIRE(policy_kind == 1 || (!h0_out && !c0_out), "uav_rollout_snapshot: the MLP policy has no recurrent state");
+    if (policy_kind == 0) {
+        UAV_REQUIRE(!stash && !y_out, "uav_rollout: stash / y_out belong to the LSTM policy");
+        return launch_rollout_mlp(ctx, env_state, n_env, cfg, params, horizon, iter, cur_obs, obs, act, rew, val, logp, done,
+                                  flags, last_val, forced_act, noise, nan_count, info, heads, as_stream(stream));
+    }
+    UAV_REQUIRE(h && c && keep, "uav_rollout: LSTM policy needs h, c, keep");
+    UAV_REQUIRE((h0_out == nullptr) == (c0_out == nullptr), "uav_rollout_snapshot: h0_out and c0_out go together");
+    UAV_REQUIRE(!h0_out || (h0_out != h && c0_out != c), "uav_rollout_snapshot: the snapshot must not alias h / c");
+    EnvParams P;
+    int rc = env_params_from_cfg(ctx, cfg, n_env, P);
+    if (rc) return rc;
+    UAV_REQUIRE((stash == nullptr) == (y_out == nullptr), "uav_rollout: stash and y_out go together");
+    UAV_REQUIRE(!stash || (int64_t)n_env * horizon * 6 * hidden < (1ll << 32), "uav_rollout: stash rows exceed 32-bit offsets");
+    RolloutBufs B{cur_obs, h, c, obs, act, rew, val, logp, done, flags, keep, last_val, forced_act, noise, nan_count, info, heads, stash, y_out};
+    B.h0_out = h0_out;
+    B.c0_out = c0_out;
+    EnvBlob blob = env_blob_view(env_state, n_env);
+    const bool trend = P.trend_k != 0;
+    UAV_REQUIRE(!trend || !h0_out, "uav_rollout_snapshot: trend_k=%d: the trend-observation kernels write no snapshot", P.trend_k);
+    switch (hidden) {
+        case 64: return trend ? launch_rollout<64, false, false, true>(P, blob, n_env, horizon, iter, params, B, as_stream(stream))
+                     : h0_out ? launch_rollout<64, false, false, false, true>(P, blob, n_env, horizon, iter, params, B, as_stream(stream))
+                              : launch_rollout<64>(P, blob, n_env, horizon, iter, params, B, as_stream(stream));
+        case 128: return trend ? launch_rollout<128, false, false, true>(P, blob, n_env, horizon, iter, params, B, as_stream(stream))
+                      : h0_out ? launch_rollout<128, false, false, false, true>(P, blob, n_env, horizon, iter, params, B, as_stream(stream))
+                               : launch_rollout<128>(P, blob, n_env, horizon, iter, params, B, as_stream(stream));
+    }
+    UAV_REQUIRE(false, "uav_rollout: hidden=%d unsupported (64, 128)", hidden);
+}
+
 extern "C" int uav_rollout(uav_ctx* ctx, void* env_state, int n_env, const uav_env_cfg* cfg, int policy_kind,
                            const float* params, int hidden, int horizon, uint64_t iter, float* cur_obs, float* h,
                            float* c, float* obs, int32_t* act, float* rew, float* val, float* logp, float* done,
                            uint8_t* flags, float* keep, float* last_val, const int32_t* forced_act,
                            const double* noise, int32_t* nan_count, float* stash, float* y_out, float* info,
                            float* heads, uav_stream stream) {
-    UAV_REQUIRE(ctx && env_state && params && cur_obs && obs && act && rew && val && logp && done && flags && nan_count,
-                "uav_rollout: NULL argument");
-    UAV_REQUIRE(n_env > 0 && horizon > 0, "uav_rollout: n_env=%d horizon=%d", n_env, horizon);
-    UAV_REQUIRE(policy_kind == 0 || policy_kind == 1, "uav_rollout: policy_kind %d (0 = MLP, 1 = LSTM)", policy_kind);
-    if (policy_kind == 0) {
-        UAV_REQUIRE(!stash && !y_out, "uav_rollout: stash / y_out belong to the LSTM policy");
-        return launch_rollout_mlp(ctx, env_state, n_env, cfg, params, horizon, iter, cur_obs, obs, act, rew, val, logp, done,
-                                  flags, last_val, forced_act, noise, nan_count, info, heads, as_stream(stream));
-    }
-    UAV_REQUIRE(h && c && keep, "uav_rollout: LSTM policy needs h, c, keep");
-    EnvParams P;
-    int rc = env_params_from_cfg(ctx, cfg, n_env, P);
-    if (rc) return rc;
-    UAV_REQUIRE((stash == nullptr) == (y_out == nullptr), "uav_rollout: stash and y_out go together");
-    UAV_REQUIRE(!stash || (int64_t)n_env * horizon * 6 * hidden < (1ll << 32), "uav_rollout: stash rows exceed 32-bit offsets");
-    RolloutBufs B{cur_obs, h, c, obs, act, rew, val, logp, done, flags, keep, last_val, forced_act, noise, nan_count, info, heads, stash, y_out};
-    EnvBlob blob = env_blob_view(env_state, n_env);
-    const bool trend = P.trend_k != 0;
-    switch (hidden) {
-        case 64: return trend ? launch_rollout<64, false, false, true>(P, blob, n_env, horizon, iter, params, B, as_stream(stream))
-                              : launch_rollout<64>(P, blob, n_env, horizon, iter, params, B, as_stream(stream));
-        case 128: return trend ? launch_rollout<128, false, false, true>(P, blob, n_env, horizon, iter, params, B, as_stream(stream))
-                               : launch_rollout<128>(P, blob, n_env, horizon, iter, params, B, as_stream(stream));
-    }
-    UAV_REQUIRE(false, "uav_rollout: hidden=%d unsupported (64, 128)", hidden);
+    return rollout_impl(ctx, env_state, n_env, cfg, policy_kind, params, hidden, horizon, iter, cur_obs, h, c, obs, act, rew, val,
+                        logp, done, flags, keep, last_val, forced_act, noise, nan_count, stash, y_out, info, heads, nullptr, nullptr,
+                        stream);
+}
+
+extern "C" int uav_rollout_snapshot(uav_ctx* ctx, void* env_state, int n_env, const uav_env_cfg* cfg, int policy_kind,
+                                    const float* params, int hidden, int horizon, uint64_t iter, float* cur_obs, float* h,
+                                    float* c, float* obs, int32_t* act, float* rew, float* val, float* logp, float* done,
+                                    uint8_t* flags, float* keep, float* last_val, const int32_t* forced_act,
+                                    const double* noise, int32_t* nan_count, float* stash, float* y_out, float* info,
+                                    float* heads, float* h0_out, float* c0_out, uav_stream stream) {
+    return rollout_impl(ctx, env_state, n_env, cfg, policy_kind, params, hidden, horizon, iter, cur_obs, h, c, obs, act, rew, val,
+                        logp, done, flags, keep, last_val, forced_act, noise, nan_count, stash, y_out, info, heads, h0_out, c0_out,
+                        stream);
 }
 
 static int greedy_episodes_impl(const char* who, uav_ctx* ctx, void* env_state, int n_env, const uav_env_cfg* cfg, int policy_kind,
@@ -769,7 +809,7 @@
                     : launch_greedy_mlp(P, env_state, n_env, params, steps, cur_obs, active, noise, act, obs, pos, flags, nan_count, st);
     UAV_REQUIRE(h && c, "%s: LSTM policy needs h, c", who);
     RolloutBufs B{cur_obs, h, c, obs, act, nullptr, nullptr, nullptr, nullptr, flags, nullptr, nullptr, nullptr, noise, nan_count,
-                  nullptr, nullptr, nullptr, nullptr, active, pos, stop_win, stop_cnt, rule_val, R};
+                  nullptr, nullptr, nullptr, nullptr, {active}, {pos}, stop_win, stop_cnt, rule_val, R};
     EnvBlob blob = env_blob_view(env_state, n_env);
 #define LAUNCH_G(H_)                                                                                      \
     (P.trend_k ? (rule ? launch_rollout<H_, true, true, true>(P, blob, n_env, steps, 0, params, B, st)        \
diff --git a/uav-wrf-les-ppo-lstm_amd/csrc/wgrad.hip b/uav-wrf-les-ppo-lstm_amd/csrc/wgrad.hip
--- a/uav-wrf-les-ppo-lstm_amd/csrc/wgrad.hip
+++ b/uav-wrf-les-ppo-lstm_amd/csrc/wgrad.hip
@@ -499,29 +499,40 @@
 __global__ __launch_bounds__(256) void wgrad_reduce_kernel(const float* __restrict__ slabs, int nb, int I, int NH,
                                                            float* __restrict__ dw_ih, float* __restrict__ dw_hh,
                                                            float* __restrict__ db, float* __restrict__ db_hh,
-                                                           float* __restrict__ dw_head) {
+                                                           float* __restrict__ dw_head, double* __restrict__ sumsq_partial,
+                                                           unsigned* __restrict__ pmax_zero) {
     using G = WG<H>;
+    if (pmax_zero && blockIdx.x == 0 && threadIdx.x == 0) *pmax_zero = 0u;
     const size_t o = (size_t)blockIdx.x * 256 + threadIdx.x;
-    if (o >= G::SLAB) return;
-    float p8[8] = {0.f, 0.f, 0.f, 0.f, 0.f, 0.f, 0.f, 0.f};
-    int b = 0;
-    for (; b + 8 <= nb; b += 8)
-#pragma unroll
-        for (int k = 0; k < 8; ++k) p8[k] += slabs[(size_t)(b + k) * G::SLAB + o];
-    for (; b < nb; ++b) p8[0] += slabs[(size_t)b * G::SLAB + o];
-    const float s = ((p8[0] + p8[1]) + (p8[2] + p8[3])) + ((p8[4] + p8[5]) + (p8[6] + p8[7]));
-    const size_t gsz = (size_t)4 * H * G::NC;
-    if (o < gsz) {
-        const int m = (int)(o / G::NC), c = (int)(o % G::NC);
-        if (c < H) dw_hh[(size_t)m * H + c] = s;
-        else if (c - H < I) dw_ih[(size_t)m * I + (c - H)] = s;
-        else if (c - H == 6) {
-            db[m] = s;
-            if (db_hh) db_hh[m] = s;
-        }
-    } else if (dw_head) {
-        const int a = (int)((o - gsz) / H), uu = (int)((o - gsz) % H);
-        if (a < NH) dw_head[(size_t)a * H + uu] = s;
+    double sq = 0.0;
+    if (o < G::SLAB) {
+        float p8[8] = {0.f, 0.f, 0.f, 0.f, 0.f, 0.f, 0.f, 0.f};
+        int b = 0;
+        for (; b + 8 <= nb; b += 8)
+#pragma unroll
+            for (int k = 0; k < 8; ++k) p8[k] += slabs[(size_t)(b + k) * G::SLAB + o];
+        for (; b < nb; ++b) p8[0] += slabs[(size_t)b * G::SLAB + o];
+        const float s = ((p8[0] + p8[1]) + (p8[2] + p8[3])) + ((p8[4] + p8[5]) + (p8[6] + p8[7]));
+        const double s2 = (double)s * (double)s;
+        const size_t gsz = (size_t)4 * H * G::NC;
+        if (o < gsz) {
+            const int m = (int)(o / G::NC), c = (int)(o % G::NC);
+            if (c < H) { dw_hh[(size_t)m * H + c] = s; sq = s2; }
+            else if (c - H < I) { dw_ih[(size_t)m * I + (c - H)] = s; sq = s2; }
+            else if (c - H == 6) {
+                db[m] = s;
+                sq = s2;
+                if (db_hh) { db_hh[m] = s; sq = s2 + s2; }
+            }
+        } else if (dw_head) {
+            const int a = (int)((o - gsz) / H), uu = (int)((o - gsz) % H);
+            if (a < NH) { dw_head[(size_t)a * H + uu] = s; sq = s2; }
+        }
+    }
+    if (sumsq_partial) {
+        __shared__ double sm[4];
+        sq = block256_sum(sq, sm);
+        if (threadIdx.x == 0) sumsq_partial[blockIdx.x] = sq;
     }
 }
 
@@ -544,7 +555,8 @@
 template <int H>
 static int launch_wgrad(uav_ctx* ctx, const float* dgates, const float* y, const float* keep, const float* h0,
                         const float* x, int I, const float* dheads, int NH, int N, int T,
-                        float* dw_ih, float* dw_hh, float* db, float* db_hh, float* dw_head, hipStream_t st) {
+                        float* dw_ih, float* dw_hh, float* db, float* db_hh, float* dw_head, double* sumsq_partial,
+                        unsigned* pmax_zero, hipStream_t st) {
     using G = WG<H>;
     const int64_t NTr = (int64_t)N * T;
     int nb = ctx->num_cu;
@@ -567,7 +579,7 @@
                                : launch_wgrad_split<WgF16x3, H>(dgates, y, keep, h0, x, I, dheads, NH, N, T, nbx, (int)rpx, slabs, st);
             if (rc) return rc;
             hipLaunchKernelGGL((wgrad_reduce_kernel<H>), dim3((unsigned)((G::SLAB + 255) / 256)), dim3(256), 0, st, slabs,
-                               nbx, I, NH, dw_ih, dw_hh, db, db_hh, dw_head);
+                               nbx, I, NH, dw_ih, dw_hh, db, db_hh, dw_head, sumsq_partial, pmax_zero);
             UAV_LAUNCH_CHECK();
             return 0;
         }
@@ -576,18 +588,29 @@
     hipLaunchKernelGGL((lstm_wgrad_kernel<H>), dim3(nb), dim3(H * 4), G::LDS, st, dgates, y, keep, h0, x, I, dheads, NH, N,
                        T, rpb, slabs);
     hipLaunchKernelGGL((wgrad_reduce_kernel<H>), dim3((unsigned)((G::SLAB + 255) / 256)), dim3(256), 0, st, slabs, nb, I,
-                       NH, dw_ih, dw_hh, db, db_hh, dw_head);
+                       NH, dw_ih, dw_hh, db, db_hh, dw_head, sumsq_partial, pmax_zero);
     UAV_LAUNCH_CHECK();
     return 0;
 }
 
 int lstm_wgrad_fused(uav_ctx* ctx, const float* dgates, const float* y, const float* keep, const float* h0,
                      const float* x, int I, const float* dheads, int NH, int N, int T, int H,
-                     float* dw_ih, float* dw_hh, float* db, float* db_hh, float* dw_head, hipStream_t st) {
+                     float* dw_ih, float* dw_hh, float* db, float* db_hh, float* dw_head, double* sumsq_partial,
+                     unsigned* pmax_zero, hipStream_t st) {
     switch (H) {
-        case 64: return launch_wgrad<64>(ctx, dgates, y, keep, h0, x, I, dheads, NH, N, T, dw_ih, dw_hh, db, db_hh, dw_head, st);
-        case 128: return launch_wgrad<128>(ctx, dgates, y, keep, h0, x, I, dheads, NH, N, T, dw_ih, dw_hh, db, db_hh, dw_head, st);
+        case 64: return launch_wgrad<64>(ctx, dgates, y, keep, h0, x, I, dheads, NH, N, T, dw_ih, dw_hh, db, db_hh, dw_head,
+                                         sumsq_partial, pmax_zero, st);
+        case 128: return launch_wgrad<128>(ctx, dgates, y, keep, h0, x, I, dheads, NH, N, T, dw_ih, dw_hh, db, db_hh, dw_head,
+                                           sumsq_partial, pmax_zero, st);
     }
     uav_set_error("lstm_wgrad_fused: H=%d unsupported", H);
     return 2;
 }
+
+int lstm_wgrad_sumsq_count(int H) {
+    switch (H) {
+        case 64: return (int)((WG<64>::SLAB + 255) / 256);
+        case 128: return (int)((WG<128>::SLAB + 255) / 256);
+    }
+    return 0;
+}
diff --git a/uav-wrf-les-ppo-lstm_amd/uavppo/_lib.py b/uav-wrf-les-ppo-lstm_amd/uavppo/_lib.py
--- a/uav-wrf-les-ppo-lstm_amd/uavppo/_lib.py
+++ b/uav-wrf-les-ppo-lstm_amd/uavppo/_lib.py
@@ -44,6 +44,7 @@
     "uav_set_debug_flags": (I32, [P, C.c_uint]),
     "uav_absmax": (I32, [P, P, I64, P, P]),
     "uav_gae": (I32, [P, P, P, P, P, I32, I32, F32, F32, I32, P, P]),
+    "uav_gae_normalise": (I32, [P, P, P, P, P, I32, I32, F32, F32, I32, P, P, P, P, P]),
     "uav_adv_stats": (I32, [P, P, I64, P, P]),
     "uav_adv_normalise": (I32, [P, P, P, I64, P, P, P, P]),
     "uav_pack_success_bits": (I32, [P, P, I64, I32, P, P]),
@@ -58,6 +59,7 @@
     "uav_store_transition": (I32, [P, I32, I32, I32, P, P, P, P, P, P, P, P, P]),
     "uav_rollout_tail": (I32, [P, P, I32, P, P, I64, I32, P, P, I32, P, I64, I32, I32, U64, U64, I64, P, P, P, P, P, P, P, P, P, P, P, P, P, P, P]),
     "uav_clip_adam": (I32, [P, P, P, P, P, I64, I64, F32, F32, F32, F32, F32, P, P, P]),
+    "uav_clip_adam_presummed": (I32, [P, P, P, P, P, I64, I64, F32, F32, F32, F32, F32, P, P, P, I32, I64, I64, P]),
     "uav_clip_adamw": (I32, [P, P, P, P, P, I64, I64, F32, F32, F32, F32, F32, F32, P, P]),
     "uav_smooth_l1": (I32, [P, P, P, I64, F32, P, P, P]),
     "uav_mse_bce": (I32, [P, P, P, I64, P, P, P]),
@@ -85,6 +87,8 @@
     "uav_lstm_dgates_f32": (I32, [P, P, I32, I32, I32, P, P]),
     "uav_lstm_bwd_stack": (I32, [P, I32, P, P, P, P, I32, I32, I32, I32, P]),
     "uav_lstm_wgrad": (I32, [P, P, P, P, P, P, P, P, P, I32, I32, I32, I32, I32, P, P, P, P, P, P, P]),
+    "uav_lstm_wgrad_sumsq": (I32, [P, P, P, P, P, P, P, P, P, I32, I32, I32, I32, I32, P, P, P, P, P, P, P, P, P]),
+    "uav_lstm_wgrad_sumsq_count": (I32, [I32]),
     "uav_env_state_bytes": (SZ, [I32]),
     "uav_env_reset": (I32, [P, P, I32, C.POINTER(EnvCfg), P, P]),
     "uav_env_step": (I32, [P, P, I32, C.POINTER(EnvCfg), P, P, P, P, P, P, P, P, P, P]),
@@ -92,6 +96,8 @@
     "uav_env_materialise": (I32, [P, P, I32, C.POINTER(EnvCfg), I32, P, P]),
     "uav_rollout": (I32, [P, P, I32, C.POINTER(EnvCfg), I32, P, I32, I32, U64, P, P, P, P, P, P, P, P, P, P,
                           P, P, P, P, P, P, P, P, P, P]),
+    "uav_rollout_snapshot": (I32, [P, P, I32, C.POINTER(EnvCfg), I32, P, I32, I32, U64, P, P, P, P, P, P, P, P, P, P,
+                                   P, P, P, P, P, P, P, P, P, P, P, P]),
     "uav_greedy_episodes": (I32, [P, P, I32, C.POINTER(EnvCfg), I32, P, I32, I32, P, P, P, P, P, P, P, P, P, P, P]),
     "uav_greedy_episodes_stop": (I32, [P, P, I32, C.POINTER(EnvCfg), I32, P, I32, I32, P, P, P, P, P, P, P, P, P, P,
                                        C.POINTER(StopRule), P, P, P, P]),
diff --git a/uav-wrf-les-ppo-lstm_amd/uavppo/ops.py b/uav-wrf-les-ppo-lstm_amd/uavppo/ops.py
--- a/uav-wrf-les-ppo-lstm_amd/uavppo/ops.py
+++ b/uav-wrf-les-ppo-lstm_amd/uavppo/ops.py
@@ -101,6 +101,21 @@
                         float(gamma), float(lam), GAE_MODES[mode], _p(adv, F32, (n, T), "adv"), _stream()),
           "uav_gae")
     return adv
+
+
+def gae_normalise(rew, val, done, gamma, lam, mode="reference_exact", last_val=None, adv=None, stats3=None, adv_out=None,
+                  ret_out=None):
+    n, T = rew.shape
+    adv = torch.empty_like(rew) if adv is None else adv
+    stats3 = torch.empty(3, dtype=F64, device=rew.device) if stats3 is None else stats3
+    adv_out = torch.empty_like(rew) if adv_out is None else adv_out
+    ret_out = torch.empty_like(rew) if ret_out is None else ret_out
+    check(lib().uav_gae_normalise(_h(rew), _p(rew, F32, (n, T), "rew"), _p(val, F32, (n, T), "val"),
+                                  _p(done, F32, (n, T), "done"), _p(last_val, F32, (n,), "last_val"), n, T,
+                                  float(gamma), float(lam), GAE_MODES[mode], _p(adv, F32, (n, T), "adv"),
+                                  _p(stats3, F64, (3,), "stats3"), _p(adv_out, F32, (n, T), "adv_out"),
+                                  _p(ret_out, F32, (n, T), "ret_out"), _stream()), "uav_gae_normalise")
+    return adv, stats3, adv_out, ret_out
 
 
 def adv_stats(adv, out=None):
@@ -359,6 +374,34 @@
                               float(lr), float(beta1), float(beta2), float(eps), float(max_norm),
                               _p(gnorm_out, F32, (1,), "gnorm_out"), _p(pmax_out, F32, (1,), "pmax_out"), _stream()),
           "uav_clip_adam")
+
+
+def clip_adam_presummed(param, grad, exp_avg, exp_avg_sq, step, lr, sumsq_partial, rest_offset=0, rest_n=0, beta1=0.9,
+                        beta2=0.999, eps=1e-8, max_norm=0.5, gnorm_out=None, pmax_out=None):
+    n = param.numel()
+    for t, nm in ((grad, "grad"), (exp_avg, "exp_avg"), (exp_avg_sq, "exp_avg_sq")):
+        if t.numel() != n:
+            raise RuntimeError(f"clip_adam_presummed: {nm} has {t.numel()} elements, param has {n}")
+    check(lib().uav_clip_adam_presummed(_h(param), _p(param, F32, name="param"), _p(grad, F32, name="grad"),
+                                        _p(exp_avg, F32, name="exp_avg"), _p(exp_avg_sq, F32, name="exp_avg_sq"), n, int(step),
+                                        float(lr), float(beta1), float(beta2), float(eps), float(max_norm),
+                                        _p(gnorm_out, F32, (1,), "gnorm_out"), _p(pmax_out, F32, (1,), "pmax_out"),
+                                        _p(sumsq_partial, F64, name="sumsq_partial"), sumsq_partial.numel(), int(rest_offset),
+                                        int(rest_n), _stream()), "uav_clip_adam_presummed")
+
+
+def lstm_wgrad_sumsq_count(H):
+    return int(lib().uav_lstm_wgrad_sumsq_count(int(H)))
+
+
+def _wgrad_call(sumsq_partial, H, args, pmax_zero=None):
+    if sumsq_partial is None:
+        check(lib().uav_lstm_wgrad(*args, _stream()), "uav_lstm_wgrad")
+    else:
+        cnt = lstm_wgrad_sumsq_count(H)
+        check(lib().uav_lstm_wgrad_sumsq(*args, _p(sumsq_partial, F64, (cnt,) if cnt else None, "sumsq_partial"),
+                                         _p(pmax_zero, F32, (1,), "pmax_zero"), _stream()),
+              "uav_lstm_wgrad_sumsq")
 
 
 def gemm_rows(a, b_t, bias, out):
@@ -593,23 +636,26 @@
     return out
 
 
-def lstm_wgrad(x, keep, h0, y, stash, dgates, w_ih, dheads=None):
+def lstm_wgrad(x, keep, h0, y, stash, dgates, w_ih, dheads=None, out=None, sumsq_partial=None, pmax_zero=None):
     N, T, I = x.shape
     H = y.shape[-1]
     dev = x.device
     nh = 0 if dheads is None else dheads.shape[-1]
-    dw_ih = torch.empty(4 * H, I, dtype=F32, device=dev)
-    dw_hh = torch.empty(4 * H, H, dtype=F32, device=dev)
-    db = torch.empty(4 * H, dtype=F32, device=dev)
-    dw_head = torch.empty(nh, H, dtype=F32, device=dev) if nh else None
-    check(lib().uav_lstm_wgrad(_h(x), _p(x, F32, (N, T, I), "x"), _p(keep, F32, (N, T), "keep"), _p(h0, F32, (N, H), "h0"),
-                               _p(y, F32, (N, T, H), "y"), _p(stash, F32, (N, T, 6 * H), "stash"),
-                               _pdg(dgates, N, T, H), _p(w_ih, F32, (4 * H, I), "w_ih"),
-                               _p(dheads, F32, (N, T, nh), "dheads"), nh, N, T, I, H,
-                               _p(dw_ih, F32, (4 * H, I), "dw_ih"), _p(dw_hh, F32, (4 * H, H), "dw_hh"),
-                               _p(db, F32, (4 * H,), "db"), None, _p(dw_head, F32, (nh, H), "dw_head"), _p(None), _stream()),
-          "uav_lstm_wgrad")
-    return {"dw_ih": dw_ih, "dw_hh": dw_hh, "db": db, "dw_head": dw_head}
+    out = out or {}
+    dw_ih = out["dw_ih"] if "dw_ih" in out else torch.empty(4 * H, I, dtype=F32, device=dev)
+    dw_hh = out["dw_hh"] if "dw_hh" in out else torch.empty(4 * H, H, dtype=F32, device=dev)
+    db = out["db"] if "db" in out else torch.empty(4 * H, dtype=F32, device=dev)
+    db_hh = out.get("db_hh")
+    dw_head = (out["dw_head"] if "dw_head" in out else torch.empty(nh, H, dtype=F32, device=dev)) if nh else None
+    _wgrad_call(sumsq_partial, H,
+                (_h(x), _p(x, F32, (N, T, I), "x"), _p(keep, F32, (N, T), "keep"), _p(h0, F32, (N, H), "h0"),
+                 _p(y, F32, (N, T, H), "y"), _p(stash, F32, (N, T, 6 * H), "stash"),
+                 _pdg(dgates, N, T, H), _p(w_ih, F32, (4 * H, I), "w_ih"),
+                 _p(dheads, F32, (N, T, nh), "dheads"), nh, N, T, I, H,
+                 _p(dw_ih, F32, (4 * H, I), "dw_ih"), _p(dw_hh, F32, (4 * H, H), "dw_hh"),
+                 _p(db, F32, (4 * H,), "db"), _p(db_hh, F32, (4 * H,), "db_hh"), _p(dw_head, F32, (nh, H), "dw_head"), _p(None)),
+                pmax_zero)
+    return {"dw_ih": dw_ih, "dw_hh": dw_hh, "db": db, "db_hh": db_hh, "dw_head": dw_head}
 
 
 def lstm_bwd_caps(device, I, H):
@@ -639,7 +685,7 @@
 
 def lstm_bwd(x, keep, stash, w_ih, w_hh, y, h0, dy=None, dheads=None, w_head=None, dhn=None, dcn=None, need_dx=False,
              dgates=None, dw_ih=None, dw_hh=None, db=None, dw_head=None, want_dstate=True, wgrad_dheads=None, bwd_done=False,
-             db_hh=None):
+             db_hh=None, sumsq_partial=None, pmax_zero=None):
     N, T, I = x.shape
     H = w_hh.shape[1]
     dev = x.device
@@ -669,14 +715,14 @@
     if _t is not None:
         _t.record()
     _t = KERNEL_TIMER.bracket("lstm_wgrad")
-    check(lib().uav_lstm_wgrad(_h(x), _p(x, F32, (N, T, I), "x"), _p(keep, F32, (N, T), "keep"), _p(h0, F32, (N, H), "h0"),
-                               _p(y, F32, (N, T, H), "y"), _p(stash, F32, (N, T, 6 * H), "stash"),
-                               _pdg(dgates, N, T, H), _p(w_ih, F32, (4 * H, I), "w_ih"),
-                               _p(wgrad_dheads, F32, (N, T, nhw), "dheads"), nhw, N, T, I, H,
-                               _p(dw_ih, F32, (4 * H, I), "dw_ih"), _p(dw_hh, F32, (4 * H, H), "dw_hh"),
-                               _p(db, F32, (4 * H,), "db"), _p(db_hh, F32, (4 * H,), "db_hh"), _p(dw_head, F32, (nhw, H), "dw_head"),
-                               None if dx_in_bwd else _p(dx), _stream()),
-          "uav_lstm_wgrad")
+    _wgrad_call(sumsq_partial, H,
+                (_h(x), _p(x, F32, (N, T, I), "x"), _p(keep, F32, (N, T), "keep"), _p(h0, F32, (N, H), "h0"),
+                 _p(y, F32, (N, T, H), "y"), _p(stash, F32, (N, T, 6 * H), "stash"),
+                 _pdg(dgates, N, T, H), _p(w_ih, F32, (4 * H, I), "w_ih"),
+                 _p(wgrad_dheads, F32, (N, T, nhw), "dheads"), nhw, N, T, I, H,
+                 _p(dw_ih, F32, (4 * H, I), "dw_ih"), _p(dw_hh, F32, (4 * H, H), "dw_hh"),
+                 _p(db, F32, (4 * H,), "db"), _p(db_hh, F32, (4 * H,), "db_hh"), _p(dw_head, F32, (nhw, H), "dw_head"),
+                 None if dx_in_bwd else _p(dx)), pmax_zero)
     if _t is not None:
         _t.record()
     return {"dx": dx, "dw_ih": dw_ih, "dw_hh": dw_hh, "db": db, "dh0": dh0, "dc0": dc0, "dgates": dgates,
@@ -746,21 +792,25 @@
 
 
 def rollout_lstm(env_state, n_env, cfg, params, hidden, horizon, it, cur_obs, h, c, bufs, last_val=None,
-                 forced_act=None, noise=None, nan_count=None, stash=None, y=None, info=None, heads=None):
+                 forced_act=None, noise=None, nan_count=None, stash=None, y=None, info=None, heads=None, h0_out=None,
+                 c0_out=None):
     N, T, D = n_env, horizon, 6 + cfg.trend_k
+    snap = h0_out is not None or c0_out is not None
+    tail = (_p(h0_out, F32, (N, hidden), "h0_out"), _p(c0_out, F32, (N, hidden), "c0_out")) if snap else ()
+    fn = lib().uav_rollout_snapshot if snap else lib().uav_rollout
     _t = KERNEL_TIMER.bracket("rollout")
-    check(lib().uav_rollout(_h(cur_obs), _p(env_state, U8, name="env state"), N, C.byref(cfg), 1,
-                            _p(params, F32, name="params"), int(hidden), T, int(it),
-                            _p(cur_obs, F32, (N, D), "cur_obs"), _p(h, F32, (N, hidden), "h"), _p(c, F32, (N, hidden), "c"),
-                            _p(bufs["obs"], F32, (N, T, D), "obs"), _p(bufs["act"], I32, (N, T), "act"),
-                            _p(bufs["rew"], F32, (N, T), "rew"), _p(bufs["val"], F32, (N, T), "val"),
-                            _p(bufs["logp"], F32, (N, T), "logp"), _p(bufs["done"], F32, (N, T), "done"),
-                            _p(bufs["flags"], U8, (N, T), "flags"), _p(bufs["keep"], F32, (N, T), "keep"),
-                            _p(last_val, F32, (N,), "last_val"), _p(forced_act, I32, (N, T), "forced_act"),
-                            _p(noise, F64, (N, T, 2), "noise"), _p(nan_count, I32, (1,), "nan_count"),
-                            _p(stash, F32, (N, T, 6 * hidden), "stash"), _p(y, F32, (N, T, hidden), "y"),
-                            _p(info, F32, (N, T, 10), "info"), _p(heads, F32, (N, T, 6), "heads"), _stream()),
-          "uav_rollout")
+    check(fn(_h(cur_obs), _p(env_state, U8, name="env state"), N, C.byref(cfg), 1,
+             _p(params, F32, name="params"), int(hidden), T, int(it),
+             _p(cur_obs, F32, (N, D), "cur_obs"), _p(h, F32, (N, hidden), "h"), _p(c, F32, (N, hidden), "c"),
+             _p(bufs["obs"], F32, (N, T, D), "obs"), _p(bufs["act"], I32, (N, T), "act"),
+             _p(bufs["rew"], F32, (N, T), "rew"), _p(bufs["val"], F32, (N, T), "val"),
+             _p(bufs["logp"], F32, (N, T), "logp"), _p(bufs["done"], F32, (N, T), "done"),
+             _p(bufs["flags"], U8, (N, T), "flags"), _p(bufs["keep"], F32, (N, T), "keep"),
+             _p(last_val, F32, (N,), "last_val"), _p(forced_act, I32, (N, T), "forced_act"),
+             _p(noise, F64, (N, T, 2), "noise"), _p(nan_count, I32, (1,), "nan_count"),
+             _p(stash, F32, (N, T, 6 * hidden), "stash"), _p(y, F32, (N, T, hidden), "y"),
+             _p(info, F32, (N, T, 10), "info"), _p(heads, F32, (N, T, 6), "heads"), *tail, _stream()),
+          "uav_rollout_snapshot" if snap else "uav_rollout")
     if _t is not None:
         _t.record()
 
diff --git a/uav-wrf-les-ppo-lstm_amd/uavppo/policy.py b/uav-wrf-les-ppo-lstm_amd/uavppo/policy.py
--- a/uav-wrf-les-ppo-lstm_amd/uavppo/policy.py
+++ b/uav-wrf-les-ppo-lstm_amd/uavppo/policy.py
@@ -254,7 +254,12 @@
             x = y
         return ops.gemm(x.view(N, self.hidden), v["head.weight"], trans_b=True, bias=v["head.bias"])
 
-    def backward(self, dheads, work=None, dhead_bias=None):
+    def sumsq_ok(self):
+        return self.num_layers == 1 and self.obs_dim <= 6 and ops.lstm_wgrad_sumsq_count(self.hidden) > 0
+
+    def backward(self, dheads, work=None, dhead_bias=None, sumsq_partial=None, pmax_zero=None):
+        if sumsq_partial is not None and not self.sumsq_ok():
+            raise RuntimeError("backward: sumsq_partial needs one layer of h = 64 / 128 with 6 observation features")
         saved, keep, y_last = self._saved
         N, T, H = y_last.shape
         v, g = self.views, self.grad_views
@@ -308,7 +313,8 @@
                              wgrad_dheads=dheads.view(N, T, -1) if top else None,
                              need_dx=(l > 0), dgates=work.get("dgates"), dw_ih=g[f"lstm.weight_ih_l{l}"],
                              dw_hh=g[f"lstm.weight_hh_l{l}"], db=g[f"lstm.bias_ih_l{l}"],
-                             dw_head=g["head.weight"] if top else None, want_dstate=False, db_hh=g[f"lstm.bias_hh_l{l}"])
+                             dw_head=g["head.weight"] if top else None, want_dstate=False, db_hh=g[f"lstm.bias_hh_l{l}"],
+                             sumsq_partial=sumsq_partial, pmax_zero=pmax_zero)
             dy = r["dx"]
         self._saved = None
         return self.grad
diff --git a/uav-wrf-les-ppo-lstm_amd/uavppo/trainer.py b/uav-wrf-les-ppo-lstm_amd/uavppo/trainer.py
--- a/uav-wrf-les-ppo-lstm_amd/uavppo/trainer.py
+++ b/uav-wrf-les-ppo-lstm_amd/uavppo/trainer.py
@@ -48,12 +48,14 @@
 class VecPPOTrainer:
     def __init__(self, num_envs, horizon, policy="lstm", hidden=128, layers=1, variant="v2.0", device="cuda",
                  seed=1234, gae_mode="reference_exact", num_minibatches=1, bank=None, bank_sources=None,
-                 rank=0, world_size=1, use_curriculum=True, trend_k=0, log_info=False, device_curriculum=None, **hp):
+                 rank=0, world_size=1, use_curriculum=True, trend_k=0, log_info=False, device_curriculum=None,
+                 fewer_launches=True, **hp):
         self.hp = dict(DEFAULTS)
         self.hp.update(hp)
         self.N, self.T = int(num_envs), int(horizon)
         self.rank, self.world = int(rank), int(world_size)
         self._coll = self.world > 1 or collectives_on()
+        self.fewer_launches = bool(fewer_launches) and not self._coll
         self.device = torch.device(device)
         self.variant, self.seed = variant, int(seed)
         self.gae_mode = gae_mode
@@ -157,8 +159,12 @@
             self.work = {"stash": None}
             self._mlp_tmp = {"rew": torch.zeros(N, **f32), "done": torch.zeros(N, **f32),
                              "flags": torch.zeros(N, dtype=torch.uint8, device=d), "stash": None}
+        self._sumsq = None
         if policy == "lstm":
             self.dhead_bias = self.policy.grad_views["head.bias"]
+            if self.fewer_launches and self.policy.sumsq_ok():
+                self._sumsq = torch.zeros(ops.lstm_wgrad_sumsq_count(hidden), dtype=torch.float64, device=d)
+                self._rest = ((self.dhead_bias.data_ptr() - self.policy.grad.data_ptr()) // 4, self.dhead_bias.numel())
         self.dheads = torch.empty((N // self.num_minibatches) * T, 6, **f32)
         self.reset()
 
@@ -334,13 +340,16 @@
             self._state0.copy_(self._state)
             self._collect_stepwise_lstm(forced_act, noise)
         elif self.kind == "lstm":
-            self._state0.copy_(self._state)
+            snap = self.fewer_launches and self.trend_k == 0
+            if not snap:
+                self._state0.copy_(self._state)
             reuse = self.reuse_rollout_forward and self.num_minibatches == 1
             ops.rollout_lstm(self.env_state, self.N, self.env_cfg(), self.policy.flat, self.policy.hidden, self.T,
                              self.iteration, self.cur_obs, self.h[0], self.c[0], self.buf, last_val=self.last_val,
                              forced_act=forced_act, noise=noise, nan_count=self.nan_count,
                              stash=self.work["stash0"] if reuse else None, y=self.work["y0"] if reuse else None,
-                             info=self.info, heads=self.work["heads"] if reuse else None)
+                             info=self.info, heads=self.work["heads"] if reuse else None,
+                             h0_out=self.h0[0] if snap else None, c0_out=self.c0[0] if snap else None)
             self._rollout_forward_valid = reuse
         elif self.fused_mlp:
             ops.rollout_mlp(self.env_state, self.N, self.env_cfg(), self.policy.flat, self.T, self.iteration, self.cur_obs,
@@ -509,6 +518,10 @@
 
     def compute_advantages(self):
         b, hp = self.buf, self.hp
+        if self.fewer_launches:
+            ops.gae_normalise(b["rew"], b["val"], b["done"], hp["gamma"], hp["lam"], self.gae_mode, last_val=self.last_val,
+                              adv=self.adv, stats3=self.stats3, adv_out=self.adv_n, ret_out=self.ret)
+            return
         ops.gae(b["rew"], b["val"], b["done"], hp["gamma"], hp["lam"], self.gae_mode, last_val=self.last_val, out=self.adv)
         ops.adv_stats(self.adv, out=self.stats3)
         allreduce_adv_stats(self.stats3)
@@ -551,15 +564,21 @@
                     heads = self.policy.heads(b["obs"][sl].reshape(nb * T, self.obs_dim), stash=self.work["stash"])
                     ops.ppo_loss_heads(heads, *args)
                 if self.kind == "lstm":
-                    grad = self.policy.backward(self.dheads, self.work, self.dhead_bias)
+                    grad = self.policy.backward(self.dheads, self.work, self.dhead_bias, sumsq_partial=self._sumsq,
+                                                pmax_zero=None if self._sumsq is None else self.ranges[0:1])
                 elif not self.fused_mlp:
                     grad = self.policy.backward(self.dheads)
                 allreduce_grad(grad)
                 if self.record_grads:
                     self.grad_log.append((grad.clone(), self.policy.flat.clone()))
                 self.opt_step += 1
-                ops.clip_adam(self.policy.flat, grad, self.exp_avg, self.exp_avg_sq, self.opt_step, hp["lr"],
-                              max_norm=hp["max_grad_norm"], gnorm_out=self.gnorm, pmax_out=self.ranges[0:1])
+                if self._sumsq is not None:
+                    ops.clip_adam_presummed(self.policy.flat, grad, self.exp_avg, self.exp_avg_sq, self.opt_step, hp["lr"],
+                                            self._sumsq, *self._rest, max_norm=hp["max_grad_norm"], gnorm_out=self.gnorm,
+                                            pmax_out=self.ranges[0:1])
+                else:
+                    ops.clip_adam(self.policy.flat, grad, self.exp_avg, self.exp_avg_sq, self.opt_step, hp["lr"],
+                                  max_norm=hp["max_grad_norm"], gnorm_out=self.gnorm, pmax_out=self.ranges[0:1])
                 if self.record:
                     self.log.append((self.loss_sums.clone(), self.gnorm.clone()))
         if self._guarded():
```

New measurement: 74.12 million, median of 3. Within noise of the previous version (+0.0%).
